# trifectatechfoundation/zlib-rs

Hardware: NVIDIA H100
Metric: deflate_level6_raw_input_throughput_silesia_small_tar (higher is better)
Workload: dtype u8

## Files before the change

### __graft_entry__.py

```python
import os
import subprocess
import sys

ROOT = os.path.dirname(os.path.abspath(__file__))
if ROOT not in sys.path:
    sys.path.insert(0, ROOT)
sys.path.insert(0, os.path.join(ROOT, "tests"))


def build():
    subprocess.check_call(["make", "-C", os.path.join(ROOT, "zlib_rs_b200", "csrc"), "-j8"])
    subprocess.check_call(["make", "-C", os.path.join(ROOT, "oracle")])
    subprocess.check_call(["make", "-C", os.path.join(ROOT, "oracle"), "ref"])
    subprocess.check_call(["make", "-C", os.path.join(ROOT, "tests", "hostmodel")])
    import zlib_rs_b200
    zlib_rs_b200.lib()


def smoke():
    import zlib
    import zlib_rs_b200 as Z
    import oracle_lib as O
    from corpus import synthetic_mix
    d = synthetic_mix(300000, seed=1)
    out = Z.compress2(d, 6)
    assert out == O.compress(d, 6)[1], "GPU deflate differs from the oracle"
    assert zlib.decompress(out) == d
    assert Z.uncompress(out, len(d)) == d
    assert Z.crc32(d) == O.crc32(d) and Z.adler32(d) == O.adler32(d)
    print("smoke ok: %d -> %d bytes, bit-exact vs oracle" % (len(d), len(out)))


if __name__ == "__main__":
    build()
    if len(sys.argv) > 1 and sys.argv[1] == "smoke":
        smoke()
```

### include/zb_engine.h

```cpp
#ifndef ZB_ENGINE_H
#define ZB_ENGINE_H
#include <stddef.h>
#include <stdint.h>

#ifdef __cplusplus
extern "C" {
#endif

#define ZB_API __attribute__((visibility("default")))

#define ZB_OK 0
#define ZB_E_NODEVICE (-100)
#define ZB_E_CUDA (-101)
#define ZB_E_BUF (-5)
#define ZB_E_MEM (-4)
#define ZB_E_PARAM (-2)
#define ZB_E_DATA (-3)
#define ZB_E_INTERNAL (-102)

typedef struct zb_engine zb_engine;

typedef struct zb_deflate_result {
    uint64_t out_bytes;
    uint32_t check;
    int32_t data_type;
    uint32_t iterations;
    uint32_t n_symbols;
    uint32_t n_blocks;
    uint32_t gpu_launches;
    int32_t exact_parity;
    float gpu_ms;
    uint32_t bits_used;
    uint32_t carry;
} zb_deflate_result;

ZB_API zb_engine *zb_engine_create(int device, int *err);
ZB_API void zb_engine_destroy(zb_engine *e);
ZB_API const char *zb_last_error(void);
ZB_API int zb_device_count(void);

ZB_API int zb_deflate(zb_engine *e, const void *src, size_t src_len, int src_on_device, void *dst, size_t dst_cap, int dst_on_device,
               int level, int strategy, int window_bits, zb_deflate_result *res);
#define ZB_FLAG_NOT_LAST 1u
#define ZB_FLAG_LOW_PARALLEL 2u
#define ZB_FLAG_CHECK_ADLER 4u
#define ZB_FLAG_CHECK_CRC 8u
#define ZB_FLAG_END_PARTIAL 16u
#define ZB_FLAG_END_BLOCK 32u
#define ZB_FLAG_PRIME(bits, val) ((((uint32_t)(bits) & 7u) << 12) | (((uint32_t)(val) & 0xffu) << 16))
#define ZB_FLAG_MEMLEVEL(m) ((uint32_t)(m) << 8)
ZB_API int zb_deflate_ex(zb_engine *e, const void *src, size_t src_len, int src_on_device, void *dst, size_t dst_cap, int dst_on_device,
                  int level, int strategy, int window_bits, uint32_t flags, zb_deflate_result *res);
ZB_API int zb_deflate_dict(zb_engine *e, const void *dict, size_t dict_len, const void *src, size_t src_len, int src_on_device, void *dst,
                           size_t dst_cap, int dst_on_device, int level, int strategy, int window_bits, uint32_t flags, zb_deflate_result *res);
ZB_API size_t zb_deflate_bound(size_t src_len);

typedef struct zb_inflate_result {
    uint64_t out_bytes;
    uint64_t in_bytes;
    uint32_t check;
    int32_t status;
    uint32_t gpu_launches;
    float gpu_ms;
    char msg[64];
} zb_inflate_result;

ZB_API int zb_inflate(zb_engine *e, const void *src, size_t src_len, int src_on_device, void *dst, size_t dst_cap, int dst_on_device,
               int window_bits, zb_inflate_result *res);

#define ZB_INF_CHECK_ADLER 1u
#define ZB_INF_CHECK_CRC 2u
ZB_API int zb_inflate_ex(zb_engine *e, const void *src, size_t src_len, int src_on_device, void *dst, size_t dst_cap, int dst_on_device,
                         int window_bits, uint32_t flags, zb_inflate_result *res);

typedef struct zb_inflate_seg {
    uint64_t out_bytes;
    uint64_t end_bit;
    uint32_t final_block, need_input, sync_point;
    uint32_t check;
    uint32_t gpu_launches;
    float gpu_ms;
    char msg[64];
} zb_inflate_seg;
ZB_API int zb_inflate_blocks(zb_engine *e, const void *src, size_t src_len, uint64_t start_bit, const void *dict, size_t dict_len,
                             void *dst, size_t dst_cap, int check_kind, uint32_t check_start, zb_inflate_seg *out);

ZB_API int zb_adler32(zb_engine *e, uint32_t start, const void *buf, size_t len, int on_device, uint32_t *out, float *gpu_ms);
ZB_API int zb_crc32(zb_engine *e, uint32_t start, const void *buf, size_t len, int on_device, uint32_t *out, float *gpu_ms);

ZB_API void zb_engine_set_profile(zb_engine *e, int on);
ZB_API int zb_engine_get_profile(zb_engine *e, float *ms, uint32_t *launches, int n);

ZB_API void *zb_device_alloc(zb_engine *e, size_t bytes);
ZB_API void zb_device_free(zb_engine *e, void *p);
ZB_API int zb_copy_to_device(zb_engine *e, void *dst, const void *src, size_t bytes);
ZB_API int zb_copy_to_host(zb_engine *e, void *dst, const void *src, size_t bytes);
ZB_API int zb_device_fill_random(zb_engine *e, void *dst, size_t bytes, uint64_t seed);

#ifdef __cplusplus
}
#endif
#endif
```

### zlib_rs_b200/__init__.py

```python
import ctypes
import os

_HERE = os.path.dirname(os.path.abspath(__file__))
LIB_PATH = os.environ.get("ZB_LIB_PATH") or os.path.join(_HERE, "libz_b200.so")

Z_OK, Z_STREAM_END, Z_NEED_DICT = 0, 1, 2
Z_ERRNO, Z_STREAM_ERROR, Z_DATA_ERROR, Z_MEM_ERROR, Z_BUF_ERROR, Z_VERSION_ERROR = -1, -2, -3, -4, -5, -6
Z_NO_FLUSH, Z_PARTIAL_FLUSH, Z_SYNC_FLUSH, Z_FULL_FLUSH, Z_FINISH, Z_BLOCK = 0, 1, 2, 3, 4, 5
Z_DEFAULT_STRATEGY, Z_FILTERED, Z_HUFFMAN_ONLY, Z_RLE, Z_FIXED = 0, 1, 2, 3, 4
ZLIB_VERSION = b"1.3.0-zlib-rs-0.6.7-b200"
ZB_FLAG_NOT_LAST = 1
ZB_FLAG_LOW_PARALLEL = 2
ZB_FLAG_CHECK_ADLER = 4
ZB_FLAG_CHECK_CRC = 8


class ZStream(ctypes.Structure):
    _fields_ = [("next_in", ctypes.c_void_p), ("avail_in", ctypes.c_uint), ("total_in", ctypes.c_ulong),
                ("next_out", ctypes.c_void_p), ("avail_out", ctypes.c_uint), ("total_out", ctypes.c_ulong),
                ("msg", ctypes.c_char_p), ("state", ctypes.c_void_p), ("zalloc", ctypes.c_void_p),
                ("zfree", ctypes.c_void_p), ("opaque", ctypes.c_void_p), ("data_type", ctypes.c_int),
                ("adler", ctypes.c_ulong), ("reserved", ctypes.c_ulong)]


class DeflateResult(ctypes.Structure):
    _fields_ = [("out_bytes", ctypes.c_uint64), ("check", ctypes.c_uint32), ("data_type", ctypes.c_int32),
                ("iterations", ctypes.c_uint32), ("n_symbols", ctypes.c_uint32), ("n_blocks", ctypes.c_uint32),
                ("gpu_launches", ctypes.c_uint32), ("exact_parity", ctypes.c_int32), ("gpu_ms", ctypes.c_float),
                ("bits_used", ctypes.c_uint32), ("carry", ctypes.c_uint32)]


class InflateResult(ctypes.Structure):
    _fields_ = [("out_bytes", ctypes.c_uint64), ("in_bytes", ctypes.c_uint64), ("check", ctypes.c_uint32),
                ("status", ctypes.c_int32), ("gpu_launches", ctypes.c_uint32), ("gpu_ms", ctypes.c_float),
                ("msg", ctypes.c_char * 64)]


class ZlibError(Exception):
    def __init__(self, code, msg=""):
        super().__init__("zlib error %d %s" % (code, msg))
        self.code = code
        self.msg = msg


_lib = None


def lib():
    global _lib
    if _lib is None:
        if not os.path.exists(LIB_PATH):
            raise RuntimeError("libz_b200.so is not built: run `python -c 'import __graft_entry__ as g; g.build()'` "
                               "or `make -C zlib_rs_b200/csrc` (needs nvcc, sm_90a)")
        L = ctypes.CDLL(LIB_PATH, mode=ctypes.RTLD_LOCAL)
        vp, sz, u32, u64, ci = ctypes.c_void_p, ctypes.c_size_t, ctypes.c_uint32, ctypes.c_uint64, ctypes.c_int
        ul = ctypes.c_ulong
        zs = ctypes.POINTER(ZStream)
        L.zlibVersion.restype = ctypes.c_char_p
        L.zError.restype, L.zError.argtypes = ctypes.c_char_p, [ci]
        L.deflateInit2_.argtypes = [zs, ci, ci, ci, ci, ci, ctypes.c_char_p, ci]
        L.deflateInit_.argtypes = [zs, ci, ctypes.c_char_p, ci]
        L.deflate.argtypes = [zs, ci]
        L.deflateEnd.argtypes = [zs]
        L.deflateReset.argtypes = [zs]
        L.deflateBound.argtypes, L.deflateBound.restype = [zs, ul], ul
        L.inflateInit2_.argtypes = [zs, ci, ctypes.c_char_p, ci]
        L.inflateInit_.argtypes = [zs, ctypes.c_char_p, ci]
        L.inflate.argtypes = [zs, ci]
        L.inflateEnd.argtypes = [zs]
        L.compress2.argtypes = [vp, ctypes.POINTER(ul), vp, ul, ci]
        L.compress.argtypes = [vp, ctypes.POINTER(ul), vp, ul]
        L.compressBound.argtypes, L.compressBound.restype = [ul], ul
        L.uncompress.argtypes = [vp, ctypes.POINTER(ul), vp, ul]
        L.uncompress2.argtypes = [vp, ctypes.POINTER(ul), vp, ctypes.POINTER(ul)]
        for f in ("adler32", "crc32"):
            getattr(L, f).argtypes, getattr(L, f).restype = [ul, vp, ctypes.c_uint], ul
            getattr(L, f + "_z").argtypes, getattr(L, f + "_z").restype = [ul, vp, sz], ul
        L.adler32_combine.argtypes, L.adler32_combine.restype = [ul, ul, ctypes.c_long], ul
        L.crc32_combine.argtypes, L.crc32_combine.restype = [ul, ul, ctypes.c_long], ul
        L.crc32_combine_gen.argtypes, L.crc32_combine_gen.restype = [ctypes.c_long], ul
        L.adler32_combine64.argtypes, L.adler32_combine64.restype = [ul, ul, ctypes.c_longlong], ul
        L.crc32_combine64.argtypes, L.crc32_combine64.restype = [ul, ul, ctypes.c_longlong], ul
        L.crc32_combine_gen64.argtypes, L.crc32_combine_gen64.restype = [ctypes.c_longlong], ul
        L.crc32_combine_op.argtypes, L.crc32_combine_op.restype = [ul, ul, ul], ul
        L.zb_engine_create.argtypes, L.zb_engine_create.restype = [ci, ctypes.POINTER(ci)], vp
        L.zb_engine_destroy.argtypes = [vp]
        L.zb_last_error.restype = ctypes.c_char_p
        L.zb_device_count.restype = ci
        L.zb_deflate.argtypes = [vp, vp, sz, ci, vp, sz, ci, ci, ci, ci, ctypes.POINTER(DeflateResult)]
        L.zb_deflate_ex.argtypes = [vp, vp, sz, ci, vp, sz, ci, ci, ci, ci, u32, ctypes.POINTER(DeflateResult)]
        L.zb_deflate_bound.argtypes, L.zb_deflate_bound.restype = [sz], sz
        L.zb_inflate.argtypes = [vp, vp, sz, ci, vp, sz, ci, ci, ctypes.POINTER(InflateResult)]
        L.zb_adler32.argtypes = [vp, u32, vp, sz, ci, ctypes.POINTER(u32), ctypes.POINTER(ctypes.c_float)]
        L.zb_crc32.argtypes = [vp, u32, vp, sz, ci, ctypes.POINTER(u32), ctypes.POINTER(ctypes.c_float)]
        L.zb_engine_set_profile.argtypes = [vp, ci]
        L.zb_engine_get_profile.argtypes = [vp, ctypes.POINTER(ctypes.c_float), ctypes.POINTER(u32), ci]
        L.zb_device_alloc.argtypes, L.zb_device_alloc.restype = [vp, sz], vp
        L.zb_device_free.argtypes = [vp, vp]
        L.zb_copy_to_device.argtypes = [vp, vp, vp, sz]
        L.zb_copy_to_host.argtypes = [vp, vp, vp, sz]
        L.zb_device_fill_random.argtypes = [vp, vp, sz, u64]
        _lib = L
    return _lib


def _buf(data):
    data = bytes(data)
    return data, (ctypes.c_char * max(len(data), 1)).from_buffer_copy(data or b"\0")


def compressBound(n):
    return lib().compressBound(n)


def compress2(data, level=-1):
    data, src = _buf(data)
    n = ctypes.c_ulong(lib().compressBound(len(data)))
    dst = ctypes.create_string_buffer(n.value)
    rc = lib().compress2(dst, ctypes.byref(n), src, len(data), level)
    if rc != Z_OK:
        raise ZlibError(rc, lib().zb_last_error().decode())
    return dst.raw[: n.value]


def compress(data):
    return compress2(data, -1)


def uncompress(data, bufsize):
    data, src = _buf(data)
    n = ctypes.c_ulong(bufsize)
    dst = ctypes.create_string_buffer(max(bufsize, 1))
    rc = lib().uncompress(dst, ctypes.byref(n), src, len(data))
    if rc != Z_OK:
        raise ZlibError(rc, lib().zb_last_error().decode())
    return dst.raw[: n.value]


def crc32(data, value=0):
    data, src = _buf(data)
    return lib().crc32_z(value, src if data else None, len(data)) if data else (value if True else 0)


def adler32(data, value=1):
    data, src = _buf(data)
    return lib().adler32_z(value, src, len(data)) if data else value


class Deflate:

    def __init__(self, level=-1, window_bits=15, mem_level=8, strategy=0):
        self.s = ZStream()
        rc = lib().deflateInit2_(ctypes.byref(self.s), level, 8, window_bits, mem_level, strategy, ZLIB_VERSION,
                                 ctypes.sizeof(ZStream))
        if rc != Z_OK:
            raise ZlibError(rc, (self.s.msg or b"").decode())
        self._open = True

    def deflate(self, data, flush=Z_NO_FLUSH, out_chunk=1 << 16):
        data, src = _buf(data)
        self.s.next_in = ctypes.addressof(src)
        self.s.avail_in = len(data)
        out = bytearray()
        obuf = ctypes.create_string_buffer(out_chunk)
        while True:
            self.s.next_out = ctypes.addressof(obuf)
            self.s.avail_out = out_chunk
            rc = lib().deflate(ctypes.byref(self.s), flush)
            out += obuf.raw[: out_chunk - self.s.avail_out]
            if rc == Z_STREAM_END:
                break
            if rc == Z_BUF_ERROR and self.s.avail_in == 0:
                break
            if rc != Z_OK:
                raise ZlibError(rc, (self.s.msg or b"").decode())
            if self.s.avail_out != 0 and self.s.avail_in == 0:
                break
        self.last_rc = rc
        return bytes(out)

    @property
    def adler(self):
        return self.s.adler

    @property
    def total_in(self):
        return self.s.total_in

    @property
    def total_out(self):
        return self.s.total_out

    @property
    def data_type(self):
        return self.s.data_type

    def end(self):
        if self._open:
            self._open = False
            return lib().deflateEnd(ctypes.byref(self.s))
        return Z_OK

    def __del__(self):
        try:
            self.end()
        except Exception:
            pass


class Inflate:

    def __init__(self, window_bits=15):
        self.s = ZStream()
        rc = lib().inflateInit2_(ctypes.byref(self.s), window_bits, ZLIB_VERSION, ctypes.sizeof(ZStream))
        if rc != Z_OK:
            raise ZlibError(rc, (self.s.msg or b"").decode())
        self._open = True
        self.eof = False

    def inflate(self, data, flush=Z_NO_FLUSH, out_chunk=1 << 16):
        data, src = _buf(data)
        self.s.next_in = ctypes.addressof(src)
        self.s.avail_in = len(data)
        out = bytearray()
        obuf = ctypes.create_string_buffer(out_chunk)
        while True:
            self.s.next_out = ctypes.addressof(obuf)
            self.s.avail_out = out_chunk
            rc = lib().inflate(ctypes.byref(self.s), flush)
            out += obuf.raw[: out_chunk - self.s.avail_out]
            if rc == Z_STREAM_END:
                self.eof = True
                break
            if rc == Z_BUF_ERROR:
                break
            if rc != Z_OK:
                raise ZlibError(rc, (self.s.msg or b"").decode())
            if self.s.avail_out != 0 and self.s.avail_in == 0:
                break
        self.last_rc = rc
        return bytes(out)

    @property
    def adler(self):
        return self.s.adler

    def end(self):
        if self._open:
            self._open = False
            return lib().inflateEnd(ctypes.byref(self.s))
        return Z_OK

    def __del__(self):
        try:
            self.end()
        except Exception:
            pass


class Engine:
    def __init__(self, device=0):
        err = ctypes.c_int(0)
        self.h = lib().zb_engine_create(device, ctypes.byref(err))
        if not self.h:
            raise RuntimeError("zb_engine_create failed (%d): %s" % (err.value, lib().zb_last_error().decode()))

    def close(self):
        if self.h:
            lib().zb_engine_destroy(self.h)
            self.h = None

    def __del__(self):
        try:
            self.close()
        except Exception:
            pass

    def _check(self, rc):
        if rc != 0:
            raise ZlibError(rc, lib().zb_last_error().decode())

    def alloc(self, n):
        p = lib().zb_device_alloc(self.h, n)
        if not p:
            raise MemoryError("zb_device_alloc(%d)" % n)
        return p

    def free(self, p):
        lib().zb_device_free(self.h, p)

    def to_device(self, dptr, data):
        data, src = _buf(data)
        self._check(lib().zb_copy_to_device(self.h, dptr, src, len(data)))

    def to_host(self, dptr, n):
        dst = ctypes.create_string_buffer(max(n, 1))
        self._check(lib().zb_copy_to_host(self.h, dst, dptr, n))
        return dst.raw[:n]

    def deflate(self, src, n=None, level=6, strategy=0, window_bits=15, flags=0, src_on_device=False, dst=None, dst_cap=0,
                dst_on_device=False, mem_level=8):
        res = DeflateResult()
        flags |= (mem_level & 15) << 8
        keep = None
        if not src_on_device:
            data, keep = _buf(src)
            n = len(data)
            src = ctypes.addressof(keep)
        own = None
        if dst is None:
            dst_cap = lib().zb_deflate_bound(n) + 64
            own = ctypes.create_string_buffer(dst_cap)
            dst = ctypes.addressof(own)
            dst_on_device = False
        rc = lib().zb_deflate_ex(self.h, src, n, int(src_on_device), dst, dst_cap, int(dst_on_device), level, strategy,
                                 window_bits, flags, ctypes.byref(res))
        self._check(rc)
        return (own.raw[: res.out_bytes] if own is not None else None), res

    def inflate(self, src, out_cap, n=None, window_bits=15, src_on_device=False, dst=None, dst_on_device=False):
        res = InflateResult()
        keep = None
        if not src_on_device:
            data, keep = _buf(src)
            n = len(data)
            src = ctypes.addressof(keep)
        own = None
        if dst is None:
            own = ctypes.create_string_buffer(max(out_cap, 1))
            dst = ctypes.addressof(own)
        rc = lib().zb_inflate(self.h, src, n, int(src_on_device), dst, out_cap, int(dst_on_device), window_bits, ctypes.byref(res))
        return rc, (own.raw[: res.out_bytes] if own is not None else None), res

    def adler32(self, buf, n=None, start=1, on_device=False):
        out, ms = ctypes.c_uint32(0), ctypes.c_float(0)
        keep = None
        if not on_device:
            data, keep = _buf(buf)
            n = len(data)
            buf = ctypes.addressof(keep)
        self._check(lib().zb_adler32(self.h, start, buf, n, int(on_device), ctypes.byref(out), ctypes.byref(ms)))
        return out.value, ms.value

    def crc32(self, buf, n=None, start=0, on_device=False):
        out, ms = ctypes.c_uint32(0), ctypes.c_float(0)
        keep = None
        if not on_device:
            data, keep = _buf(buf)
            n = len(data)
            buf = ctypes.addressof(keep)
        self._check(lib().zb_crc32(self.h, start, buf, n, int(on_device), ctypes.byref(out), ctypes.byref(ms)))
        return out.value, ms.value

    PHASES = ["links", "match", "nxt", "path", "emit_holes", "tail", "blocks", "encode", "checksum", "h2d", "d2h", "match_first"]

    def set_profile(self, on=True):
        lib().zb_engine_set_profile(self.h, int(on))

    def get_profile(self):
        ms = (ctypes.c_float * 12)()
        ln = (ctypes.c_uint32 * 12)()
        k = lib().zb_engine_get_profile(self.h, ms, ln, 12)
        return {self.PHASES[i]: {"ms": ms[i], "launches": ln[i]} for i in range(min(k, len(self.PHASES)))}

    def fill_random(self, dptr, n, seed=42):
        self._check(lib().zb_device_fill_random(self.h, dptr, n, seed))
```

### zlib_rs_b200/csrc/zb_engine.cu

```cuda
#include <cuda_runtime.h>
#include <stdio.h>
#include <stdlib.h>
#include <string.h>
#include <new>
#include "../../include/zb_engine.h"
#include "zb_kernels.cuh"
#include "zb_engine_internal.h"

namespace zb {

constexpr uint32_t kSlowSub9 = 24576;
constexpr uint32_t kTailTiles = 2;
constexpr uint32_t kTailSub = 512;

thread_local char g_err[256] = "";

static void set_err(const char *what, cudaError_t e)
{
    snprintf(g_err, sizeof g_err, "%s: %s", what, cudaGetErrorString(e));
}

#define CK(call)                                                  \
    do {                                                          \
        cudaError_t e_ = (call);                                  \
        if (e_ != cudaSuccess) { set_err(#call, e_); return ZB_E_CUDA; } \
    } while (0)

__global__ void k_match(JobBufs);
__global__ void k_skip(JobBufs);
__global__ void k_nxt(JobBufs);
__global__ void k_path_tiles(JobBufs);
__global__ void k_path_chain(JobBufs, uint32_t, uint32_t);
__global__ void k_path_groups(JobBufs, uint32_t, uint32_t, uint4 *, uint32_t *);
__global__ void k_path_chain2(JobBufs, uint32_t, uint32_t, const uint4 *, uint32_t *, uint32_t *);
__global__ void k_path_mark(JobBufs, const uint32_t *, const uint32_t *);
__global__ void k_iter_lists(JobBufs, uint32_t *, uint32_t *, uint32_t);
__global__ void k_emit(JobBufs);
__global__ void k_holes(JobBufs, uint32_t);
__global__ void k_holes_cmp(JobBufs, uint32_t, uint32_t);
__global__ void k_tail(JobBufs);
__global__ void k_block_hist(JobBufs, uint32_t *);
__global__ void k_build_blocks(JobBufs, const uint32_t *);
__global__ void k_scan_blocks(JobBufs);
__global__ void k_encode(JobBufs);
__global__ void k_finish(JobBufs, const uint32_t *);
__global__ void k_literal_syms(JobBufs);
__global__ void k_stored(JobBufs);
__global__ void k_links2_std(JobBufs, uint32_t);
__global__ void k_links2_roll(JobBufs, uint32_t);
__global__ void k_links_fix_std(JobBufs);
__global__ void k_links_fix_roll(JobBufs);
__global__ void k_slow(JobBufs);
__global__ void k_rle(JobBufs);
__global__ void k_emit_slow(JobBufs);
__global__ void k_tail_slow(JobBufs);
__global__ void k_serial_low(JobBufs);
__global__ void k_links_dict_ghost(JobBufs, uint32_t *);
__global__ void k_links_dict_ghost_apply(JobBufs, const uint32_t *);

constexpr uint32_t kMatchSmemBytes = (kWSize + kMatchSub + 512) + (kWSize + kMatchSub) * 2 + ((kWSize + kMatchSub) / 32 + 1) * 4 * 4 + 8192;
constexpr uint32_t kPathSmemBytes = kPathTile * 4 * 3;
constexpr uint32_t kLinks2SmemBytes = 65536 * 2 + kLinkTile * 2 + kLinkTile + 64 + 2048;
constexpr uint32_t kSkipSmemBytes = 2 * kWSize * 2 + 2 * (2 * kWSize / 32) * 4 + 8192 + 64;
constexpr uint32_t kSlowSubMax = 24576;
constexpr uint32_t kSlowSmemBytes = (kWSize + kSlowSubMax + kSlowAhead) * 3;
constexpr uint32_t kChainSmemBytes = kChainChunkTiles * kPathHead * 8;
constexpr uint32_t kChain2MaxSmem = 200 * 1024;
constexpr uint32_t kSerialSmemBytes = (65536 + kWSize) * 2 + 35824 + 16;
constexpr uint32_t kSerialSmemQuick = 65536 * 2 + 65536 + 16;

int Engine::init(int dev)
{
    int n = 0;
    cudaError_t e = cudaGetDeviceCount(&n);
    if (e != cudaSuccess || n == 0) {
        snprintf(g_err, sizeof g_err, "no CUDA device (%s)", e == cudaSuccess ? "count 0" : cudaGetErrorString(e));
        return ZB_E_NODEVICE;
    }
    if (dev < 0 || dev >= n) { snprintf(g_err, sizeof g_err, "device %d out of range", dev); return ZB_E_PARAM; }
    device = dev;
    CK(cudaSetDevice(dev));
    CK(cudaStreamCreateWithFlags(&st, cudaStreamNonBlocking));
    CK(cudaStreamCreateWithFlags(&st2, cudaStreamNonBlocking));
    CK(cudaEventCreateWithFlags(&evf, cudaEventDisableTiming));
    CK(cudaEventCreateWithFlags(&evt, cudaEventDisableTiming));
    for (int i = 0; i < kUpChunks; i++) CK(cudaEventCreateWithFlags(&evc[i], cudaEventDisableTiming));
    CK(cudaEventCreateWithFlags(&evk, cudaEventDisableTiming));
    CK(cudaEventCreate(&ev0));
    CK(cudaEventCreate(&ev1));
    CK(upload_tables());
    CK(cudaFuncSetAttribute(k_match, cudaFuncAttributeMaxDynamicSharedMemorySize, kMatchSmemBytes));
    CK(cudaFuncSetAttribute(k_skip, cudaFuncAttributeMaxDynamicSharedMemorySize, kSkipSmemBytes));
    CK(cudaFuncSetAttribute(k_links2_std, cudaFuncAttributeMaxDynamicSharedMemorySize, kLinks2SmemBytes));
    CK(cudaFuncSetAttribute(k_links2_roll, cudaFuncAttributeMaxDynamicSharedMemorySize, kLinks2SmemBytes));
    CK(cudaFuncSetAttribute(k_slow, cudaFuncAttributeMaxDynamicSharedMemorySize, kSlowSmemBytes));
    CK(cudaFuncSetAttribute(k_path_tiles, cudaFuncAttributeMaxDynamicSharedMemorySize, kPathSmemBytes));
    CK(cudaFuncSetAttribute(k_path_mark, cudaFuncAttributeMaxDynamicSharedMemorySize, kPathSmemBytes));
    CK(cudaFuncSetAttribute(k_path_chain, cudaFuncAttributeMaxDynamicSharedMemorySize, kChainSmemBytes));
    CK(cudaFuncSetAttribute(k_path_groups, cudaFuncAttributeMaxDynamicSharedMemorySize, kChain2MaxSmem));
    CK(cudaFuncSetAttribute(k_path_chain2, cudaFuncAttributeMaxDynamicSharedMemorySize, kChain2MaxSmem));
    CK(cudaFuncSetAttribute(k_serial_low, cudaFuncAttributeMaxDynamicSharedMemorySize, kSerialSmemBytes));
    CK(cudaMallocHost(&h_info, sizeof(JobInfo)));
    CK(cudaMalloc(&d_info, sizeof(JobInfo)));
    CK(cudaMalloc(&d_check, 16));
    { int rc_ = inflate_init(); if (rc_ != ZB_OK) return rc_; }
    return ZB_OK;
}

Engine::~Engine()
{
    if (device < 0) return;
    cudaSetDevice(device);
    for (auto &b : bufs) if (b.p) cudaFree(b.p);
    if (h_stage) cudaFreeHost(h_stage);
    if (h_info) cudaFreeHost(h_info);
    if (d_info) cudaFree(d_info);
    if (d_check) cudaFree(d_check);
    if (ev0) cudaEventDestroy(ev0);
    if (ev1) cudaEventDestroy(ev1);
    if (evf) cudaEventDestroy(evf);
    if (evt) cudaEventDestroy(evt);
    for (int i = 0; i < kUpChunks; i++) if (evc[i]) cudaEventDestroy(evc[i]);
    if (evk) cudaEventDestroy(evk);
    if (st2) cudaStreamDestroy(st2);
    if (st) cudaStreamDestroy(st);
}

void Engine::pbegin()
{
    if (!profile) return;
    if (!pev0) { cudaEventCreate(&pev0); cudaEventCreate(&pev1); }
    cudaEventRecord(pev0, st);
}

void Engine::pend(int phase, uint32_t nlaunch)
{
    if (!profile) return;
    cudaEventRecord(pev1, st);
    cudaEventSynchronize(pev1);
    float ms = 0;
    cudaEventElapsedTime(&ms, pev0, pev1);
    phase_ms[phase] += ms;
    phase_launches[phase] += nlaunch;
}

int Engine::reserve(int slot, size_t bytes, void **out)
{
    Buf &b = bufs[slot];
    if (b.cap < bytes) {
        if (b.p) { cudaFree(b.p); b.p = nullptr; b.cap = 0; }
        size_t want = bytes + (bytes >> 3) + 4096;
        cudaError_t e = cudaMalloc(&b.p, want);
        if (e != cudaSuccess) { set_err("cudaMalloc", e); return ZB_E_MEM; }
        b.cap = want;
    }
    *out = b.p;
    return ZB_OK;
}

int Engine::stage(size_t bytes)
{
    if (h_stage_cap < bytes) {
        if (h_stage) cudaFreeHost(h_stage);
        h_stage = nullptr;
        h_stage_cap = 0;
        cudaError_t e = cudaMallocHost(&h_stage, bytes + (bytes >> 3) + 4096);
        if (e != cudaSuccess) { set_err("cudaMallocHost", e); return ZB_E_MEM; }
        h_stage_cap = bytes + (bytes >> 3) + 4096;
    }
    return ZB_OK;
}

enum { S_IN, S_L, S_HOLES, S_HOLESN, S_M, S_NXT, S_PEXIT, S_PCNT, S_SYMIDX, S_TENTRY, S_TSYMB, S_TDIRTY, S_SYMS, S_SYMB,
       S_BLOCKS, S_SCRATCH, S_FREQ, S_OUT, S_CK, S_INF0, S_INF1, S_PHEAD, S_SK, S_MARKN, S_LLIST, S_LCNT, S_BMAP, S_HDIFF, S_HCOARSE, S_CSTATE, S_LISTS, S_LR, S_LLAST, S_BBASE, S_MCHG, S_GFN, S_KEYS, S_COUNT };
static_assert(S_COUNT <= Engine::kSlots, "slots");

size_t deflate_bound(size_t n)
{
    return n + ((n + 7) >> 3) + ((n + 63) >> 6) + 5 + 18 + 64;
}

int Engine::deflate(const void *src, size_t n_in, bool src_dev, void *dst, size_t dst_cap, bool dst_dev, int level, int strategy,
                    int window_bits, uint32_t flags, zb_deflate_result *res, const void *dict, size_t dict_len)
{
    size_t dstart = 0;
    if (dict_len) {
        if (!dict || window_bits >= 0) { snprintf(g_err, sizeof g_err, "a dictionary needs a raw stream (the caller frames FDICT / DICTID)"); return ZB_E_PARAM; }
        if (dict_len >= 2 * (size_t)kWSize) { dict = static_cast<const uint8_t *>(dict) + (dict_len - kWSize); dict_len = kWSize; }
        dstart = dict_len;
    }
    const size_t n = n_in + dstart;
    int mem_level = (int)((flags >> 8) & 15u);
    if (mem_level == 0) mem_level = 8;
    if (mem_level > 9) return ZB_E_PARAM;
    if (!res || (!src && n) || !dst) return ZB_E_PARAM;
    memset(res, 0, sizeof *res);
    if (n > 0xF0000000ull) { snprintf(g_err, sizeof g_err, "input too large for one job (%zu)", n); return ZB_E_PARAM; }
    if (level == -1) level = 6;
    if (level < 0 || level > 9 || strategy < 0 || strategy > 4) return ZB_E_PARAM;
    uint32_t wrap;
    if (window_bits < 0) { if (window_bits < -15 || window_bits > -8) return ZB_E_PARAM; wrap = 0; }
    else if (window_bits > 15) { if (window_bits < 24 || window_bits > 31) return ZB_E_PARAM; wrap = 2; }
    else { if (window_bits < 8) return ZB_E_PARAM; wrap = 1; }
    const int wb = window_bits < 0 ? -window_bits : window_bits > 15 ? window_bits - 16 : window_bits;
    CK(cudaSetDevice(device));
    const uint32_t N = (uint32_t)n;
    launches = 0;

    JobBufs jb;
    memset(&jb, 0, sizeof jb);
    int rc;
    void *p;
    const size_t npad = (size_t)N + kPad;
    const uint32_t nwords = (N >> 5) + 2;
    const uint32_t nmt = N / kMatchTile + 1, npt = N / kPathTile + 1;
    const bool low_parallel = (flags & ZB_FLAG_LOW_PARALLEL) != 0 || dstart != 0;
    const bool serial_low = (level == 1 || level == 2) && strategy != 2 && strategy != 3 && !low_parallel;
    const uint32_t block_syms = (serial_low && level == 1) ? kBlockSyms : (1u << (mem_level + 6)) - 1u;
    const uint32_t max_blocks = N / block_syms + 2;
    const size_t out_cap = (deflate_bound(n) + 15) & ~(size_t)15;
    if ((rc = stage((size_t)nmt + 64 + ((size_t)N / 512 + 2 + npt + nmt + 8) * 4 + 64)) != ZB_OK) return rc;
    uint8_t *h_dirty = static_cast<uint8_t *>(h_stage);
    uint32_t *h_lists = reinterpret_cast<uint32_t *>(static_cast<uint8_t *>(h_stage) + (((size_t)nmt + 64 + 15) & ~(size_t)15));
#define RES(slot, bytes, field, type)                                   \
    if ((rc = reserve(slot, bytes, &p)) != ZB_OK) return rc;            \
    jb.field = static_cast<type>(p);
    uint8_t *d_in;
    if ((rc = reserve(S_IN, npad + 16, &p)) != ZB_OK) return rc;
    d_in = static_cast<uint8_t *>(p);
    jb.in = d_in;
    jb.N = N;
    jb.start = (uint32_t)dstart;
    jb.nmt = nmt;
    jb.tail_start = N > 2 * kTailZone ? N - kTailZone : 0;
    jb.block_syms = block_syms;
    jb.serial_mode = serial_low ? (uint32_t)level : 0u;
    RES(S_L, npad * 2, L, uint16_t *)
    RES(S_SK, npad * 2, SK, uint16_t *)
    RES(S_HOLES, (size_t)nwords * 4, holes, uint32_t *)
    RES(S_HOLESN, (size_t)nwords * 4, holes_new, uint32_t *)
    RES(S_M, npad * 4, M, uint32_t *)
    RES(S_NXT, ((size_t)N + 16) * 4, nxt, uint32_t *)
    RES(S_PEXIT, ((size_t)N + 16) * 4, pexit, uint32_t *)
    RES(S_PCNT, ((size_t)N + 16) * 4, pcnt, uint32_t *)
    RES(S_SYMIDX, ((size_t)N + 16) * 4, symidx, uint32_t *)
    RES(S_PHEAD, (size_t)npt * kPathHead * 8, phead, uint2 *)
    RES(S_TENTRY, (size_t)npt * 4, tile_entry, uint32_t *)
    RES(S_TSYMB, (size_t)npt * 4, tile_symbase, uint32_t *)
    RES(S_MARKN, (size_t)npt + 16, mark_needed, uint8_t *)
    const uint32_t nlists = npt * (kPathTile / kPathSub);
    RES(S_LLIST, (size_t)nlists * kLongPerSub * 4, long_list, uint32_t *)
    RES(S_LCNT, (size_t)nlists * 4, long_cnt, uint32_t *)
    RES(S_TDIRTY, (size_t)nmt + 16, tile_dirty, uint8_t *)
    RES(S_SYMS, ((size_t)N + 64) * sizeof(Sym), syms, Sym *)
    RES(S_SYMB, 40000 * 4, sym_base, uint32_t *)
    RES(S_BMAP, (size_t)nmt * 8192, bucket_map, uint32_t *)
    RES(S_LR, npad * 2, Lr, uint16_t *)
    RES(S_KEYS, npad * 2, keys, uint16_t *)
    RES(S_LLAST, (size_t)nmt * 65536 * 2, link_last, uint16_t *)
    RES(S_CSTATE, (size_t)(npt + 1) * 16, chain_state, uint4 *)
    uint32_t chainG = 16;
    while ((uint64_t)chainG * chainG < npt) chainG += 8;
    const uint32_t chain_groups = (npt + chainG - 1) / chainG;
    const uint32_t chain2_smem = chainG * kPathHead * 8 + chain_groups * kPathHead * 16 + chainG * 8;
    const bool chain2 = chain2_smem <= kChain2MaxSmem;
    if ((rc = reserve(S_GFN, (size_t)chain_groups * kPathHead * 16 + ((size_t)npt + 4) * 4, &p)) != ZB_OK) return rc;
    uint4 *d_gfn = static_cast<uint4 *>(p);
    uint32_t *d_mark_cnt = reinterpret_cast<uint32_t *>(d_gfn + (size_t)chain_groups * kPathHead);
    uint32_t *d_mark_list = d_mark_cnt + 4;
    auto launch_chain = [&](uint32_t first_tile) {
        if (chain2) {
            k_path_groups<<<chain_groups, 1024, chainG * kPathHead * 8, st>>>(jb, npt, chainG, d_gfn, d_mark_cnt);
            k_path_chain2<<<chain_groups, 1024, chain2_smem, st>>>(jb, npt, chainG, d_gfn, d_mark_list, d_mark_cnt);
            launches++;
        } else k_path_chain<<<1, 1024, kChainSmemBytes, st>>>(jb, npt, first_tile);
    };
    auto launch_mark = [&](uint32_t grid) {
        if (chain2) k_path_mark<<<grid < npt ? grid : npt, 1024, kPathSmemBytes, st>>>(jb, d_mark_list, d_mark_cnt);
        else k_path_mark<<<npt, 1024, kPathSmemBytes, st>>>(jb, nullptr, nullptr);
    };
    uint32_t *d_lists;
    const uint32_t max_list = N / 512 + 2;
    if ((rc = reserve(S_LISTS, ((size_t)max_list + npt + nmt + 8) * 4, &p)) != ZB_OK) return rc;
    d_lists = static_cast<uint32_t *>(p);
    RES(S_HDIFF, (size_t)nwords * 8, hdiff, uint32_t *)
    jb.hdiff_words = nwords;
    RES(S_HCOARSE, (size_t)(N >> 10) + 16, hcoarse, uint8_t *)
    RES(S_MCHG, (((size_t)N >> 8) + 16) * 4 + 64, mchg, uint8_t *)
    RES(S_BLOCKS, (size_t)max_blocks * sizeof(BlockDesc), blocks, BlockDesc *)
    RES(S_BBASE, (size_t)max_blocks * 4, block_base, uint32_t *)
    uint32_t *d_freq;
    if ((rc = reserve(S_FREQ, (size_t)max_blocks * 320 * 4, &p)) != ZB_OK) return rc;
    d_freq = static_cast<uint32_t *>(p);
    uint8_t *d_out;
    if (dst_dev && dst_cap >= out_cap) d_out = static_cast<uint8_t *>(dst);
    else { if ((rc = reserve(S_OUT, out_cap + 16, &p)) != ZB_OK) return rc; d_out = static_cast<uint8_t *>(p); }
    jb.out = d_out;
    jb.out_cap = out_cap;
    void *d_ck;
    const size_t ck_bytes = ((size_t)N / 16384 + 16) * 8;
    if ((rc = reserve(S_CK, ck_bytes, &d_ck)) != ZB_OK) return rc;
#undef RES
    jb.info = d_info;
    jb.level = (uint32_t)level;
    jb.strategy_fixed = strategy == 4;
    const bool lf_zero = strategy >= 2;
    jb.wrap = wrap;
    jb.hdr_len = wrap == 1 ? 2 : wrap == 2 ? 10 : 0;
    jb.huffman_only = strategy == 2 && level != 0;
    jb.not_last = (flags & ZB_FLAG_NOT_LAST) ? 1 : 0;
    jb.end_mode = (flags & ZB_FLAG_END_PARTIAL) ? 1u : (flags & ZB_FLAG_END_BLOCK) ? 2u : 0u;
    jb.prime_bits = (flags >> 12) & 7u;
    if ((jb.end_mode && !jb.not_last) || (jb.prime_bits && wrap != 0)) { snprintf(g_err, sizeof g_err, "END_* needs NOT_LAST, PRIME a raw stream"); return ZB_E_PARAM; }
    if (jb.not_last && (level == 0 || wrap != 0)) { snprintf(g_err, sizeof g_err, "NOT_LAST needs raw deflate and level > 0"); return ZB_E_PARAM; }
    jb.xfl = level == 9 ? 2 : (strategy >= 2 || level < 2) ? 4 : 0;
    int eng_level = level;
    const int wb_eff = wb == 8 ? 9 : wb;
    const bool small_ok = wb_eff < 15 && (uint64_t)N + kMinLookahead <= (1ull << wb_eff);
    bool exact = (wb_eff == 15 || small_ok) && (dstart == 0 || wb_eff == 15);
    jb.cinfo = small_ok ? (uint32_t)(wb_eff - 8) : 7u;
    jb.wsize = kWSize;
    const bool serial_win = wb_eff < 15 && !small_ok && N <= 32000u && level >= 3 && level <= 6 && strategy != 2 && strategy != 3;
    if (serial_win) {
        jb.wsize = 1u << wb_eff;
        jb.cinfo = (uint32_t)(wb_eff - 8);
        jb.tail_start = 0;
        exact = true;
    }
    const bool par_win = wb_eff < 15 && !small_ok && !serial_win && level >= 3 && level <= 6 && strategy != 2 && strategy != 3 && dstart == 0;
    if (par_win) {
        jb.wsize = 1u << wb_eff;
        jb.cinfo = (uint32_t)(wb_eff - 8);
        exact = true;
    }
    const bool slow_win = wb_eff < 15 && !small_ok && dstart == 0 && level != 0 && ((level >= 7 && strategy != 2) || strategy == 3);
    if (slow_win) {
        jb.wsize = 1u << wb_eff;
        jb.cinfo = (uint32_t)(wb_eff - 8);
        exact = true;
    }
    if (wb_eff < 15 && (level == 0 || (strategy == 2 && level != 0) || serial_low)) {
        jb.wsize = 1u << wb_eff;
        jb.cinfo = (uint32_t)(wb_eff - 8);
        exact = true;
    }
    if (level != 0 && !jb.huffman_only) {
        if (level < 3 && !serial_low) { eng_level = 3; exact = exact && strategy == 3; }
        if (strategy == 3) jb.slow_mode = 2;
        else if (level > 6) { jb.slow_mode = 1; jb.sp = slow_params(level); jb.sp.filtered = strategy == 1; jb.sp.wsize = jb.wsize; }
    }
    if (jb.slow_mode) jb.tail_start = N;
    jb.lp = level_params(eng_level);
    if (level != 0 && !jb.huffman_only) jb.level = (uint32_t)level;
    if (lf_zero && !jb.strategy_fixed && !jb.huffman_only) jb.level = 1;

    CK(cudaEventRecord(ev0, st));
    if (profile) { for (int i = 0; i < kPhases; i++) { phase_ms[i] = 0; phase_launches[i] = 0; } }
    uint32_t up_chunks = 0;
    size_t up_len[kUpChunks] = {0};
    const bool chunked_upload = !src_dev && !dstart && n_in >= ((size_t)4 << 20) && level != 0 && !jb.huffman_only &&
                                !jb.serial_mode && jb.slow_mode != 2;
    if (chunked_upload) {
        size_t chunk = (n_in / kUpChunks + kLinkTile - 1) / kLinkTile * kLinkTile;
        if (chunk < (size_t)device_sm_count() * kLinkTile) chunk = (size_t)device_sm_count() * kLinkTile;
        CK(cudaStreamWaitEvent(st2, ev0, 0));
        for (size_t off = 0; off < n_in; off += chunk) {
            const size_t len = n_in - off < chunk ? n_in - off : chunk;
            CK(cudaMemcpyAsync(d_in + off, static_cast<const uint8_t *>(src) + off, len, cudaMemcpyHostToDevice, st2));
            if (off + len == n_in) CK(cudaMemsetAsync(d_in + n, 0, kPad, st2));
            CK(cudaEventRecord(evc[up_chunks], st2));
            up_len[up_chunks++] = off + len;
        }
    } else {
        pbegin();
        if (dstart) CK(cudaMemcpyAsync(d_in, dict, dstart, src_dev ? cudaMemcpyDefault : cudaMemcpyHostToDevice, st));
        if (n_in) CK(cudaMemcpyAsync(d_in + dstart, src, n_in, src_dev ? cudaMemcpyDeviceToDevice : cudaMemcpyHostToDevice, st));
        CK(cudaMemsetAsync(d_in + n, 0, kPad, st));
        pend(9, 0);
    }
    CK(cudaMemsetAsync(d_info, 0, sizeof(JobInfo), st));
    CK(cudaMemsetAsync(d_out, 0, out_cap, st));
    if (jb.prime_bits) {
        h_prime = (uint8_t)((flags >> 16) & ((1u << jb.prime_bits) - 1u));
        CK(cudaMemcpyAsync(d_out, &h_prime, 1, cudaMemcpyHostToDevice, st));
    }
    cudaStream_t st_ck = chunked_upload ? st2 : st;
    pbegin();
    if (wrap == 1 || (wrap == 0 && (flags & ZB_FLAG_CHECK_ADLER))) { CK(launch_adler32(d_in + dstart, n_in, 1, d_ck, ck_bytes, d_check, st_ck)); launches += 2; }
    else if (wrap == 2 || (wrap == 0 && (flags & ZB_FLAG_CHECK_CRC))) { CK(launch_crc32(d_in + dstart, n_in, 0, d_ck, ck_bytes, d_check, st_ck)); launches += 2; }
    else CK(cudaMemsetAsync(d_check, 0, 4, st_ck));
    if (chunked_upload) CK(cudaEventRecord(evk, st2));
    pend(8, 2);

    auto links_tiles = [&](bool roll) {
        uint32_t t_done = 0;
        for (uint32_t k = 0; k < (chunked_upload ? up_chunks : 1u); k++) {
            uint32_t t_hi = nmt;
            if (chunked_upload) {
                cudaStreamWaitEvent(st, evc[k], 0);
                if (k + 1 < up_chunks) t_hi = up_len[k] >= 64 ? (uint32_t)((up_len[k] - 64) / kLinkTile) : 0;
            }
            if (t_hi <= t_done) continue;
            if (roll) k_links2_roll<<<t_hi - t_done, 1024, kLinks2SmemBytes, st>>>(jb, t_done);
            else k_links2_std<<<t_hi - t_done, 1024, kLinks2SmemBytes, st>>>(jb, t_done);
            if (k) launches++;
            t_done = t_hi;
        }
        if (chunked_upload) cudaStreamWaitEvent(st, evk, 0);
    };
    uint32_t iters = 0;
    if (level == 0) {
        const uint32_t nb = n_in == 0 ? 1 : (uint32_t)((n_in + 65534) / 65535);
        k_stored<<<nb, 256, 0, st>>>(jb);
        launches++;
        k_finish<<<1, 32, 0, st>>>(jb, d_check);
        launches++;
    } else {
        if (jb.huffman_only) {
            k_literal_syms<<<(uint32_t)(n_in / 256 + 1), 256, 0, st>>>(jb);
            launches++;
        } else if (jb.serial_mode) {
            iters = 1;
            pbegin();
            k_serial_low<<<1, 32, jb.serial_mode == 2 ? kSerialSmemBytes : kSerialSmemQuick, st>>>(jb);
            launches++;
            pend(1, 1);
        } else {
            CK(cudaMemsetAsync(jb.holes, 0, (size_t)nwords * 4, st));
            CK(cudaMemsetAsync(jb.holes_new, 0, (size_t)nwords * 4, st));
            CK(cudaMemsetAsync(jb.tile_dirty, 1, nmt, st));
            CK(cudaMemsetAsync(jb.tile_entry, 0xee, (size_t)npt * 4, st));
            CK(cudaMemsetAsync(jb.M + N, 0, (size_t)kPad * 4, st));
            CK(cudaMemsetAsync(jb.L + N, 0, (size_t)kPad * 2, st));
            pbegin();
            if (jb.slow_mode == 2) {
            } else if (jb.slow_mode && jb.sp.slow) {
                links_tiles(true);
                k_links_fix_roll<<<N / 256 + 1, 256, 0, st>>>(jb);
                launches += 2;
            } else {
                links_tiles(false);
                k_links_fix_std<<<N / 256 + 1, 256, 0, st>>>(jb);
                launches += 2;
                if (dstart >= 3 && n_in) {
                    uint32_t *d_first = reinterpret_cast<uint32_t *>(d_check) + 2;
                    CK(cudaMemsetAsync(d_first, 0xff, 4, st));
                    k_links_dict_ghost<<<(kMaxDist + 255) / 256, 256, 0, st>>>(jb, d_first);
                    k_links_dict_ghost_apply<<<1, 32, 0, st>>>(jb, d_first);
                    launches += 2;
                }
            }
            if (!jb.slow_mode) CK(cudaMemcpyAsync(jb.Lr, jb.L, npad * 2, cudaMemcpyDeviceToDevice, st));
            pend(0, 1);
            if (jb.slow_mode) {
                if (n_in > 0) {
                    iters = 1;
                    pbegin();
                    if (jb.slow_mode == 2) k_rle<<<(N + 255) / 256, 256, 0, st>>>(jb);
                    else {
                        jb.match_sub = level >= 9 ? kSlowSub9 : level == 8 ? 4096u : 8192u;
                        k_slow<<<(N + jb.match_sub - 1) / jb.match_sub, 1024, (kWSize + jb.match_sub + kSlowAhead) * 3, st>>>(jb);
                    }
                    pend(1, 1);
                    if (profile) phase_ms[11] = phase_ms[1];
                    pbegin();
                    k_path_tiles<<<npt, 1024, kPathSmemBytes, st>>>(jb);
                    launch_chain(0);
                    launch_mark(npt);
                    pend(3, 3);
                    pbegin();
                    k_emit_slow<<<(N + 255) / 256, 256, 0, st>>>(jb);
                    pend(4, 1);
                    launches += 5;
                }
                pbegin();
                k_tail_slow<<<1, 32, 0, st>>>(jb);
                launches++;
                pend(5, 1);
            } else {
            if (jb.tail_start > 0) {
                uint32_t n_dirty = nmt;
                for (;;) {
                    iters++;
                    uint32_t mthreads = 1024;
                    if (iters == 1) jb.match_sub = 4096;
                    else if (n_dirty <= kTailTiles) { jb.match_sub = kTailSub; mthreads = 256; }
                    else {
                        const uint64_t per_cta = (uint64_t)n_dirty * kMatchTile / (4 * (uint64_t)device_sm_count());
                        jb.match_sub = per_cta >= 8192 ? 8192 : per_cta >= 4096 ? 4096 : per_cta >= 2048 ? 2048 : 1024;
                    }
                    uint32_t nsub = (N + jb.match_sub - 1) / jb.match_sub;
                    uint32_t n_ptiles = npt, first_ptile = 0;
                    jb.skip_list = nullptr;
                    jb.nxt_list = nullptr;
                    if (iters > 1) {
                        jb.skip_list = d_lists;
                        jb.nxt_list = d_lists + nmt + 8;
                        n_ptiles = h_info->n_ptiles ? h_info->n_ptiles : 1;
                        first_ptile = h_info->first_ptile;
                        nsub = (n_dirty ? n_dirty : 1) * (kMatchTile / jb.match_sub);
                        if (n_dirty) {
                            pbegin();
                            k_skip<<<n_dirty, 1024, kSkipSmemBytes, st>>>(jb);
                            pend(1, 1);
                            launches++;
                        }
                    }
                    const uint32_t msmem = (kWSize + jb.match_sub + 512) + (kWSize + jb.match_sub) * 2 +
                                           (iters > 1 ? ((kWSize + jb.match_sub) / 32 + 1) * 4 * 4 + 8192 : 64);
                    jb.use_bucket_map = iters > 1;
                    pbegin();
                    k_match<<<nsub, mthreads, msmem, st>>>(jb);
                    pend(1, 1);
                    if (profile && iters == 1) phase_ms[11] = phase_ms[1];
                    pbegin();
                    k_nxt<<<n_ptiles * (kPathTile / 1024), 1024, 0, st>>>(jb);
                    pend(2, 1);
                    pbegin();
                    k_path_tiles<<<n_ptiles, 1024, kPathSmemBytes, st>>>(jb);
                    launch_chain(first_ptile);
                    launch_mark(iters == 1 ? npt : 2 * n_ptiles + 16);
                    pend(3, 3);
                    pbegin();
                    k_holes<<<(nlists * kLongPerSub + 255) / 256, 256, 0, st>>>(jb, nlists);
                    k_holes_cmp<<<(nwords + 255) / 256, 256, 0, st>>>(jb, nwords, nmt);
                    pend(4, 2);
                    launches += 7;
                    k_iter_lists<<<1, 1024, 0, st>>>(jb, d_lists, d_lists + nmt + 8, npt);
                    launches++;
                    CK(cudaMemcpyAsync(h_info, d_info, sizeof(JobInfo), cudaMemcpyDeviceToHost, st));
                    CK(cudaStreamSynchronize(st));
                    if (h_info->error) { snprintf(g_err, sizeof g_err, "engine error flags 0x%x (parse)", h_info->error); return ZB_E_INTERNAL; }
                    if (getenv("ZB_DEBUG")) {
                        static unsigned long long last[3];
                        if (iters == 1) memset(last, 0, sizeof last);
                        const double ctas = (double)(h_info->dbg[0] - last[0]) + 1e-9;
                        fprintf(stderr, "iter %u dirty %u: ctas %llu stage %.1f walk %.1f kcyc/cta, holes_changed %u\n", iters, n_dirty,
                                h_info->dbg[0] - last[0], (h_info->dbg[1] - last[1]) / 1e3 / ctas, (h_info->dbg[2] - last[2]) / 1e3 / ctas,
                                h_info->holes_changed);
                        memcpy(last, h_info->dbg, sizeof last);
                    }
                    if (!h_info->holes_changed) break;
                    n_dirty = h_info->n_dirty;
                    if (iters > N / 257u + 4096u) { snprintf(g_err, sizeof g_err, "hole iteration did not converge"); return ZB_E_INTERNAL; }
                }
            }
            CK(cudaEventRecord(evf, st));
            CK(cudaStreamWaitEvent(st2, evf, 0));
            k_tail<<<1, 32, 0, st2>>>(jb);
            launches++;
            CK(cudaEventRecord(evt, st2));
            if (jb.tail_start > 0) {
                pbegin();
                k_emit<<<(jb.tail_start + 255) / 256, 256, 0, st>>>(jb);
                launches++;
                pend(4, 1);
            }
            pbegin();
            CK(cudaStreamWaitEvent(st, evt, 0));
            pend(5, 1);
            }
        }
        CK(cudaMemcpyAsync(h_info, d_info, sizeof(JobInfo), cudaMemcpyDeviceToHost, st));
        CK(cudaStreamSynchronize(st));
        if (h_info->error) { snprintf(g_err, sizeof g_err, "engine error flags 0x%x (tail)", h_info->error); return ZB_E_INTERNAL; }
        const uint32_t nblocks = h_info->n_blocks;
        if (nblocks == 0 || nblocks > max_blocks) { snprintf(g_err, sizeof g_err, "bad block count %u", nblocks); return ZB_E_INTERNAL; }
        pbegin();
        k_block_hist<<<nblocks, 256, 0, st>>>(jb, d_freq);
        k_build_blocks<<<nblocks, 32, 0, st>>>(jb, d_freq);
        k_scan_blocks<<<1, 256, 0, st>>>(jb);
        pend(6, 3);
        pbegin();
        k_encode<<<nblocks, 1024, 0, st>>>(jb);
        k_finish<<<1, 32, 0, st>>>(jb, d_check);
        pend(7, 2);
        launches += 5;
    }
    CK(cudaMemcpyAsync(h_info, d_info, sizeof(JobInfo), cudaMemcpyDeviceToHost, st));
    CK(cudaStreamSynchronize(st));
    CK(cudaGetLastError());
    if (h_info->error) {
        if (h_info->error & 8u) return ZB_E_BUF;
        snprintf(g_err, sizeof g_err, "engine error flags 0x%x (encode)", h_info->error);
        return ZB_E_INTERNAL;
    }
    const uint64_t out_bytes = h_info->out_bytes;
    if (out_bytes > dst_cap) {
        res->out_bytes = out_bytes;
        return ZB_E_BUF;
    }
    if (d_out != dst) {
        pbegin();
        CK(cudaMemcpyAsync(dst, d_out, out_bytes, dst_dev ? cudaMemcpyDeviceToDevice : cudaMemcpyDeviceToHost, st));
        pend(10, 0);
    }
    CK(cudaEventRecord(ev1, st));
    CK(cudaStreamSynchronize(st));
    float ms = 0;
    CK(cudaEventElapsedTime(&ms, ev0, ev1));
    res->out_bytes = out_bytes;
    res->check = h_info->adler;
    res->data_type = (int32_t)h_info->data_type;
    res->iterations = iters;
    res->n_symbols = h_info->n_syms;
    res->n_blocks = h_info->n_blocks;
    res->gpu_launches = launches;
    res->exact_parity = exact ? 1 : 0;
    res->gpu_ms = ms;
    res->bits_used = (uint32_t)(h_info->total_bits & 7u) ? (uint32_t)(h_info->total_bits & 7u) : 8u;
    if (jb.not_last && jb.end_mode && (h_info->total_bits & 7u)) {
        uint8_t last = 0;
        CK(cudaMemcpy(&last, d_out + out_bytes, 1, cudaMemcpyDeviceToHost));
        res->carry = last & ((1u << (h_info->total_bits & 7u)) - 1u);
    }
    return ZB_OK;
}

int Engine::checksum(bool crc, uint32_t start, const void *buf, size_t len, bool on_dev, uint32_t *out, float *ms_out)
{
    if (!out) return ZB_E_PARAM;
    CK(cudaSetDevice(device));
    int rc;
    void *p;
    const uint8_t *d = static_cast<const uint8_t *>(buf);
    CK(cudaEventRecord(ev0, st));
    if (!on_dev && len) {
        if ((rc = reserve(S_IN, len + 16, &p)) != ZB_OK) return rc;
        CK(cudaMemcpyAsync(p, buf, len, cudaMemcpyHostToDevice, st));
        d = static_cast<const uint8_t *>(p);
    }
    void *d_ck;
    const size_t ck_bytes = (len / 16384 + 16) * 8;
    if ((rc = reserve(S_CK, ck_bytes, &d_ck)) != ZB_OK) return rc;
    if (crc) CK(launch_crc32(d, len, start, d_ck, ck_bytes, d_check, st));
    else CK(launch_adler32(d, len, start, d_ck, ck_bytes, d_check, st));
    launches = 2;
    CK(cudaMemcpyAsync(h_info, d_check, 4, cudaMemcpyDeviceToHost, st));
    CK(cudaEventRecord(ev1, st));
    CK(cudaStreamSynchronize(st));
    *out = *reinterpret_cast<uint32_t *>(h_info);
    if (ms_out) CK(cudaEventElapsedTime(ms_out, ev0, ev1));
    return ZB_OK;
}

__global__ void k_fill_random(uint64_t *dst, uint64_t nwords, uint64_t seed)
{
    for (uint64_t i = blockIdx.x * (uint64_t)blockDim.x + threadIdx.x; i < nwords; i += (uint64_t)gridDim.x * blockDim.x) {
        uint64_t z = (i + seed) * 0x9E3779B97F4A7C15ull;
        z = (z ^ (z >> 30)) * 0xBF58476D1CE4E5B9ull;
        z = (z ^ (z >> 27)) * 0x94D049BB133111EBull;
        dst[i] = z ^ (z >> 31);
    }
}

}

using zb::Engine;

extern "C" {

struct zb_engine { Engine e; };

const char *zb_last_error(void) { return zb::g_err; }

int zb_device_count(void)
{
    int n = 0;
    if (cudaGetDeviceCount(&n) != cudaSuccess) return 0;
    return n;
}

zb_engine *zb_engine_create(int device, int *err)
{
    zb_engine *z = new (std::nothrow) zb_engine;
    int rc = z ? z->e.init(device) : ZB_E_MEM;
    if (err) *err = rc;
    if (rc != ZB_OK) { delete z; return nullptr; }
    return z;
}

void zb_engine_destroy(zb_engine *z) { delete z; }

int zb_deflate(zb_engine *z, const void *src, size_t n, int src_dev, void *dst, size_t cap, int dst_dev, int level, int strategy,
               int window_bits, zb_deflate_result *res)
{
    if (!z) return ZB_E_NODEVICE;
    return z->e.deflate(src, n, src_dev != 0, dst, cap, dst_dev != 0, level, strategy, window_bits, 0, res);
}

int zb_deflate_dict(zb_engine *z, const void *dict, size_t dict_len, const void *src, size_t n, int src_dev, void *dst, size_t cap, int dst_dev,
                    int level, int strategy, int window_bits, uint32_t flags, zb_deflate_result *res)
{
    if (!z) return ZB_E_NODEVICE;
    return z->e.deflate(src, n, src_dev != 0, dst, cap, dst_dev != 0, level, strategy, window_bits, flags, res, dict, dict_len);
}

int zb_deflate_ex(zb_engine *z, const void *src, size_t n, int src_dev, void *dst, size_t cap, int dst_dev, int level, int strategy,
                  int window_bits, uint32_t flags, zb_deflate_result *res)
{
    if (!z) return ZB_E_NODEVICE;
    return z->e.deflate(src, n, src_dev != 0, dst, cap, dst_dev != 0, level, strategy, window_bits, flags, res);
}

size_t zb_deflate_bound(size_t n) { return zb::deflate_bound(n); }

int zb_inflate(zb_engine *z, const void *src, size_t n, int src_dev, void *dst, size_t cap, int dst_dev, int window_bits,
               zb_inflate_result *res)
{
    if (!z) return ZB_E_NODEVICE;
    return z->e.inflate(src, n, src_dev != 0, dst, cap, dst_dev != 0, window_bits, res);
}

int zb_inflate_ex(zb_engine *z, const void *src, size_t n, int src_dev, void *dst, size_t cap, int dst_dev, int window_bits, uint32_t flags,
                  zb_inflate_result *res)
{
    if (!z) return ZB_E_NODEVICE;
    return z->e.inflate(src, n, src_dev != 0, dst, cap, dst_dev != 0, window_bits, res, flags);
}

int zb_inflate_blocks(zb_engine *z, const void *src, size_t n, uint64_t start_bit, const void *dict, size_t dict_len, void *dst, size_t cap,
                      int check_kind, uint32_t check_start, zb_inflate_seg *out)
{
    if (!z) return ZB_E_NODEVICE;
    return z->e.inflate_blocks(src, n, start_bit, dict, dict_len, dst, cap, check_kind, check_start, out);
}

int zb_adler32(zb_engine *z, uint32_t start, const void *buf, size_t len, int on_dev, uint32_t *out, float *ms)
{
    if (!z) return ZB_E_NODEVICE;
    return z->e.checksum(false, start, buf, len, on_dev != 0, out, ms);
}

int zb_crc32(zb_engine *z, uint32_t start, const void *buf, size_t len, int on_dev, uint32_t *out, float *ms)
{
    if (!z) return ZB_E_NODEVICE;
    return z->e.checksum(true, start, buf, len, on_dev != 0, out, ms);
}

void zb_engine_set_profile(zb_engine *z, int on) { if (z) z->e.profile = on != 0; }

int zb_engine_get_profile(zb_engine *z, float *ms, uint32_t *launches, int n)
{
    if (!z) return 0;
    int k = n < Engine::kPhases ? n : Engine::kPhases;
    for (int i = 0; i < k; i++) { if (ms) ms[i] = z->e.phase_ms[i]; if (launches) launches[i] = z->e.phase_launches[i]; }
    return k;
}

void *zb_device_alloc(zb_engine *z, size_t bytes)
{
    if (!z) return nullptr;
    cudaSetDevice(z->e.device);
    void *p = nullptr;
    if (cudaMalloc(&p, bytes + zb::kPad + 16) != cudaSuccess) return nullptr;
    cudaMemset(static_cast<uint8_t *>(p) + bytes, 0, zb::kPad);
    return p;
}

void zb_device_free(zb_engine *z, void *p)
{
    if (!z || !p) return;
    cudaSetDevice(z->e.device);
    cudaFree(p);
}

int zb_copy_to_device(zb_engine *z, void *dst, const void *src, size_t bytes)
{
    if (!z) return ZB_E_NODEVICE;
    cudaSetDevice(z->e.device);
    return cudaMemcpy(dst, src, bytes, cudaMemcpyHostToDevice) == cudaSuccess ? ZB_OK : ZB_E_CUDA;
}

int zb_copy_to_host(zb_engine *z, void *dst, const void *src, size_t bytes)
{
    if (!z) return ZB_E_NODEVICE;
    cudaSetDevice(z->e.device);
    return cudaMemcpy(dst, src, bytes, cudaMemcpyDeviceToHost) == cudaSuccess ? ZB_OK : ZB_E_CUDA;
}

int zb_device_fill_random(zb_engine *z, void *dst, size_t bytes, uint64_t seed)
{
    if (!z) return ZB_E_NODEVICE;
    cudaSetDevice(z->e.device);
    zb::k_fill_random<<<zb::device_sm_count() * 8, 256, 0, z->e.st>>>(static_cast<uint64_t *>(dst), bytes / 8, seed);
    return cudaStreamSynchronize(z->e.st) == cudaSuccess ? ZB_OK : ZB_E_CUDA;
}

}
```

### zlib_rs_b200/csrc/zb_engine_internal.h

```cpp
#pragma once
#include <cuda_runtime.h>
#include <stddef.h>
#include <stdint.h>
#include "../../include/zb_engine.h"
#include "zb_kernels.cuh"

namespace zb {

extern thread_local char g_err[256];
size_t deflate_bound(size_t n);

struct Engine {
    static constexpr int kSlots = 40;
    struct Buf { void *p = nullptr; size_t cap = 0; };
    int device = -1;
    cudaStream_t st = nullptr, st2 = nullptr;
    cudaEvent_t evf = nullptr, evt = nullptr;
    cudaEvent_t ev0 = nullptr, ev1 = nullptr;
    static constexpr int kUpChunks = 8;
    cudaEvent_t evk = nullptr;
    cudaEvent_t evc[kUpChunks] = {nullptr};
    Buf bufs[kSlots];
    void *h_stage = nullptr;
    size_t h_stage_cap = 0;
    JobInfo *h_info = nullptr, *d_info = nullptr;
    uint32_t *d_check = nullptr;
    void *d_inf_state = nullptr, *h_inf_state = nullptr;
    uint32_t launches = 0;
    uint8_t h_prime = 0;
    static constexpr int kPhases = 12;
    bool profile = false;
    float phase_ms[kPhases] = {0};
    uint32_t phase_launches[kPhases] = {0};
    cudaEvent_t pev0 = nullptr, pev1 = nullptr;
    void pbegin();
    void pend(int phase, uint32_t nlaunch);

    int init(int dev);
    int inflate_init();
    ~Engine();
    int reserve(int slot, size_t bytes, void **out);
    int stage(size_t bytes);
    int deflate(const void *src, size_t n, bool src_dev, void *dst, size_t dst_cap, bool dst_dev, int level, int strategy,
                int window_bits, uint32_t flags, zb_deflate_result *res, const void *dict = nullptr, size_t dict_len = 0);
    int inflate(const void *src, size_t n, bool src_dev, void *dst, size_t dst_cap, bool dst_dev, int window_bits,
                zb_inflate_result *res, uint32_t flags = 0);
    int inflate_blocks(const void *src, size_t n, uint64_t start_bit, const void *dict, size_t dict_len, void *dst, size_t dst_cap,
                       int check_kind, uint32_t check_start, zb_inflate_seg *out);
    int checksum(bool crc, uint32_t start, const void *buf, size_t len, bool on_dev, uint32_t *out, float *ms);
};

}
```

### zlib_rs_b200/csrc/zb_kernels.cu

```cuda
#include "zb_kernels.cuh"

namespace zb {

__constant__ HuffTables c_tab;

cudaError_t upload_tables()
{
    HuffTables t;
    init_tables(t);
    return cudaMemcpyToSymbol(c_tab, &t, sizeof t);
}

struct GAcc {
    const uint8_t *data;
    uint32_t N;
    const uint16_t *L;
    const uint32_t *holes;
    const uint32_t *M;
    uint32_t w = kWSize;
    __device__ __forceinline__ uint32_t byte(uint32_t y) const
    {
        while (y >= N) {
            if (y < 2 * w) return 0;
            y -= w;
        }
        return data[y];
    }
    __device__ __forceinline__ uint32_t link(uint32_t y) const { return y + 4 <= N ? L[y] : 0; }
    __device__ __forceinline__ bool inserted(uint32_t y) const { return !((holes[y >> 5] >> (y & 31)) & 1u); }
    __device__ __forceinline__ Match mlook(uint32_t x) const
    {
        uint32_t v = M[x];
        return Match{v >> 16, x - (v & 0xffffu)};
    }
};

struct SAcc {
    const uint8_t *sdata;
    const uint16_t *sL;
    const uint32_t *sholes;
    uint32_t ws;
    __device__ __forceinline__ uint32_t byte(uint32_t y) const { return sdata[y - ws]; }
    __device__ __forceinline__ uint32_t link(uint32_t y) const { return sL[y - ws]; }
    __device__ __forceinline__ bool inserted(uint32_t y) const
    {
        uint32_t i = y - ws;
        return !((sholes[i >> 5] >> (i & 31)) & 1u);
    }
};

struct SAccR {
    const uint8_t *sdata;
    const uint16_t *sL;
    uint32_t ws;
    __device__ __forceinline__ uint32_t byte(uint32_t y) const { return sdata[y - ws]; }
    __device__ __forceinline__ uint32_t link(uint32_t y) const { const uint32_t v = sL[y - ws]; return v == 0xffffu ? 0u : v; }
    __device__ __forceinline__ bool inserted(uint32_t) const { return true; }
};


__device__ __forceinline__ uint32_t lds_u32(const uint32_t *words, uint32_t byte_idx)
{
    const uint32_t w = byte_idx >> 2;
    return __funnelshift_r(words[w], words[w + 1], (byte_idx & 3u) * 8u);
}

constexpr uint32_t kFirstFlag = 0xffffu;

template <bool kRoll>
__device__ __forceinline__ void links2_body(const JobBufs &jb, uint32_t tile0)
{
    const uint32_t tile = tile0 + blockIdx.x;
    extern __shared__ __align__(16) uint8_t smem[];
    constexpr uint32_t kKeys = kRoll ? 32768u : 65536u;
    uint16_t *head = reinterpret_cast<uint16_t *>(smem);
    uint16_t *lists = reinterpret_cast<uint16_t *>(smem + kKeys * 2);
    uint8_t *sd = smem + kKeys * 2 + kLinkTile * 2;
    uint16_t *run = reinterpret_cast<uint16_t *>(smem + kKeys * 2 + kLinkTile * 2 + kLinkTile + 64);
    __shared__ uint16_t c_base[32], c_total[32];
    const uint32_t *words = reinterpret_cast<const uint32_t *>(sd);
    const uint32_t tid = threadIdx.x, lane = tid & 31, warp = tid >> 5;
    const uint32_t N = jb.N, need = kRoll ? 3u : 4u, cap = kRoll ? jb.wsize - 1u : jb.wsize - kMinLookahead;
    const uint32_t ts = tile * kLinkTile;
    const uint32_t te = min(ts + kLinkTile, N);
    const uint32_t tv = N >= need ? min(te, N - need + 1) : ts;
    for (uint32_t i = tid; i < kKeys / 2; i += 1024) reinterpret_cast<uint32_t *>(head)[i] = 0;
    run[tid] = 0;
    {
        const uint4 *src = reinterpret_cast<const uint4 *>(jb.in + ts);
        uint4 *dst = reinterpret_cast<uint4 *>(sd);
        for (uint32_t i = tid; i < (te - ts + 16 + 15) / 16; i += 1024) dst[i] = src[i];
    }
    __syncthreads();
    const uint32_t nv = tv > ts ? tv - ts : 0;
    auto key_of = [&](uint32_t i) -> uint32_t { return kRoll ? hash_roll3(sd[i], sd[i + 1], sd[i + 2]) : hash_u32(lds_u32(words, i)); };
    uint16_t *myrun = run + warp * 32;
    for (uint32_t b = 0; b < 32; b++) {
        const uint32_t i = warp * 1024 + b * 32 + lane;
        const uint32_t key = i < nv ? key_of(i) : 0u;
        const uint32_t c = i < nv ? (key & 31u) : 32u;
        if (!kRoll && i < nv) jb.keys[ts + i] = (uint16_t)key;
        const uint32_t peers = __match_any_sync(0xffffffffu, c);
        if (c < 32u && (peers & ((1u << lane) - 1u)) == 0) myrun[c] += (uint16_t)__popc(peers);
        __syncwarp();
    }
    __syncthreads();
    if (warp == 0) {
        uint32_t tot = 0;
        for (uint32_t w = 0; w < 32; w++) { const uint32_t t = run[w * 32 + lane]; run[w * 32 + lane] = (uint16_t)tot; tot += t; }
        uint32_t incl = tot;
#pragma unroll
        for (int d = 1; d < 32; d <<= 1) { const uint32_t t = __shfl_up_sync(0xffffffffu, incl, d); if (lane >= (uint32_t)d) incl += t; }
        const uint32_t base = incl - tot;
        for (uint32_t w = 0; w < 32; w++) run[w * 32 + lane] += (uint16_t)base;
        c_base[lane] = (uint16_t)base;
        c_total[lane] = (uint16_t)tot;
    }
    __syncthreads();
    for (uint32_t b = 0; b < 32; b++) {
        const uint32_t i = warp * 1024 + b * 32 + lane;
        const uint32_t c = i < nv ? (key_of(i) & 31u) : 32u;
        const uint32_t peers = __match_any_sync(0xffffffffu, c);
        const uint32_t lower = peers & ((1u << lane) - 1u);
        if (c < 32u) {
            const uint32_t at = myrun[c];
            lists[at + __popc(lower)] = (uint16_t)i;
        }
        __syncwarp();
        if (c < 32u && lower == 0) myrun[c] += (uint16_t)__popc(peers);
        __syncwarp();
    }
    __syncthreads();
    {
        const uint32_t lb = c_base[warp], ln = c_total[warp];
        for (uint32_t k = 0; k < ln; k += 32) {
            const bool mine = k + lane < ln;
            const uint32_t m = __ballot_sync(0xffffffffu, mine);
            if (mine) {
                const uint32_t i = lists[lb + k + lane];
                const uint32_t key = key_of(i);
                const uint32_t peers = __match_any_sync(m, key);
                const uint32_t lower = peers & ((1u << lane) - 1u);
                const uint32_t pi = __shfl_sync(m, i, lower ? 31 - __clz(lower) : lane);
                const uint32_t pred = lower ? pi + 1 : head[key];
                uint32_t d = pred ? i + 1 - pred : kFirstFlag;
                if (pred && d > cap) d = 0;
                jb.L[ts + i] = (uint16_t)d;
                if ((peers >> lane) == 1u) head[key] = (uint16_t)(i + 1);
            }
            __syncwarp();
        }
    }
    for (uint32_t x = tv + tid; x < te; x += 1024) jb.L[x] = 0;
    __syncthreads();
    uint4 *out = reinterpret_cast<uint4 *>(jb.link_last + (size_t)tile * kKeys);
    const uint4 *hv = reinterpret_cast<const uint4 *>(head);
    for (uint32_t i = tid; i < kKeys * 2 / 16; i += 1024) out[i] = hv[i];
}

template <bool kRoll>
__device__ __forceinline__ void links_fix_body(const JobBufs &jb)
{
    constexpr uint32_t kKeys = kRoll ? 32768u : 65536u;
    const uint32_t x = blockIdx.x * 256 + threadIdx.x;
    if (x >= jb.N || jb.L[x] != kFirstFlag) return;
    const uint32_t tile = x / kLinkTile, cap = kRoll ? jb.wsize - 1u : jb.wsize - kMinLookahead;
    uint32_t d = 0;
    if (tile > 0) {
        const uint8_t *q = jb.in + x;
        const uint32_t key = kRoll ? hash_roll3(q[0], q[1], q[2])
                                   : hash_u32((uint32_t)q[0] | ((uint32_t)q[1] << 8) | ((uint32_t)q[2] << 16) | ((uint32_t)q[3] << 24));
        const uint32_t last = jb.link_last[(size_t)(tile - 1) * kKeys + key];
        if (last) {
            d = x - ((tile - 1) * kLinkTile + last - 1);
            if (d > cap) d = 0;
        }
    }
    jb.L[x] = (uint16_t)d;
}

__global__ void __launch_bounds__(1024) k_links2_std(JobBufs jb, uint32_t tile0) { links2_body<false>(jb, tile0); }
__global__ void __launch_bounds__(1024) k_links2_roll(JobBufs jb, uint32_t tile0) { links2_body<true>(jb, tile0); }
__global__ void __launch_bounds__(256) k_links_fix_std(JobBufs jb) { links_fix_body<false>(jb); }
__global__ void __launch_bounds__(256) k_links_fix_roll(JobBufs jb) { links_fix_body<true>(jb); }

constexpr uint32_t kSkipSpan = 2 * kWSize;
__global__ void __launch_bounds__(1024) k_skip(JobBufs jb)
{
    extern __shared__ __align__(16) uint8_t smem[];
    uint16_t *sL = reinterpret_cast<uint16_t *>(smem);
    uint32_t *sh = reinterpret_cast<uint32_t *>(smem + kSkipSpan * 2);
    uint32_t *sf = sh + kSkipSpan / 32;
    uint32_t *sbm = sf + kSkipSpan / 32;
    const uint32_t tile = jb.skip_list ? jb.skip_list[blockIdx.x] : blockIdx.x;
    const uint32_t ts = tile * kMatchTile;
    if (ts >= jb.N) return;
    const uint32_t te = min(ts + kMatchTile, jb.N);
    const uint32_t ws = ts >= kWSize ? ts - kWSize : 0;
    const uint32_t span = te - ws, tid = threadIdx.x;
    const uint32_t md = jb.wsize - kMinLookahead;
    {
        const uint4 *ls = reinterpret_cast<const uint4 *>(jb.L + ws);
        uint4 *ld = reinterpret_cast<uint4 *>(sL);
        for (uint32_t i = tid; i < (span + 7) / 8; i += 1024) ld[i] = ls[i];
        for (uint32_t i = tid; i < (span + 31) / 32; i += 1024) sh[i] = jb.holes[(ws >> 5) + i];
        const uint32_t *bm1 = jb.bucket_map + (size_t)tile * 2048, *bm0 = tile ? bm1 - 2048 : bm1;
        for (uint32_t i = tid; i < 2048; i += 1024) sbm[i] = bm0[i] | bm1[i];
    }
    __syncthreads();
    {
        const uint4 *kp = reinterpret_cast<const uint4 *>(jb.keys + ws);
        const uint32_t ngrp = ((span + 31) & ~31u) / 8, ngrp_w = (ngrp + 31) & ~31u;
#pragma unroll 4
        for (uint32_t g = tid; g < ngrp_w; g += 1024) {
            const bool valid = g < ngrp;
            const uint4 kv = valid ? kp[g] : make_uint4(0, 0, 0, 0);
            const uint32_t k[8] = {kv.x & 0xffffu, kv.x >> 16, kv.y & 0xffffu, kv.y >> 16, kv.z & 0xffffu, kv.z >> 16, kv.w & 0xffffu, kv.w >> 16};
            uint32_t b = 0;
#pragma unroll
            for (int j = 0; j < 8; j++) b |= ((sbm[k[j] >> 5] >> (k[j] & 31u)) & 1u) << j;
            b <<= 8 * (tid & 3u);
            b |= __shfl_xor_sync(0xffffffffu, b, 1);
            b |= __shfl_xor_sync(0xffffffffu, b, 2);
            if (valid && (tid & 3u) == 0) sf[g >> 2] = b;
        }
    }
    __syncthreads();
    const uint32_t lane = tid & 31, warp = tid >> 5, nwords = (span + 31) / 32;
    uint32_t nz[2];
#pragma unroll
    for (int h = 0; h < 2; h++) {
        const uint32_t w = warp * 64 + lane + 32 * h;
        nz[h] = __ballot_sync(0xffffffffu, w < nwords && (sh[w] & sf[w]) != 0);
    }
    for (uint32_t round = 0; round < 24; round++) {
        int ch = 0;
#pragma unroll
        for (int h = 0; h < 2; h++) {
            uint32_t m = nz[h];
            while (m) {
                const uint32_t w = warp * 64 + (__ffs(m) - 1) + 32 * h;
                m &= m - 1;
                const uint32_t i = w * 32 + lane;
                const bool on = (((sh[w] & sf[w]) >> lane) & 1u) && i < span;
                for (int rep = 0; rep < 6; rep++) {
                    bool c = false;
                    if (on) {
                        const uint32_t d = sL[i];
                        if (d != 0 && d <= i) {
                            const uint32_t t = i - d;
                            if ((sh[t >> 5] >> (t & 31)) & 1u) {
                                const uint32_t d2 = sL[t];
                                sL[i] = (uint16_t)((d2 == 0 || d + d2 > md) ? 0u : d + d2);
                                c = true;
                            }
                        }
                    }
                    __syncwarp();
                    if (!__any_sync(0xffffffffu, c)) break;
                    ch = 1;
                }
            }
        }
        if (!__syncthreads_or(ch)) break;
    }
    for (uint32_t i = ts - ws + tid; i < span; i += 1024) {
        if (sf[i >> 5] == 0) continue;
        if (!((sf[i >> 5] >> (i & 31)) & 1u)) continue;
        uint32_t d = sL[i];
        if (!((sh[i >> 5] >> (i & 31)) & 1u) && d != 0 && d <= i) {
            const uint32_t t = i - d;
            if ((sh[t >> 5] >> (t & 31)) & 1u) {
                const uint32_t d2 = sL[t];
                d = (d2 == 0 || d + d2 > md) ? 0u : d + d2;
            }
        }
        jb.Lr[ws + i] = (uint16_t)d;
    }
}

constexpr uint32_t kMatchData = kWSize + kMatchSub + 512;
constexpr uint32_t kMatchSmem = kMatchData + (kWSize + kMatchSub) * 2 + ((kWSize + kMatchSub) / 32) * 4;

constexpr uint32_t kBatch = 8;
constexpr uint32_t kBatchCmp = 2;
constexpr uint32_t kWalkBurst = 8;
constexpr uint32_t kCmpBurst = 4;
constexpr uint32_t kCoopCmp = 4;
enum { LS_IDLE = 0, LS_WALK = 1, LS_PEND = 2, LS_DONE = 3, LS_FIN = 4 };

struct DiffMaps {
    const uint32_t *del, *pdel;
    const uint32_t *add, *padd;
    __device__ __forceinline__ static bool any(const uint32_t *b, const uint32_t *p, uint32_t lo, uint32_t hi)
    {
        const uint32_t c_hi = p[hi >> 5] + __popc(b[hi >> 5] & ((1u << (hi & 31)) - 1u));
        const uint32_t c_lo = p[lo >> 5] + __popc(b[lo >> 5] & ((1u << (lo & 31)) - 1u));
        return c_hi != c_lo;
    }
};

__device__ __forceinline__ void sld_u64u(uint32_t a, uint32_t &lo, uint32_t &hi)
{
    const uint32_t al = a & ~3u, sh = (a & 3u) * 8u;
    const uint32_t w0 = sld_u32(al), w1 = sld_u32(al + 4), w2 = sld_u32(al + 8);
    lo = __funnelshift_r(w0, w1, sh);
    hi = __funnelshift_r(w1, w2, sh);
}

__device__ __forceinline__ void match_tile_fast(const JobBufs &jb, const uint8_t *sdata, const uint16_t *sL, const uint32_t *sbm,
                                                const DiffMaps dm, uint32_t ws, uint32_t te, uint32_t *s_next)
{
    const bool filt = jb.use_bucket_map != 0;
    const uint32_t dbase = (uint32_t)__cvta_generic_to_shared(sdata);
    const uint32_t lbase = (uint32_t)__cvta_generic_to_shared(sL);
    const uint32_t N = jb.N, nice = jb.lp.nice, budget = jb.lp.chain;
    const uint32_t md = jb.wsize - kMinLookahead;
    const uint32_t lane = threadIdx.x & 31;
    uint32_t *const Mout = jb.M + ws;
    uint16_t *const RDout = jb.SK + ws;
    uint32_t xr = 0;
    uint32_t cr = 0;
    uint32_t dn = 0;
    uint32_t best = 2, chain = 0, res = 0;
    uint32_t xb = 0;
    uint32_t fbase = 0;
    uint32_t lowr = 0;
    uint32_t clen = 0;
    uint32_t rd = 0;
    uint32_t xw4 = 0;
    uint32_t state = LS_IDLE;
    auto second_look = [&]() -> bool {
        const uint32_t w = sld_u32u((best >= 3u ? fbase - 3u : dbase) + cr) ^ xw4;
        return (best >= 3u ? w : (w & 0x00ffffffu)) == 0u;
    };
    auto load_xw4 = [&]() { xw4 = sld_u32u((best >= 3u ? fbase - 3u : dbase) + xr); };
    for (;;) {
        if (state == LS_WALK) {
            if (chain > kWalkBurst) {
                uint32_t crl = cr - lowr;
                uint32_t fl = fbase + lowr, ll = lbase + 2 * lowr;
                asm volatile("" : "+r"(fl), "+r"(ll));
                bool more = false;
#pragma unroll
                for (uint32_t k = 0; k < kWalkBurst; k++) {
                    const uint32_t fbk = sld_u8(fl + crl);
                    dn = sld_u16(ll + 2 * crl);
                    if (fbk == xb) break;
                    chain--;
                    if ((int32_t)crl < (int32_t)dn) break;
                    crl -= dn;
                    if (k + 1 == kWalkBurst) more = true;
                }
                cr = crl + lowr;
                const uint32_t fb = more ? ~xb : sld_u8(fl + crl);
                if (!more) {
                    if (fb == xb) {
                        if (second_look()) { state = LS_PEND; clen = 0; }
                        else {
                            chain--;
                            if (cr < lowr + dn) { rd = 0xffffu; state = LS_FIN; }
                            else cr -= dn;
                        }
                    }
                    else { rd = 0xffffu; state = LS_FIN; }
                }
            } else {
                const uint32_t fb = sld_u8(fbase + cr);
                dn = sld_u16(lbase + 2 * cr);
                if (fb == xb && second_look()) { state = LS_PEND; clen = 0; }
                else if (--chain == 0) { rd = (xr - cr) | 0x8000u; state = LS_FIN; }
                else if (cr < lowr + dn) { rd = 0xffffu; state = LS_FIN; }
                else cr -= dn;
            }
        }
        const uint32_t m_walk = __ballot_sync(0xffffffffu, state == LS_WALK);
        const uint32_t m_pend = __ballot_sync(0xffffffffu, state == LS_PEND);
        if (m_pend && (__popc(m_pend) >= (int)kBatchCmp || m_walk == 0)) {
            uint32_t len = 0;
            bool resolved = false;
            if (state == LS_PEND) {
                uint32_t pa = dbase + xr + clen, pb = dbase + cr + clen;
#pragma unroll 1
                for (uint32_t k = 0; k < kCmpBurst; k++) {
                    uint32_t a0, a1, b0, b1;
                    sld_u64u(pa, a0, a1);
                    sld_u64u(pb, b0, b1);
                    const uint32_t d0 = a0 ^ b0, d1 = a1 ^ b1;
                    if ((d0 | d1) != 0 || clen + 8 >= kMaxMatch) {
                        len = d0 ? clen + ((__ffs(d0) - 1) >> 3) : d1 ? clen + 4 + ((__ffs(d1) - 1) >> 3) : clen + 8;
                        resolved = true;
                        break;
                    }
                    clen += 8; pa += 8; pb += 8;
                }
            }
            uint32_t m_long = 0;
            if (__popc(m_walk | m_pend) <= kCoopCmp) m_long = __ballot_sync(0xffffffffu, state == LS_PEND && !resolved);
            if (m_long) {
                while (m_long) {
                    const uint32_t src = __ffs(m_long) - 1;
                    m_long &= m_long - 1;
                    const uint32_t cl0 = __shfl_sync(0xffffffffu, clen, src);
                    const uint32_t pa0 = __shfl_sync(0xffffffffu, dbase + xr + clen, src) + 8u * lane;
                    const uint32_t pb0 = __shfl_sync(0xffffffffu, dbase + cr + clen, src) + 8u * lane;
                    uint32_t a0, a1, b0, b1;
                    sld_u64u(pa0, a0, a1);
                    sld_u64u(pb0, b0, b1);
                    const uint32_t d0 = a0 ^ b0, d1 = a1 ^ b1;
                    const uint32_t mm = __ballot_sync(0xffffffffu, (d0 | d1) != 0);
                    const uint32_t first = mm ? __ffs(mm) - 1 : 0u;
                    const uint32_t mine = d0 ? ((__ffs(d0) - 1) >> 3) : 4u + ((__ffs(d1) - 1) >> 3);
                    const uint32_t bo = __shfl_sync(0xffffffffu, mine, first);
                    if (lane == src) { len = mm ? cl0 + 8u * first + bo : cl0 + 256u; resolved = true; }
                }
            }
            if (resolved) {
                if (len > kMaxMatch) len = kMaxMatch;
                state = LS_WALK;
                if (len > best) {
                    best = len;
                    res = (len << 16) | (xr - cr);
                    if (best >= nice) { rd = xr - cr; state = LS_FIN; }
                    else { fbase = dbase + best; xb = sld_u8(fbase + xr); load_xw4(); }
                }
                if (state == LS_WALK) {
                    if (--chain == 0) { rd = (xr - cr) | 0x8000u; state = LS_FIN; }
                    else if (cr < lowr + dn) { rd = 0xffffu; state = LS_FIN; }
                    else cr -= dn;
                }
            }
        }
        if (state == LS_FIN) {
            if (filt && Mout[xr] != res) jb.mchg[(ws + xr) >> 6] = 1;
            Mout[xr] = res; RDout[xr] = (uint16_t)rd; state = LS_IDLE;
        }
        const uint32_t m_idle = __ballot_sync(0xffffffffu, state == LS_IDLE);
        const uint32_t m_busy = __ballot_sync(0xffffffffu, state == LS_WALK || state == LS_PEND);
        if ((m_idle | m_busy) == 0) break;
        if (m_idle == 0) continue;
        if (__popc(m_idle) < (int)kBatch && m_busy != 0) continue;
        {
            uint32_t base = 0;
            const uint32_t leader = __ffs(m_idle) - 1;
            if (lane == leader) base = atomicAdd(s_next, (uint32_t)__popc(m_idle));
            base = __shfl_sync(0xffffffffu, base, leader);
            if (state == LS_IDLE) {
                const uint32_t x = base + __popc(m_idle & ((1u << lane) - 1u));
                if (x >= te) state = LS_DONE;
                else if (x + kMSafe > N) { jb.M[x] = 0; }
                else {
                    xr = x - ws;
                    bool skip = false;
                    if (filt) {
                        const uint32_t h = hash_u32(sld_u32u(dbase + xr));
                        skip = !((sbm[h >> 5] >> (h & 31)) & 1u);
                        if (!skip) {
                            const uint32_t rdo = RDout[xr];
                            const bool on_budget = rdo != 0xffffu && (rdo & 0x8000u);
                            const uint32_t lo = rdo == 0xffffu ? (xr > md ? xr - md : 0u) : xr - (rdo & 0x7fffu);
                            bool redo = DiffMaps::any(dm.del, dm.pdel, lo, xr);
                            if (!redo) {
                                if (on_budget) redo = DiffMaps::any(dm.add, dm.padd, lo, xr);
                                else {
                                    const uint32_t m = Mout[xr];
                                    if (m) { const uint32_t h2 = xr - (m & 0xffffu); redo = (dm.add[h2 >> 5] >> (h2 & 31)) & 1u; }
                                }
                            }
                            if (!redo) redo = sld_u16(lbase + 2 * xr) == md;
                            skip = !redo;
                        }
                    }
                    if (!skip) {
                        const uint32_t d0 = sld_u16(lbase + 2 * xr);
                        lowr = xr > md ? xr - md : 0;
                        if (ws == 0 && lowr == 0) lowr = 1;
                        if (xr < lowr + d0) {
                            if (filt && Mout[xr] != 0) jb.mchg[(ws + xr) >> 6] = 1;
                            Mout[xr] = 0; RDout[xr] = 0xffffu;
                        }
                        else {
                            cr = xr - d0;
                            if (lowr + md == xr) lowr++;
                            best = 2; chain = budget; res = 0;
                            fbase = dbase + 2;
                            xb = sld_u8(fbase + xr);
                            load_xw4();
                            state = LS_WALK;
                        }
                    }
                }
            }
        }
    }
}

__global__ void __launch_bounds__(1024, 2) k_match(JobBufs jb)
{
    extern __shared__ __align__(16) uint8_t smem[];
    __shared__ uint32_t s_next;
    __shared__ __align__(8) unsigned long long s_mbar;
    const uint32_t sub = jb.match_sub;
    const uint32_t per_tile = kMatchTile / sub;
    const uint32_t ts = (jb.skip_list ? jb.skip_list[blockIdx.x / per_tile] * per_tile + blockIdx.x % per_tile : blockIdx.x) * sub;
    if (ts >= jb.N) return;
    {
        const uint32_t t0 = ts / kMatchTile, t1 = (min(ts + sub, jb.N) - 1) / kMatchTile;
        if (!jb.tile_dirty[t0] && !jb.tile_dirty[t1]) return;
    }
    const uint32_t data_bytes = kWSize + sub + 512;
    uint8_t *sdata = smem;
    uint16_t *sL = reinterpret_cast<uint16_t *>(smem + data_bytes);
    uint32_t *sh = reinterpret_cast<uint32_t *>(smem + data_bytes + (kWSize + sub) * 2);
    uint32_t *sbm = sh;
    const uint32_t wmax = (kWSize + sub) / 32 + 1;
    uint32_t *sdel = sbm + 2048, *pdel = sdel + wmax, *sadd = pdel + wmax, *padd = sadd + wmax;
    __shared__ uint32_t s_wsum[32];
    const uint32_t N = jb.N;
    const uint32_t te = min(ts + sub, N);
    const uint32_t ws = ts >= kWSize ? ts - kWSize : 0;
    const uint32_t tid = threadIdx.x, nthr = blockDim.x;
    if (jb.use_bucket_map) {
        const uint32_t mt = ts / kMatchTile;
        const uint32_t *bm1 = jb.bucket_map + (size_t)mt * 2048, *bm0 = mt ? bm1 - 2048 : bm1;
        int hit = 0;
        for (uint32_t x = ts + tid; x < te; x += nthr) {
            const uint8_t *q = jb.in + x;
            const uint32_t h = hash_u32((uint32_t)q[0] | ((uint32_t)q[1] << 8) | ((uint32_t)q[2] << 16) | ((uint32_t)q[3] << 24));
            if (((bm0[h >> 5] | bm1[h >> 5]) >> (h & 31)) & 1u) {
                const uint32_t rd = jb.SK[x];
                const uint32_t lo = rd == 0xffffu ? (x > jb.wsize - kMinLookahead ? x - (jb.wsize - kMinLookahead) : 0u) : x - (rd & 0x7fffu);
                for (uint32_t b = lo >> 10; b <= (x >> 10); b++) hit |= jb.hcoarse[b];
            }
        }
        if (!__syncthreads_or(hit)) return;
        for (uint32_t i = tid; i < 2048; i += nthr) sbm[i] = bm0[i] | bm1[i];
        const uint32_t nwd = (te - ws + 31) / 32;
        const uint32_t per = (nwd + 1 + nthr - 1) / nthr;
        const uint32_t wb = tid * per;
        const uint32_t lane_ = tid & 31, warp_ = tid >> 5;
        for (int which = 0; which < 2; which++) {
            const uint32_t *src = which ? jb.hdiff : jb.hdiff + jb.hdiff_words;
            uint32_t *bits = which ? sadd : sdel, *pre = which ? padd : pdel;
            uint32_t mine = 0;
            for (uint32_t k = 0; k < per; k++) {
                const uint32_t w = wb + k;
                if (w <= nwd) { const uint32_t v = w < nwd ? src[(ws >> 5) + w] : 0u; bits[w] = v; mine += __popc(v); }
            }
            uint32_t incl = mine;
#pragma unroll
            for (int d = 1; d < 32; d <<= 1) {
                const uint32_t t = __shfl_up_sync(0xffffffffu, incl, d);
                if (lane_ >= (uint32_t)d) incl += t;
            }
            __syncthreads();
            if (lane_ == 31) s_wsum[warp_] = incl;
            __syncthreads();
            uint32_t run = incl - mine;
            for (uint32_t k = 0; k < warp_; k++) run += s_wsum[k];
            for (uint32_t k = 0; k < per; k++) {
                const uint32_t w = wb + k;
                if (w <= nwd) { pre[w] = run; run += __popc(bits[w]); }
            }
        }
    }
    if (tid == 0) {
        s_next = ts;
        const uint32_t mb = (uint32_t)__cvta_generic_to_shared(&s_mbar);
        asm volatile("mbarrier.init.shared::cta.b64 [%0], 1;" ::"r"(mb) : "memory");
        asm volatile("fence.proxy.async.shared::cta;" ::: "memory");
    }
    const long long t_0 = clock64();
    __syncthreads();
    {
        uint32_t n16 = (te + 512 - ws + 15) / 16;
        if (n16 > data_bytes / 16) n16 = data_bytes / 16;
        const bool bulk = (reinterpret_cast<uintptr_t>(jb.in) & 15u) == 0;
        if (bulk) {
            if (tid == 0) {
                const uint32_t mb = (uint32_t)__cvta_generic_to_shared(&s_mbar), dsts = (uint32_t)__cvta_generic_to_shared(sdata);
                asm volatile("mbarrier.arrive.expect_tx.shared::cta.b64 _, [%0], %1;" ::"r"(mb), "r"(n16 * 16u) : "memory");
                asm volatile("cp.async.bulk.shared::cluster.global.mbarrier::complete_tx::bytes [%0], [%1], %2, [%3];"
                             ::"r"(dsts), "l"(jb.in + ws), "r"(n16 * 16u), "r"(mb) : "memory");
            }
        } else {
            const uint4 *src = reinterpret_cast<const uint4 *>(jb.in + ws);
            uint4 *dst = reinterpret_cast<uint4 *>(sdata);
            for (uint32_t i = tid; i < n16; i += nthr) dst[i] = src[i];
        }
        const uint32_t nl = (te - ws + 7) / 8;
        const uint4 *ls = reinterpret_cast<const uint4 *>(jb.Lr + ws);
        uint4 *ld = reinterpret_cast<uint4 *>(sL);
        for (uint32_t i = tid; i < nl; i += nthr) {
            uint4 v = ls[i];
            v.x |= __vcmpeq2(v.x, 0u); v.y |= __vcmpeq2(v.y, 0u); v.z |= __vcmpeq2(v.z, 0u); v.w |= __vcmpeq2(v.w, 0u);
            ld[i] = v;
        }
        if (bulk) {
            const uint32_t mb = (uint32_t)__cvta_generic_to_shared(&s_mbar);
            uint32_t done = 0;
            while (!done) {
                asm volatile("{\n.reg .pred p;\nmbarrier.try_wait.parity.shared::cta.b64 p, [%1], 0;\nselp.u32 %0, 1, 0, p;\n}"
                             : "=r"(done) : "r"(mb) : "memory");
            }
        }
    }
    __syncthreads();
    const long long t_1 = clock64();
    const LevelParams lp = jb.lp;
    if (!lp.early_exit) {
        match_tile_fast(jb, sdata, sL, sbm, DiffMaps{sdel, pdel, sadd, padd}, ws, te, &s_next);
        __syncthreads();
        if (tid == 0) {
            const long long t_2 = clock64();
            atomicAdd(&jb.info->dbg[0], 1ull);
            atomicAdd(&jb.info->dbg[1], (unsigned long long)(t_1 - t_0));
            atomicAdd(&jb.info->dbg[2], (unsigned long long)(t_2 - t_1));
        }
        return;
    }
    SAccR a{sdata, sL, ws};
    for (uint32_t x = ts + tid; x < te; x += nthr) {
        uint32_t v = 0;
        if (jb.use_bucket_map && x + 4 <= N) {
            const uint32_t h = hash_u32(a.byte(x) | (a.byte(x + 1) << 8) | (a.byte(x + 2) << 16) | (a.byte(x + 3) << 24));
            if (!((sbm[h >> 5] >> (h & 31)) & 1u)) continue;
        }
        if (x + kMSafe <= N) {
            Match m = jb.wsize == kWSize ? lm_walk(a, x, 0xffffffffu, lp) : lm_walk(a, x, 0xffffffffu, lp, DynWin{jb.wsize});
            if (m.len) v = (m.len << 16) | (x - m.start);
        }
        if (jb.use_bucket_map && jb.M[x] != v) jb.mchg[x >> 6] = 1;
        jb.M[x] = v;
        jb.SK[x] = 0xffffu;
    }
}

constexpr uint32_t kMacroReach = 22016;

__device__ __forceinline__ bool path_tile_dirty(const JobBufs &jb, uint32_t pt)
{
    const uint32_t m0 = (pt * kPathTile) / kMatchTile;
    uint32_t m1 = ((pt + 1) * kPathTile + kMacroReach - 1) / kMatchTile;
    if (m1 >= jb.nmt) m1 = jb.nmt - 1;
    bool d = false;
    for (uint32_t m = m0; m <= m1; m++) d = d || jb.tile_dirty[m];
    return d;
}

__global__ void __launch_bounds__(1024) k_nxt(JobBufs jb)
{
    constexpr uint32_t per = kPathTile / 1024;
    const uint32_t tile = jb.nxt_list ? jb.nxt_list[blockIdx.x / per] : blockIdx.x / per;
    if (!path_tile_dirty(jb, tile)) return;
    const uint32_t p = tile * kPathTile + (blockIdx.x % per) * 1024 + threadIdx.x;
    if (p >= jb.tail_start) return;
    if (jb.use_bucket_map) {
        const uint32_t old = jb.nxt[p];
        const uint32_t b0 = p >> 6, b1 = min(p + (old & 0xffffu), jb.N) >> 6;
        bool chg = false;
        for (uint32_t b = b0; b <= b1; b++) chg = chg || jb.mchg[b];
        if (!chg) return;
    }
    GAcc a{jb.in, jb.N, jb.L, jb.holes, jb.M, jb.wsize};
    const uint32_t long_len = 16 * jb.lp.lazy;
    uint32_t ns = 0, nlong = 0, lpos = 0, llen = 0;
    auto see = [&](const Sym &s) {
        if (s.dist && (uint32_t)s.lc + 3u > long_len) { nlong++; lpos = s.pos; llen = s.lc + 3u; }
    };
    const uint32_t np = jb.wsize == kWSize ? macro_step(a, p, jb.lp, jb.tail_start, see, &ns)
                                           : macro_step(a, p, jb.lp, jb.tail_start, see, &ns, DynWin{jb.wsize});
    const uint32_t delta = np - p;
    if (delta > 0xffffu || ns > 0xffu || delta == 0) atomicOr(&jb.info->error, 1u);
    if (nlong && (nlong != 1 || lpos + llen != np || (jb.lp.early_exit ? lpos != p : (llen != 257u && llen != 258u))))
        atomicOr(&jb.info->error, 16u);
    jb.nxt[p] = (delta & 0xffffu) | ((ns & 0xffu) << 16) | (nlong ? kNxtLong : 0u) | (llen == 258u ? kNxtLong258 : 0u) |
                (np >= jb.tail_start ? kNxtTail : 0u);
}

constexpr uint32_t kStuck = 0x80000000u;
__device__ __forceinline__ void path_subtile(const uint32_t *nx, uint32_t *ex, uint32_t *cn, uint32_t s0, uint32_t s1, uint32_t lane)
{
    for (int32_t b = (int32_t)s1 - 32; b >= (int32_t)s0; b -= 32) {
        const uint32_t p = (uint32_t)b + lane;
        const uint32_t v = nx[p];
        uint32_t t, c;
        if (v & kNxtTail) { t = kStuck | p; c = 0; }
        else { t = p + (v & 0xffffu); c = (v >> 16) & 0xffu; }
#pragma unroll
        for (int r = 0; r < 5; r++) {
            const bool inb = !(t & kStuck) && t < (uint32_t)b + 32u;
            const uint32_t src = inb ? t - (uint32_t)b : lane;
            const uint32_t t2 = __shfl_sync(0xffffffffu, t, src);
            const uint32_t c2 = __shfl_sync(0xffffffffu, c, src);
            if (inb) { t = t2; c += c2; }
        }
        if (!(t & kStuck) && t < s1) { c += cn[t]; t = ex[t]; }
        ex[p] = t;
        cn[p] = c;
        __syncwarp();
    }
}

constexpr uint32_t kPathSmem = kPathTile * 4 * 3;

__device__ __forceinline__ void path_load(const JobBufs &jb, uint32_t tbeg, uint32_t *nx)
{
    const uint4 *src = reinterpret_cast<const uint4 *>(jb.nxt + tbeg);
    uint4 *dst = reinterpret_cast<uint4 *>(nx);
#pragma unroll 4
    for (uint32_t g = threadIdx.x; g < kPathTile / 4; g += blockDim.x) {
        const uint32_t p = tbeg + 4 * g;
        uint4 v;
        if (p + 3 < jb.tail_start) v = src[g];
        else {
            const uint32_t t = kNxtTail | 1u;
            v.x = p < jb.tail_start ? jb.nxt[p] : t;
            v.y = p + 1 < jb.tail_start ? jb.nxt[p + 1] : t;
            v.z = p + 2 < jb.tail_start ? jb.nxt[p + 2] : t;
            v.w = t;
        }
        dst[g] = v;
    }
}

__global__ void __launch_bounds__(1024) k_path_tiles(JobBufs jb)
{
    extern __shared__ __align__(16) uint8_t smem[];
    uint32_t *nx = reinterpret_cast<uint32_t *>(smem);
    uint32_t *ex = nx + kPathTile;
    uint32_t *cn = ex + kPathTile;
    const uint32_t tile = jb.nxt_list ? jb.nxt_list[blockIdx.x] : blockIdx.x;
    const uint32_t tbeg = tile * kPathTile;
    if (!path_tile_dirty(jb, tile)) return;
    path_load(jb, tbeg, nx);
    __syncthreads();
    const uint32_t warp = threadIdx.x >> 5, lane = threadIdx.x & 31;
    constexpr uint32_t kExitSub = 1024, nsub = kPathTile / kExitSub;
    for (uint32_t s = warp; s < nsub; s += blockDim.x / 32) path_subtile(nx, ex, cn, s * kExitSub, (s + 1) * kExitSub, lane);
    __syncthreads();
    for (int32_t j = (int32_t)nsub - 2; j >= 0; j--) {
        for (uint32_t i = threadIdx.x; i < kExitSub; i += blockDim.x) {
            const uint32_t p = (uint32_t)j * kExitSub + i;
            uint32_t t = ex[p];
            if (!(t & kStuck) && t < kPathTile) { cn[p] += cn[t]; ex[p] = ex[t]; }
        }
        __syncthreads();
    }
    for (uint32_t i = threadIdx.x; i < kPathTile; i += blockDim.x) {
        const uint32_t p = tbeg + i;
        const uint32_t t = ex[i];
        const uint32_t xa = (t & kStuck) ? (kStuck | (tbeg + (t & ~kStuck))) : tbeg + t;
        if (p < jb.tail_start) {
            jb.pexit[p] = xa;
            jb.pcnt[p] = cn[i];
        }
        if (i < kPathHead) jb.phead[(size_t)tile * kPathHead + i] = make_uint2(xa, cn[i]);
    }
}

constexpr uint32_t kChainChunk = kChainChunkTiles;
__global__ void __launch_bounds__(1024) k_path_chain(JobBufs jb, uint32_t ntiles, uint32_t first_tile)
{
    extern __shared__ __align__(16) uint8_t smem[];
    uint2 *hd = reinterpret_cast<uint2 *>(smem);
    __shared__ uint32_t s_e, s_base, s_done, s_tail;
    __shared__ uint32_t c_entry[kChainChunk], c_base[kChainChunk];
    if (threadIdx.x == 0) {
        if (first_tile == 0) { s_e = jb.start; s_base = 0; s_done = jb.tail_start == 0; s_tail = jb.start; }
        else { const uint4 v = jb.chain_state[first_tile]; s_e = v.x; s_base = v.y; s_done = v.z; s_tail = v.w; }
    }
    for (uint32_t t = threadIdx.x; t < first_tile; t += blockDim.x) jb.mark_needed[t] = 0;
    __syncthreads();
    for (uint32_t c0 = first_tile; c0 < ntiles; c0 += kChainChunk) {
        const uint32_t nt = min(kChainChunk, ntiles - c0);
        for (uint32_t i = threadIdx.x; i < nt * kPathHead; i += blockDim.x) hd[i] = jb.phead[(size_t)c0 * kPathHead + i];
        __syncthreads();
        if (threadIdx.x == 0) {
            uint32_t e = s_e, base = s_base;
            bool done = s_done != 0;
            uint32_t tail_entry = s_tail;
            for (uint32_t k = 0; k < nt; k++) {
                const uint32_t tbeg = (c0 + k) * kPathTile, tend = tbeg + kPathTile;
                jb.chain_state[c0 + k] = make_uint4(e, base, done ? 1u : 0u, tail_entry);
                c_base[k] = base;
                if (done || e >= tend || e >= jb.tail_start) { c_entry[k] = 0xffffffffu; continue; }
                c_entry[k] = e;
                uint32_t x, c;
                if (e - tbeg < kPathHead) { const uint2 v = hd[k * kPathHead + (e - tbeg)]; x = v.x; c = v.y; }
                else { x = jb.pexit[e]; c = jb.pcnt[e]; }
                base += c;
                if (x & kStuck) { tail_entry = x & ~kStuck; done = true; }
                else e = x;
            }
            s_e = e; s_base = base; s_done = done; s_tail = tail_entry;
        }
        __syncthreads();
        for (uint32_t k = threadIdx.x; k < nt; k += blockDim.x) {
            const uint32_t t = c0 + k;
            jb.tile_symbase[t] = c_base[k];
            jb.mark_needed[t] = (jb.tile_entry[t] != c_entry[k]) || path_tile_dirty(jb, t);
            jb.tile_entry[t] = c_entry[k];
        }
        __syncthreads();
    }
    if (threadIdx.x == 0) {
        uint32_t tail_entry = s_tail;
        if (!s_done) { tail_entry = s_e; if (s_e < jb.tail_start) atomicOr(&jb.info->error, 2u); }
        jb.info->tail_entry = tail_entry;
        jb.info->n_mid_syms = s_base;
    }
}

struct ChainState { uint32_t e, base, done, tail; };

template <bool OUT>
__device__ __forceinline__ void chain_walk_group(const JobBufs &jb, const uint2 *hd, uint32_t t0, uint32_t nt, ChainState &s,
                                                 uint32_t *c_entry, uint32_t *c_base)
{
    for (uint32_t k = 0; k < nt; k++) {
        const uint32_t tbeg = (t0 + k) * kPathTile, tend = tbeg + kPathTile;
        if (OUT) c_base[k] = s.base;
        if (s.done || s.e >= tend || s.e >= jb.tail_start) { if (OUT) c_entry[k] = 0xffffffffu; continue; }
        if (OUT) c_entry[k] = s.e;
        uint32_t x, c;
        if (s.e - tbeg < kPathHead) { const uint2 v = hd[k * kPathHead + (s.e - tbeg)]; x = v.x; c = v.y; }
        else { x = jb.pexit[s.e]; c = jb.pcnt[s.e]; }
        s.base += c;
        if (x & kStuck) { s.tail = x & ~kStuck; s.done = 1; }
        else s.e = x;
    }
}

__device__ __forceinline__ void chain_stage_heads(const JobBufs &jb, uint2 *hd, uint32_t t0, uint32_t nt)
{
    const uint4 *src = reinterpret_cast<const uint4 *>(jb.phead + (size_t)t0 * kPathHead);
    uint4 *dst = reinterpret_cast<uint4 *>(hd);
    for (uint32_t i = threadIdx.x; i < nt * kPathHead / 2; i += blockDim.x) dst[i] = src[i];
}

__global__ void __launch_bounds__(1024) k_path_groups(JobBufs jb, uint32_t ntiles, uint32_t G, uint4 *gfn, uint32_t *mark_cnt)
{
    if (blockIdx.x == 0 && threadIdx.x == 0) *mark_cnt = 0;
    extern __shared__ __align__(16) uint8_t smem[];
    uint2 *hd = reinterpret_cast<uint2 *>(smem);
    const uint32_t t0 = blockIdx.x * G, nt = min(G, ntiles - t0);
    chain_stage_heads(jb, hd, t0, nt);
    __syncthreads();
    if (threadIdx.x < kPathHead) {
        ChainState s{t0 * kPathTile + threadIdx.x, 0u, 0u, 0u};
        chain_walk_group<false>(jb, hd, t0, nt, s, nullptr, nullptr);
        gfn[(size_t)blockIdx.x * kPathHead + threadIdx.x] = make_uint4(s.e, s.base, s.done, s.tail);
    }
}

__global__ void __launch_bounds__(1024) k_path_chain2(JobBufs jb, uint32_t ntiles, uint32_t G, const uint4 *gfn, uint32_t *mark_list,
                                                        uint32_t *mark_cnt)
{
    extern __shared__ __align__(16) uint8_t smem[];
    uint2 *hd = reinterpret_cast<uint2 *>(smem);
    uint4 *sg = reinterpret_cast<uint4 *>(smem + (size_t)G * kPathHead * 8);
    uint32_t *c_entry = reinterpret_cast<uint32_t *>(sg + (size_t)blockIdx.x * kPathHead), *c_base = c_entry + G;
    __shared__ ChainState s_st;
    __shared__ uint32_t s_j;
    const uint32_t g = blockIdx.x;
    for (uint32_t i = threadIdx.x; i < g * kPathHead; i += blockDim.x) sg[i] = gfn[i];
    if (threadIdx.x == 0) { s_st = ChainState{jb.start, 0u, jb.tail_start == 0 ? 1u : 0u, jb.start}; s_j = 0; }
    __syncthreads();
    for (;;) {
        if (threadIdx.x == 0) {
            ChainState s = s_st;
            uint32_t j = s_j;
            for (; j < g; j++) {
                const uint32_t gbeg = j * G * kPathTile;
                if (s.done || s.e >= jb.tail_start || s.e - gbeg >= G * kPathTile) continue;
                if (s.e - gbeg >= kPathHead) break;
                const uint4 f = sg[j * kPathHead + (s.e - gbeg)];
                s.e = f.x; s.base += f.y;
                if (f.z) { s.done = 1; s.tail = f.w; }
            }
            s_st = s; s_j = j;
        }
        __syncthreads();
        const uint32_t j = s_j;
        if (j >= g) break;
        chain_stage_heads(jb, hd, j * G, G);
        __syncthreads();
        if (threadIdx.x == 0) {
            ChainState s = s_st;
            chain_walk_group<false>(jb, hd, j * G, G, s, nullptr, nullptr);
            s_st = s; s_j = j + 1;
        }
        __syncthreads();
    }
    const uint32_t t0 = g * G, nt = min(G, ntiles - t0);
    chain_stage_heads(jb, hd, t0, nt);
    __syncthreads();
    if (threadIdx.x == 0) {
        ChainState s = s_st;
        chain_walk_group<true>(jb, hd, t0, nt, s, c_entry, c_base);
        if (g == gridDim.x - 1) {
            uint32_t tail_entry = s.tail;
            if (!s.done) { tail_entry = s.e; if (s.e < jb.tail_start) atomicOr(&jb.info->error, 2u); }
            jb.info->tail_entry = tail_entry;
            jb.info->n_mid_syms = s.base;
        }
    }
    __syncthreads();
    for (uint32_t k = threadIdx.x; k < nt; k += blockDim.x) {
        const uint32_t t = t0 + k;
        jb.tile_symbase[t] = c_base[k];
        const bool mn = (jb.tile_entry[t] != c_entry[k]) || path_tile_dirty(jb, t);
        jb.mark_needed[t] = mn;
        jb.tile_entry[t] = c_entry[k];
        if (mn) mark_list[atomicAdd(mark_cnt, 1u)] = t;
    }
}

__global__ void __launch_bounds__(1024) k_path_mark(JobBufs jb, const uint32_t *list, const uint32_t *list_cnt)
{
    extern __shared__ __align__(16) uint8_t smem[];
    uint32_t *nx = reinterpret_cast<uint32_t *>(smem);
    uint32_t *ex = nx + kPathTile;
    uint32_t *cn = ex + kPathTile;
    __shared__ uint32_t sub_entry[kPathTile / kPathSub], sub_base[kPathTile / kPathSub];
    constexpr uint32_t nsub = kPathTile / kPathSub;
    const uint32_t count = list ? *list_cnt : gridDim.x;
    for (uint32_t b = blockIdx.x; b < count; b += gridDim.x) {
        const uint32_t tile = list ? list[b] : b;
        const uint32_t tbeg = tile * kPathTile;
        if (!jb.mark_needed[tile]) continue;
        const uint32_t entry = jb.tile_entry[tile];
        if (threadIdx.x < nsub) jb.long_cnt[tile * nsub + threadIdx.x] = 0;
        if (entry == 0xffffffffu) {
            for (uint32_t i = threadIdx.x; i < kPathTile; i += blockDim.x)
                if (tbeg + i < jb.tail_start) jb.symidx[tbeg + i] = 0;
            continue;
        }
        __syncthreads();
        path_load(jb, tbeg, nx);
        __syncthreads();
        const uint32_t warp = threadIdx.x >> 5, lane = threadIdx.x & 31;
        for (uint32_t s = warp; s < nsub; s += blockDim.x / 32) path_subtile(nx, ex, cn, s * kPathSub, (s + 1) * kPathSub, lane);
        __syncthreads();
        if (threadIdx.x == 0) {
            uint32_t cur = entry - tbeg, cbase = 0;
            for (uint32_t j = 0; j < nsub; j++) {
                if (!(cur & kStuck) && cur < (j + 1) * kPathSub) {
                    sub_entry[j] = cur;
                    sub_base[j] = cbase;
                    cbase += cn[cur];
                    cur = ex[cur];
                } else sub_entry[j] = 0xffffffffu;
            }
        }
        __syncthreads();
        for (uint32_t i = threadIdx.x; i < kPathTile; i += blockDim.x) ex[i] = 0;
        __syncthreads();
        if (threadIdx.x < nsub) {
            const uint32_t s = threadIdx.x;
            uint32_t p = sub_entry[s];
            if (p != 0xffffffffu) {
                uint32_t idx = sub_base[s], nlong = 0;
                const uint32_t s1 = (s + 1) * kPathSub;
                uint32_t *ll = jb.long_list + (size_t)(tile * nsub + s) * kLongPerSub;
                while (p < s1) {
                    const uint32_t v = nx[p];
                    if (v & kNxtTail) break;
                    if (v & kNxtLong) {
                        if (nlong < kLongPerSub) ll[nlong++] = tbeg + p;
                        else atomicOr(&jb.info->error, 32u);
                    }
                    ex[p] = idx + 1;
                    idx += (v >> 16) & 0xffu;
                    p += v & 0xffffu;
                }
                jb.long_cnt[tile * nsub + s] = nlong;
            }
        }
        __syncthreads();
        for (uint32_t i = threadIdx.x; i < kPathTile; i += blockDim.x)
            if (tbeg + i < jb.tail_start) jb.symidx[tbeg + i] = ex[i];
    }
}

__global__ void __launch_bounds__(256) k_holes(JobBufs jb, uint32_t nlists)
{
    const uint32_t t = blockIdx.x * blockDim.x + threadIdx.x;
    {
        const uint32_t nthr = gridDim.x * blockDim.x;
        for (uint32_t i = t; i < jb.nmt; i += nthr) jb.tile_dirty[i] = 0;
        for (uint32_t i = t; i < jb.nmt * 512; i += nthr) reinterpret_cast<uint4 *>(jb.bucket_map)[i] = make_uint4(0, 0, 0, 0);
        for (uint32_t i = t; i < (jb.N >> 10) + 16; i += nthr) jb.hcoarse[i] = 0;
        for (uint32_t i = t; i < (jb.N >> 8) + 16; i += nthr) reinterpret_cast<uint32_t *>(jb.mchg)[i] = 0;
        if (t == 0) jb.info->holes_changed = 0;
    }
    const uint32_t list = t / kLongPerSub, slot = t % kLongPerSub;
    if (list >= nlists || slot >= jb.long_cnt[list]) return;
    const uint32_t p = jb.long_list[(size_t)list * kLongPerSub + slot];
    const uint32_t v = jb.nxt[p], delta = v & 0xffffu;
    const uint32_t len = jb.lp.early_exit ? delta : ((v & kNxtLong258) ? 258u : 257u);
    const uint32_t pos = p + delta - len;
    uint32_t y0 = pos + 1, y1 = pos + len - 1;
    uint32_t *hn = jb.holes_new;
    while (y0 < y1) {
        const uint32_t w = y0 >> 5, lo = y0 & 31;
        const uint32_t n = min(32u - lo, y1 - y0);
        const uint32_t mask = (n == 32 ? 0xffffffffu : ((1u << n) - 1u)) << lo;
        atomicOr(&hn[w], mask);
        y0 += n;
    }
}

__global__ void __launch_bounds__(256) k_emit(JobBufs jb)
{
    const uint32_t p = blockIdx.x * blockDim.x + threadIdx.x;
    if (p >= jb.tail_start) return;
    const uint32_t idx = jb.symidx[p];
    if (!idx) return;
    GAcc a{jb.in, jb.N, jb.L, jb.holes, jb.M, jb.wsize};
    uint32_t k = jb.tile_symbase[p / kPathTile] + idx - 1, ns = 0;
    Sym *syms = jb.syms;
    auto put = [&](const Sym &s) { syms[k++] = s; };
    if (jb.wsize == kWSize) macro_step(a, p, jb.lp, jb.tail_start, put, &ns);
    else macro_step(a, p, jb.lp, jb.tail_start, put, &ns, DynWin{jb.wsize});
}

__global__ void __launch_bounds__(256) k_holes_cmp(JobBufs jb, uint32_t nwords, uint32_t nmtiles)
{
    __shared__ uint32_t sb[2048];
    const uint32_t w = blockIdx.x * blockDim.x + threadIdx.x;
    uint32_t a = 0, b = 0;
    if (w < nwords) { a = jb.holes[w]; b = jb.holes_new[w]; }
    const bool changed = a != b;
    if (!__syncthreads_or(changed)) {
        if (w < nwords) { jb.hdiff[w] = 0; jb.hdiff[jb.hdiff_words + w] = 0; jb.holes_new[w] = 0; }
        return;
    }
    for (uint32_t i = threadIdx.x; i < 2048; i += blockDim.x) sb[i] = 0;
    __syncthreads();
    if (w < nwords) {
        jb.hdiff[w] = b & ~a;
        jb.hdiff[jb.hdiff_words + w] = a & ~b;
        if (changed) {
            jb.hcoarse[w >> 5] = 1;
            const uint32_t t = (w * 32) / kMatchTile;
            jb.info->holes_changed = 1u;
            jb.tile_dirty[t] = 1;
            if (t + 1 < nmtiles) jb.tile_dirty[t + 1] = 1;
            jb.holes[w] = b;
            uint32_t diff = a ^ b;
            while (diff) {
                const uint32_t y = w * 32 + (__ffs(diff) - 1);
                diff &= diff - 1;
                if (y + 4 <= jb.N) {
                    const uint8_t *q = jb.in + y;
                    const uint32_t h = hash_u32((uint32_t)q[0] | ((uint32_t)q[1] << 8) | ((uint32_t)q[2] << 16) | ((uint32_t)q[3] << 24));
                    atomicOr(&sb[h >> 5], 1u << (h & 31));
                }
            }
        }
        jb.holes_new[w] = 0;
    }
    __syncthreads();
    uint32_t *bm = jb.bucket_map + (size_t)((blockIdx.x * blockDim.x * 32) / kMatchTile) * 2048;
    for (uint32_t i = threadIdx.x; i < 2048; i += blockDim.x) if (sb[i]) atomicOr(&bm[i], sb[i]);
}

__global__ void __launch_bounds__(1024) k_iter_lists(JobBufs jb, uint32_t *skip_list, uint32_t *path_list, uint32_t npt)
{
    __shared__ uint32_t s_wsum[32], s_total, s_first;
    const uint32_t tid = threadIdx.x, lane = tid & 31, warp = tid >> 5;
    if (tid == 0) s_first = 0xffffffffu;
    uint32_t base = 0;
    for (int which = 0; which < 2; which++) {
        const uint32_t n = which ? npt : jb.nmt;
        uint32_t *out = which ? path_list : skip_list;
        base = 0;
        for (uint32_t c0 = 0; c0 < n; c0 += 1024) {
            const uint32_t i = c0 + tid;
            const bool d = i < n && (which ? path_tile_dirty(jb, i) : jb.tile_dirty[i] != 0);
            const uint32_t m = __ballot_sync(0xffffffffu, d);
            __syncthreads();
            if (lane == 0) s_wsum[warp] = __popc(m);
            __syncthreads();
            if (warp == 0) {
                const uint32_t v = s_wsum[lane];
                uint32_t incl = v;
#pragma unroll
                for (int k = 1; k < 32; k <<= 1) { const uint32_t t = __shfl_up_sync(0xffffffffu, incl, k); if (lane >= (uint32_t)k) incl += t; }
                s_wsum[lane] = incl - v;
                if (lane == 31) s_total = incl;
            }
            __syncthreads();
            if (d) {
                out[base + s_wsum[warp] + __popc(m & ((1u << lane) - 1u))] = i;
                if (which) atomicMin(&s_first, i);
            }
            base += s_total;
        }
        __syncthreads();
        if (tid == 0) {
            if (which) { jb.info->n_ptiles = base; jb.info->first_ptile = s_first == 0xffffffffu ? 0u : s_first; }
            else jb.info->n_dirty = base;
        }
        if (tid == 0 && base == 0) out[0] = 0;
    }
}

struct GAccW {
    GAcc g;
    uint32_t w;
    __device__ __forceinline__ uint32_t byte(uint32_t y) const
    {
        while (y >= g.N) {
            if (y < 2 * w) return 0;
            y -= w;
        }
        return g.data[y];
    }
    __device__ __forceinline__ uint32_t link(uint32_t y) const { return g.link(y); }
    __device__ __forceinline__ bool inserted(uint32_t y) const { return g.inserted(y); }
};

__global__ void __launch_bounds__(32) k_tail(JobBufs jb)
{
    __shared__ uint32_t ins[1024];
    if (threadIdx.x != 0) return;
    GAcc a{jb.in, jb.N, jb.L, jb.holes, jb.M, jb.wsize};
    const uint32_t p0 = max(jb.info->tail_entry, jb.start);
    const uint32_t n_mid = jb.info->n_mid_syms;
    uint32_t k = 0;
    Sym *syms = jb.syms + n_mid;
    uint32_t *sb = jb.sym_base;
    if (jb.N - p0 > 1024u * 32u - 64u) { atomicOr(&jb.info->error, 4u); return; }
    auto emit = [&](const Sym &s, uint32_t B) {
        syms[k] = s;
        sb[k] = B;
        k++;
    };
    uint32_t fb;
    if (jb.wsize == kWSize) fb = serial_medium(a, jb.N, p0, ins, 1024u, jb.lp, emit);
    else fb = serial_medium(GAccW{a, jb.wsize}, jb.N, p0, ins, 1024u, jb.lp, emit, DynWin{jb.wsize});
    jb.info->n_syms = n_mid + k;
    jb.info->final_base = fb;
    jb.info->n_blocks = (n_mid + k) / jb.block_syms + 1;
}

__device__ __forceinline__ uint32_t sym_end(const Sym &s) { return s.pos + (s.dist ? (uint32_t)s.lc + 3u : 1u); }

__global__ void __launch_bounds__(256) k_block_hist(JobBufs jb, uint32_t *freq )
{
    __shared__ uint32_t lf[kLCodes], df[kDCodes];
    const uint32_t b = blockIdx.x;
    const uint32_t nsyms = jb.info->n_syms, nblocks = jb.info->n_blocks;
    for (uint32_t i = threadIdx.x; i < kLCodes; i += blockDim.x) lf[i] = 0;
    if (threadIdx.x < kDCodes) df[threadIdx.x] = 0;
    __syncthreads();
    const uint32_t begin = b * jb.block_syms;
    const uint32_t count = (b + 1 < nblocks) ? jb.block_syms : nsyms - begin;
    for (uint32_t i = threadIdx.x; i < count; i += blockDim.x) {
        const Sym s = jb.syms[begin + i];
        if (s.dist == 0) atomicAdd(&lf[s.lc], 1u);
        else {
            atomicAdd(&lf[257 + c_tab.length_code[s.lc]], 1u);
            atomicAdd(&df[d_code(c_tab, s.dist - 1u)], 1u);
        }
    }
    __syncthreads();
    for (uint32_t i = threadIdx.x; i < kLCodes; i += blockDim.x) freq[b * 320 + i] = lf[i];
    if (threadIdx.x < kDCodes) freq[b * 320 + kLCodes + threadIdx.x] = df[threadIdx.x];
    if (threadIdx.x == 0) {
        BlockDesc &bd = jb.blocks[b];
        const bool last = b + 1 == nblocks;
        bd.sym_begin = begin;
        bd.sym_count = count;
        bd.last = last && !jb.not_last;
        const uint32_t start = begin == 0 ? jb.start : sym_end(jb.syms[begin - 1]);
        const uint32_t end = last ? jb.N : sym_end(jb.syms[begin + count - 1]);
        bd.in_start = start;
        bd.in_len = end - start;
        uint32_t Bf;
        if (last) Bf = jb.info->final_base;
        else {
            const uint32_t li = begin + count - 1, n_mid = jb.info->n_mid_syms;
            if (jb.serial_mode) {
                Bf = jb.serial_mode == 2 ? jb.block_base[b] : 0;
            } else if (jb.huffman_only) {
                const uint32_t q = jb.syms[li].pos, w = jb.wsize;
                Bf = q < 2 * w ? 0 : w * (1 + (q - 2 * w) / w);
            } else if (jb.slow_mode == 2) {
                Bf = base_at(jb.syms[li].pos, jb.N, jb.wsize);
            } else if (jb.slow_mode) {
                Bf = base_at(jb.syms[li].pos + 1, jb.N, jb.wsize);
            } else Bf = li < n_mid ? wbase_w(DynWin{jb.wsize}, jb.syms[li].pos) : jb.sym_base[li - n_mid];
        }
        bd.have_window = start >= Bf;
    }
}

__device__ __forceinline__ uint32_t brev_bits(uint32_t code, uint32_t len) { return __brev(code) >> (32u - len); }

template <int KIND>
__device__ __forceinline__ uint32_t xbits_of(uint32_t n) { return KIND == 0 ? (n >= 257 ? extra_lbits(n - 257) : 0u) : KIND == 1 ? extra_dbits(n) : extra_blbits(n); }

template <int KIND>
__device__ int build_tree_warp(TreeScratch &s, TreeState &st, CtData *tree, uint32_t *sh_cnt )
{
    constexpr int elems = KIND == 0 ? kLCodes : KIND == 1 ? kDCodes : kBlCodes;
    constexpr int max_length = KIND == 2 ? kMaxBlBits : kMaxBits;
    const uint32_t lane = threadIdx.x & 31;
    int heap_len = 0, max_code = -1;
    for (int b0 = 0; b0 < elems; b0 += 32) {
        const int n = b0 + (int)lane;
        const bool nz = n < elems && tree[n].fc != 0;
        const uint32_t m = __ballot_sync(0xffffffffu, nz);
        if (nz) { s.heap[heap_len + 1 + __popc(m & ((1u << lane) - 1u))] = (uint32_t)n; s.depth[n] = 0; }
        else if (n < elems) tree[n].dl = 0;
        heap_len += __popc(m);
        if (m) max_code = b0 + 31 - __clz(m);
    }
    __syncwarp();
    if (heap_len < 2) {
        if (lane == 0) {
            while (heap_len < 2) {
                const int node = max_code < 2 ? ++max_code : 0;
                s.heap[++heap_len] = (uint32_t)node;
                tree[node].fc = 1;
                s.depth[node] = 0;
                st.opt_len--;
                if (KIND == 0) st.static_len -= c_tab.sl_len[node];
                else if (KIND == 1) st.static_len -= 5;
            }
        }
        heap_len = 2;
        max_code = __shfl_sync(0xffffffffu, max_code, 0);
        __syncwarp();
    }
    for (int n = 1 + (int)lane; n <= heap_len; n += 32) s.hk[n] = heap_entry(tree, s.depth, s.heap[n]);
    __syncwarp();
    for (int lvl = 31 - __clz(heap_len / 2); lvl >= 0; lvl--) {
        const int first = 1 << lvl, last = min((2 << lvl) - 1, heap_len / 2);
        for (int k = first + (int)lane; k <= last; k += 32) pqdownheap(s, heap_len, k);
        __syncwarp();
    }
    int heap_max = kHeapSize;
    if (lane == 0) {
        int node = elems;
        do {
            const int n = (int)(s.hk[1] & 0xffffu);
            s.hk[1] = s.hk[heap_len--];
            pqdownheap(s, heap_len, 1);
            const int m = (int)(s.hk[1] & 0xffffu);
            s.heap[--heap_max] = (uint32_t)n;
            s.heap[--heap_max] = (uint32_t)m;
            tree[node].fc = (uint16_t)(tree[n].fc + tree[m].fc);
            s.depth[node] = (uint8_t)((s.depth[n] >= s.depth[m] ? s.depth[n] : s.depth[m]) + 1);
            tree[n].dl = tree[m].dl = (uint16_t)node;
            s.hk[1] = heap_entry(tree, s.depth, (uint32_t)node);
            node++;
            pqdownheap(s, heap_len, 1);
        } while (heap_len >= 2);
        s.heap[--heap_max] = (uint32_t)(s.hk[1] & 0xffffu);
        int overflow = 0;
        tree[s.heap[heap_max]].dl = 0;
        for (int h = heap_max + 1; h < kHeapSize; h++) {
            const int n = (int)s.heap[h];
            int bits = tree[tree[n].dl].dl + 1;
            if (bits > max_length) { bits = max_length; overflow++; }
            tree[n].dl = (uint16_t)bits;
        }
        sh_cnt[0] = (uint32_t)overflow;
    }
    heap_max = __shfl_sync(0xffffffffu, heap_max, 0);
    __syncwarp();
    const int overflow = (int)sh_cnt[0];
    __syncwarp();
    if (lane < 16) sh_cnt[lane] = 0;
    __syncwarp();
    uint64_t opt = 0, stat = 0;
    for (int n = (int)lane; n <= max_code; n += 32) {
        const uint32_t bits = tree[n].dl;
        if (tree[n].fc == 0 || bits == 0) continue;
        atomicAdd(&sh_cnt[bits], 1u);
        const uint32_t xb = xbits_of<KIND>((uint32_t)n);
        const uint64_t f = tree[n].fc;
        opt += f * (uint64_t)(bits + xb);
        if (KIND == 0) stat += f * (uint64_t)(c_tab.sl_len[n] + xb);
        else if (KIND == 1) stat += f * (uint64_t)(5 + xb);
    }
#pragma unroll
    for (int d = 16; d >= 1; d >>= 1) { opt += __shfl_xor_sync(0xffffffffu, opt, d); stat += __shfl_xor_sync(0xffffffffu, stat, d); }
    __syncwarp();
    if (lane == 0) {
        st.opt_len += opt;
        st.static_len += stat;
        if (overflow > 0) {
            int ov = overflow, bits;
            do {
                bits = max_length - 1;
                while (sh_cnt[bits] == 0) bits--;
                sh_cnt[bits]--;
                sh_cnt[bits + 1] += 2;
                sh_cnt[max_length]--;
                ov -= 2;
            } while (ov > 0);
            int h = kHeapSize;
            for (bits = max_length; bits != 0; bits--) {
                int n = (int)sh_cnt[bits];
                while (n != 0) {
                    const int m = (int)s.heap[--h];
                    if (m > max_code) continue;
                    if (tree[m].dl != (uint16_t)bits) {
                        st.opt_len += (uint64_t)bits * tree[m].fc;
                        st.opt_len -= (uint64_t)tree[m].dl * tree[m].fc;
                        tree[m].dl = (uint16_t)bits;
                    }
                    n--;
                }
            }
        }
    }
    __syncwarp();
    uint32_t nc = 0;
    {
        uint32_t code = 0;
        for (uint32_t b = 1; b <= (uint32_t)kMaxBits; b++) { code = (code + sh_cnt[b - 1]) << 1; if (b == lane) nc = code; }
    }
    for (int b0 = 0; b0 <= max_code; b0 += 32) {
        const int n = b0 + (int)lane;
        const uint32_t len = n <= max_code ? tree[n].dl : 0u;
        const uint32_t same = __match_any_sync(0xffffffffu, len);
        const uint32_t rank = __popc(same & ((1u << lane) - 1u));
        const uint32_t base = __shfl_sync(0xffffffffu, nc, len & 31u);
        if (len) tree[n].fc = (uint16_t)brev_bits(base + rank, len);
#pragma unroll 1
        for (uint32_t l = 1; l <= (uint32_t)kMaxBits; l++) {
            const uint32_t cnt = __popc(__ballot_sync(0xffffffffu, len == l));
            if (lane == l) nc += cnt;
        }
    }
    __syncwarp();
    return max_code;
}

struct WordSink {
    uint8_t *buf;
    uint32_t nbits;
    __device__ __forceinline__ void put(uint32_t val, uint32_t len)
    {
        const uint32_t byte = nbits >> 3, sh = nbits & 7u;
        const uint32_t v = (val & ((1u << len) - 1u)) << sh;
        if (sh == 0) buf[byte] = (uint8_t)v; else buf[byte] |= (uint8_t)v;
        if (sh + len > 8) { buf[byte + 1] = (uint8_t)(v >> 8); if (sh + len > 16) buf[byte + 2] = (uint8_t)(v >> 16); }
        nbits += len;
    }
};

__device__ void send_tree_fast(WordSink &o, const CtData *bltree, const CtData *tree, int max_code)
{
    int prevlen = -1, curlen, nextlen = tree[0].dl, count = 0, max_count = 7, min_count = 4;
    if (nextlen == 0) { max_count = 138; min_count = 3; }
    for (int n = 0; n <= max_code; n++) {
        curlen = nextlen;
        nextlen = tree[n + 1].dl;
        if (++count < max_count && curlen == nextlen) continue;
        else if (count < min_count) { do { o.put(bltree[curlen].fc, bltree[curlen].dl); } while (--count != 0); }
        else if (curlen != 0) {
            if (curlen != prevlen) { o.put(bltree[curlen].fc, bltree[curlen].dl); count--; }
            o.put(bltree[16].fc, bltree[16].dl);
            o.put((uint32_t)(count - 3), 2);
        } else if (count <= 10) {
            o.put(bltree[17].fc, bltree[17].dl);
            o.put((uint32_t)(count - 3), 3);
        } else {
            o.put(bltree[18].fc, bltree[18].dl);
            o.put((uint32_t)(count - 11), 7);
        }
        count = 0;
        prevlen = curlen;
        if (nextlen == 0) { max_count = 138; min_count = 3; }
        else if (curlen == nextlen) { max_count = 6; min_count = 3; }
        else { max_count = 7; min_count = 4; }
    }
}

__device__ void build_block_warp(TreeScratch &s, BlockDesc &b, const uint32_t *lfreq, const uint32_t *dfreq, bool have_window,
                                 bool strategy_fixed, uint32_t *sh_cnt, TreeState *sh_st)
{
    const uint32_t lane = threadIdx.x & 31;
    uint64_t opt_lenb = 0, static_lenb = 0;
    int max_blindex = 0, lmax = 0, dmax = 0;
    TreeState &st = *sh_st;
    if (lane == 0) { st = TreeState{0, 0}; b.data_type = 2; b.no_eob = 0; }
    __syncwarp();
    if (b.sym_count == 0) {
        if (lane == 0) st.static_len = 7;
    } else {
        {
            bool black = false, white = false;
            for (uint32_t n = lane; n < 256; n += 32) {
                if (lfreq[n] == 0) continue;
                if (n < 32 && ((0xf3ffc07fu >> n) & 1u)) black = true;
                if (n == 9 || n == 10 || n == 13 || n >= 32) white = true;
            }
            const bool ab = __any_sync(0xffffffffu, black), aw = __any_sync(0xffffffffu, white);
            if (lane == 0) b.data_type = ab ? 0u : aw ? 1u : 0u;
        }
        for (int n = (int)lane; n < kHeapSize; n += 32) s.ltree[n] = CtData{(uint16_t)(n < kLCodes ? lfreq[n] : 0), 0};
        for (int n = (int)lane; n < 2 * kDCodes + 1; n += 32) s.dtree[n] = CtData{(uint16_t)(n < kDCodes ? dfreq[n] : 0), 0};
        for (int n = (int)lane; n < 2 * kBlCodes + 1; n += 32) s.bltree[n] = CtData{0, 0};
        __syncwarp();
        if (lane == 0) s.ltree[kEndBlock].fc = 1;
        __syncwarp();
        lmax = build_tree_warp<0>(s, st, s.ltree, sh_cnt);
        dmax = build_tree_warp<1>(s, st, s.dtree, sh_cnt);
        if (lane == 0) {
            scan_tree(s.bltree, s.ltree, lmax);
            scan_tree(s.bltree, s.dtree, dmax);
        }
        __syncwarp();
        build_tree_warp<2>(s, st, s.bltree, sh_cnt);
        for (max_blindex = kBlCodes - 1; max_blindex >= 3; max_blindex--)
            if (s.bltree[bl_order(max_blindex)].dl != 0) break;
        if (lane == 0) st.opt_len += 3 * ((uint64_t)max_blindex + 1) + 5 + 5 + 4;
        __syncwarp();
        opt_lenb = (st.opt_len + 3 + 7) >> 3;
        static_lenb = (st.static_len + 3 + 7) >> 3;
        if (static_lenb <= opt_lenb || strategy_fixed) opt_lenb = static_lenb;
    }
    __syncwarp();
    if ((uint64_t)b.in_len + 4 <= opt_lenb && have_window) {
        if (lane == 0) { b.type = 0; b.hdr[0] = (uint8_t)b.last; b.hdr_bits = 3; b.body_bits = 0; }
    } else if (static_lenb == opt_lenb) {
        if (lane == 0) { b.type = 1; b.hdr[0] = (uint8_t)(2 | b.last); b.hdr_bits = 3; b.body_bits = st.static_len; }
        for (int n = (int)lane; n < kLCodes; n += 32) { b.lcode[n] = c_tab.sl_code[n]; b.llen[n] = c_tab.sl_len[n]; }
        if (lane < (uint32_t)kDCodes) { b.dcode[lane] = c_tab.sd_code[lane]; b.dlen[lane] = 5; }
    } else {
        if (lane == 0) {
            b.type = 2;
            WordSink o{b.hdr, 0};
            o.put(4 | b.last, 3);
            const int lcodes = lmax + 1, dcodes = dmax + 1, blcodes = max_blindex + 1;
            o.put((uint32_t)(lcodes - 257), 5);
            o.put((uint32_t)(dcodes - 1), 5);
            o.put((uint32_t)(blcodes - 4), 4);
            for (int r = 0; r < blcodes; r++) o.put(s.bltree[bl_order(r)].dl, 3);
            send_tree_fast(o, s.bltree, s.ltree, lcodes - 1);
            send_tree_fast(o, s.bltree, s.dtree, dcodes - 1);
            b.hdr_bits = o.nbits;
            b.body_bits = 3 + st.opt_len - o.nbits;
        }
        for (int n = (int)lane; n < kLCodes; n += 32) { b.lcode[n] = n <= lmax ? s.ltree[n].fc : 0; b.llen[n] = n <= lmax ? (uint8_t)s.ltree[n].dl : 0; }
        if (lane < (uint32_t)kDCodes) { b.dcode[lane] = (int)lane <= dmax ? s.dtree[lane].fc : 0; b.dlen[lane] = (int)lane <= dmax ? (uint8_t)s.dtree[lane].dl : 0; }
    }
    __syncwarp();
}

__global__ void __launch_bounds__(32) k_build_blocks(JobBufs jb, const uint32_t *freq)
{
    __shared__ TreeScratch s;
    __shared__ BlockDesc bd;
    __shared__ uint32_t fr[320];
    __shared__ uint32_t sh_cnt[16];
    __shared__ TreeState sh_st;
    const uint32_t b = blockIdx.x;
    if (b >= jb.info->n_blocks) return;
    for (uint32_t i = threadIdx.x; i < 320; i += 32) fr[i] = freq[b * 320 + i];
    for (uint32_t i = threadIdx.x; i < sizeof(BlockDesc) / 4; i += 32)
        reinterpret_cast<uint32_t *>(&bd)[i] = reinterpret_cast<const uint32_t *>(&jb.blocks[b])[i];
    __syncwarp();
    if (jb.serial_mode == 1) {
        if (threadIdx.x == 0) build_quick_piece(c_tab, bd, fr, fr + kLCodes, b == 0, b + 1 == jb.info->n_blocks, jb.not_last == 0);
    } else build_block_warp(s, bd, fr, fr + kLCodes, bd.have_window != 0, jb.strategy_fixed != 0, sh_cnt, &sh_st);
    __syncwarp();
    for (uint32_t i = threadIdx.x; i < sizeof(BlockDesc) / 4; i += 32)
        reinterpret_cast<uint32_t *>(&jb.blocks[b])[i] = reinterpret_cast<const uint32_t *>(&bd)[i];
}

__device__ __forceinline__ void or_bits(uint32_t *out32, uint64_t pos, uint64_t val, uint32_t n)
{
    if (n == 0) return;
    const uint64_t w = pos >> 5;
    const uint32_t sh = (uint32_t)(pos & 31);
    atomicOr(&out32[w], (uint32_t)(val << sh));
    if (sh + n > 32) {
        atomicOr(&out32[w + 1], (uint32_t)(val >> (32 - sh)));
        if (sh + n > 64) atomicOr(&out32[w + 2], (uint32_t)(val >> (64 - sh)));
    }
}

constexpr uint32_t kScanChunk = 1024;
__global__ void __launch_bounds__(256) k_scan_blocks(JobBufs jb)
{
    __shared__ uint64_t s_bits[kScanChunk];
    __shared__ uint64_t s_base[kScanChunk];
    __shared__ uint64_t s_bit;
    const uint32_t nb = jb.info->n_blocks;
    if (threadIdx.x == 0) s_bit = 8ull * jb.hdr_len + jb.prime_bits;
    for (uint32_t c0 = 0; c0 < nb; c0 += kScanChunk) {
        const uint32_t nc = min(kScanChunk, nb - c0);
        for (uint32_t i = threadIdx.x; i < nc; i += blockDim.x) {
            const BlockDesc &bd = jb.blocks[c0 + i];
            s_bits[i] = bd.type == 0 ? (1ull << 63) | (uint16_t)bd.in_len : (uint64_t)bd.hdr_bits + bd.body_bits;
        }
        __syncthreads();
        if (threadIdx.x == 0) {
            uint64_t bit = s_bit;
            for (uint32_t i = 0; i < nc; i++) {
                s_base[i] = bit;
                const uint64_t v = s_bits[i];
                bit = (v >> 63) ? ((bit + 3 + 7) & ~7ull) + 32 + 8ull * (v & 0xffffu) : bit + v;
            }
            s_bit = bit;
        }
        __syncthreads();
        for (uint32_t i = threadIdx.x; i < nc; i += blockDim.x) jb.blocks[c0 + i].bit_base = s_base[i];
        __syncthreads();
    }
    if (threadIdx.x != 0) return;
    uint64_t bit = s_bit;
    if (jb.not_last && jb.end_mode == 0) {
        const uint64_t p = (bit + 3 + 7) & ~7ull;
        jb.info->marker_byte = p >> 3;
        bit = p + 32;
    } else if (jb.not_last && jb.end_mode == 1) {
        or_bits(reinterpret_cast<uint32_t *>(jb.out), bit, 2u, 10);
        bit += 10;
    }
    jb.info->total_bits = bit;
    const uint64_t bytes = (jb.not_last && jb.end_mode ? (bit >> 3) : ((bit + 7) >> 3)) + (jb.wrap == 1 ? 4 : jb.wrap == 2 ? 8 : 0);
    jb.info->out_bytes = bytes;
    jb.info->data_type = jb.blocks[0].sym_count ? jb.blocks[0].data_type : 2u;
    if (bytes > jb.out_cap) { atomicOr(&jb.info->error, 8u); return; }
    if (jb.wrap == 1) {
        const uint32_t lf = (jb.huffman_only || jb.strategy_fixed || jb.level < 2) ? 0 : jb.level < 6 ? 1 : jb.level == 6 ? 2 : 3;
        uint32_t h = ((8u + (jb.cinfo << 4)) << 8) | (lf << 6);
        h += 31 - (h % 31);
        jb.out[0] = (uint8_t)(h >> 8);
        jb.out[1] = (uint8_t)h;
    } else if (jb.wrap == 2) {
        const uint8_t g[10] = {31, 139, 8, 0, 0, 0, 0, 0, (uint8_t)jb.xfl, 3};
        for (int i = 0; i < 10; i++) jb.out[i] = g[i];
    }
}

__global__ void __launch_bounds__(1024) k_encode(JobBufs jb)
{
    __shared__ HuffTables st;
    __shared__ uint16_t s_lcode[kLCodes], s_dcode[kDCodes];
    __shared__ uint8_t s_llen[kLCodes], s_dlen[kDCodes];
    __shared__ uint64_t warp_sum[32];
    if (jb.info->error) return;
    const BlockDesc &bd = jb.blocks[blockIdx.x];
    uint32_t *out32 = reinterpret_cast<uint32_t *>(jb.out);
    const uint32_t tid = threadIdx.x;
    if (bd.type == 0) {
        const uint64_t p = ((bd.bit_base + 3 + 7) >> 3);
        const uint32_t sl = (uint16_t)bd.in_len;
        if (tid == 0) {
            or_bits(out32, bd.bit_base, bd.hdr[0] & 7u, 3);
            jb.out[p] = (uint8_t)sl;
            jb.out[p + 1] = (uint8_t)(sl >> 8);
            jb.out[p + 2] = (uint8_t)~sl;
            jb.out[p + 3] = (uint8_t)((~sl) >> 8);
        }
        for (uint32_t i = tid; i < sl; i += blockDim.x) jb.out[p + 4 + i] = jb.in[bd.in_start + i];
        return;
    }
    for (uint32_t i = tid; i < sizeof(HuffTables) / 4; i += blockDim.x)
        reinterpret_cast<uint32_t *>(&st)[i] = reinterpret_cast<const uint32_t *>(&c_tab)[i];
    for (uint32_t i = tid; i < kLCodes; i += blockDim.x) { s_lcode[i] = bd.lcode[i]; s_llen[i] = bd.llen[i]; }
    if (tid < kDCodes) { s_dcode[tid] = bd.dcode[tid]; s_dlen[tid] = bd.dlen[tid]; }
    __syncthreads();
    for (uint32_t wi = tid; wi * 32 < bd.hdr_bits; wi += blockDim.x) {
        uint32_t v = bd.hdr[wi * 4] | (bd.hdr[wi * 4 + 1] << 8) | (bd.hdr[wi * 4 + 2] << 16) | ((uint32_t)bd.hdr[wi * 4 + 3] << 24);
        const uint32_t n = min(32u, bd.hdr_bits - wi * 32);
        if (n < 32) v &= (1u << n) - 1u;
        or_bits(out32, bd.bit_base + wi * 32ull, v, n);
    }
    const uint32_t total = bd.sym_count + (bd.no_eob ? 0u : 1u);
    const uint32_t lane = tid & 31, warp = tid >> 5;
    uint64_t round_bits = 0;
    for (uint32_t rb = 0; rb == 0 || rb < total; rb += blockDim.x * kSymsPerThread) {
        const uint32_t first = rb + tid * kSymsPerThread;
        uint64_t vals[kSymsPerThread];
        uint8_t lens[kSymsPerThread];
        uint32_t mybits = 0;
#pragma unroll
        for (uint32_t j = 0; j < kSymsPerThread; j++) {
            const uint32_t i = first + j;
            uint64_t v = 0;
            uint32_t n = 0;
            if (i < bd.sym_count) {
                const Sym s = jb.syms[bd.sym_begin + i];
                if (s.dist == 0) { v = s_lcode[s.lc]; n = s_llen[s.lc]; }
                else {
                    uint32_t code = st.length_code[s.lc];
                    v = s_lcode[code + 257];
                    n = s_llen[code + 257];
                    uint32_t extra = extra_lbits(code);
                    if (extra) { v |= (uint64_t)(s.lc - st.base_length[code]) << n; n += extra; }
                    const uint32_t d = s.dist - 1u;
                    code = st.dist_code[d < 256 ? d : 256 + (d >> 7)];
                    uint64_t dv = s_dcode[code];
                    uint32_t dn = s_dlen[code];
                    extra = extra_dbits(code);
                    if (extra) { dv |= (uint64_t)(d - st.base_dist[code]) << dn; dn += extra; }
                    v |= dv << n;
                    n += dn;
                }
            } else if (i + 1 == total && !bd.no_eob) { v = s_lcode[kEndBlock]; n = s_llen[kEndBlock]; }
            vals[j] = v;
            lens[j] = (uint8_t)n;
            mybits += n;
        }
        uint64_t incl = mybits;
#pragma unroll
        for (int o = 1; o < 32; o <<= 1) {
            const uint64_t t = __shfl_up_sync(0xffffffffu, incl, o);
            if ((int)lane >= o) incl += t;
        }
        if (lane == 31) warp_sum[warp] = incl;
        __syncthreads();
        if (warp == 0) {
            uint64_t ws = warp_sum[lane];
#pragma unroll
            for (int o = 1; o < 32; o <<= 1) {
                const uint64_t t = __shfl_up_sync(0xffffffffu, ws, o);
                if ((int)lane >= o) ws += t;
            }
            warp_sum[lane] = ws;
        }
        __syncthreads();
        uint64_t pos = bd.bit_base + bd.hdr_bits + round_bits + (incl - mybits) + (warp ? warp_sum[warp - 1] : 0);
#pragma unroll
        for (uint32_t j = 0; j < kSymsPerThread; j++) {
            or_bits(out32, pos, vals[j], lens[j]);
            pos += lens[j];
        }
        round_bits += warp_sum[31];
        __syncthreads();
    }
    if (tid == blockDim.x - 1 && round_bits != bd.body_bits) atomicOr(&jb.info->error, 16u);
}

__global__ void k_finish(JobBufs jb, const uint32_t *check)
{
    if (threadIdx.x != 0 || blockIdx.x != 0) return;
    if (jb.info->error) return;
    const uint64_t p = (jb.info->total_bits + 7) >> 3;
    const uint32_t a = *check;
    if (jb.not_last && jb.end_mode == 0) { jb.out[jb.info->marker_byte + 2] = 0xff; jb.out[jb.info->marker_byte + 3] = 0xff; }
    if (jb.wrap == 1) {
        jb.out[p] = (uint8_t)(a >> 24);
        jb.out[p + 1] = (uint8_t)(a >> 16);
        jb.out[p + 2] = (uint8_t)(a >> 8);
        jb.out[p + 3] = (uint8_t)a;
    } else if (jb.wrap == 2) {
        for (int i = 0; i < 4; i++) jb.out[p + i] = (uint8_t)(a >> (8 * i));
        for (int i = 0; i < 4; i++) jb.out[p + 4 + i] = (uint8_t)((jb.N - jb.start) >> (8 * i));
    }
    jb.info->adler = a;
}

__global__ void __launch_bounds__(256) k_literal_syms(JobBufs jb)
{
    const uint32_t p = blockIdx.x * blockDim.x + threadIdx.x;
    const uint32_t n = jb.N - jb.start;
    if (p == 0) {
        jb.info->n_mid_syms = n;
        jb.info->n_syms = n;
        jb.info->n_blocks = n / jb.block_syms + 1;
        const uint32_t w = jb.wsize, q = jb.N ? jb.N - 1 : 0;
        uint32_t B = q < 2 * w ? 0 : w * (1 + (q - 2 * w) / w);
        if (jb.N - B >= 2 * w - kMinLookahead) B += w;
        jb.info->final_base = B;
    }
    if (p < n) jb.syms[p] = Sym{0, jb.in[jb.start + p], jb.start + p};
}

__global__ void __launch_bounds__(256) k_stored(JobBufs jb)
{
    const uint32_t N = jb.N - jb.start;
    const uint32_t nb = N == 0 ? 1 : (N + 65534) / 65535;
    const uint32_t b = blockIdx.x;
    if (b >= nb) return;
    const uint32_t start = b * 65535u;
    const uint32_t len = min(65535u, N - start);
    uint8_t *o = jb.out + jb.hdr_len + (uint64_t)b * (65535u + 5u);
    if (threadIdx.x == 0) {
        o[0] = b + 1 == nb ? 1 : 0;
        o[1] = (uint8_t)len;
        o[2] = (uint8_t)(len >> 8);
        o[3] = (uint8_t)~len;
        o[4] = (uint8_t)((~len) >> 8);
        if (b == 0) {
            jb.info->total_bits = 8ull * (jb.hdr_len + (uint64_t)N + 5ull * nb);
            jb.info->out_bytes = jb.hdr_len + (uint64_t)N + 5ull * nb + (jb.wrap == 1 ? 4 : jb.wrap == 2 ? 8 : 0);
            jb.info->data_type = 2;
            if (jb.wrap == 1) {
                uint32_t h = (8u + (jb.cinfo << 4)) << 8;
                h += 31 - (h % 31);
                jb.out[0] = (uint8_t)(h >> 8);
                jb.out[1] = (uint8_t)h;
            }
            else if (jb.wrap == 2) {
                const uint8_t g[10] = {31, 139, 8, 0, 0, 0, 0, 0, 4, 3};
                for (int i = 0; i < 10; i++) jb.out[i] = g[i];
            }
        }
    }
    for (uint32_t i = threadIdx.x; i < len; i += blockDim.x) o[5 + i] = jb.in[jb.start + start + i];
}

__global__ void __launch_bounds__(256) k_links_dict_ghost(JobBufs jb, uint32_t *first)
{
    const uint32_t s = jb.start;
    if (s < 3 || s >= jb.N) return;
    const uint8_t *d = jb.in;
    const uint32_t g = s - 3;
    const uint32_t k0 = hash_u32((uint32_t)d[g] | ((uint32_t)d[g + 1] << 8) | ((uint32_t)d[g + 2] << 16));
    const uint32_t kt = hash_u32((uint32_t)d[g] | ((uint32_t)d[g + 1] << 8) | ((uint32_t)d[g + 2] << 16) | ((uint32_t)d[g + 3] << 24));
    if (k0 == kt) return;
    const uint32_t x = g + 1 + blockIdx.x * blockDim.x + threadIdx.x;
    if (x > g + kMaxDist || x + 4 > jb.N) return;
    const uint32_t kx = hash_u32((uint32_t)d[x] | ((uint32_t)d[x + 1] << 8) | ((uint32_t)d[x + 2] << 16) | ((uint32_t)d[x + 3] << 24));
    if (kx == k0) atomicMin(first, x);
}
__global__ void k_links_dict_ghost_apply(JobBufs jb, const uint32_t *first)
{
    if (threadIdx.x != 0 || blockIdx.x != 0) return;
    const uint32_t x = *first;
    if (x != 0xffffffffu) jb.L[x] = (uint16_t)(x - (jb.start - 3));
}

}
```

### zlib_rs_b200/csrc/zb_kernels.cuh

```cuda
#pragma once
#include <cuda_runtime.h>
#include "zb_core.h"
#include "zb_huff.h"
#include "zb_slow.h"

namespace zb {

constexpr uint32_t kLinkTile = 32768;
constexpr uint32_t kMatchTile = 32768;
constexpr uint32_t kMatchSub = 8192;
constexpr uint32_t kPathTile = 16384;
constexpr uint32_t kPathSub = 256;
constexpr uint32_t kLongPerSub = 4;
constexpr uint32_t kPathHead = 64;
constexpr uint32_t kChainChunkTiles = 320;
constexpr uint32_t kNxtTail = 0x80000000u;
constexpr uint32_t kNxtLong = 0x40000000u;
constexpr uint32_t kNxtLong258 = 0x20000000u;
constexpr uint32_t kSymsPerThread = 16;
constexpr uint32_t kSlowAhead = 1024;

__device__ __forceinline__ uint32_t sld_u8(uint32_t a) { uint32_t v; asm volatile("ld.shared.u8 %0, [%1];" : "=r"(v) : "r"(a)); return v; }
__device__ __forceinline__ uint32_t sld_u16(uint32_t a) { uint32_t v; asm volatile("ld.shared.u16 %0, [%1];" : "=r"(v) : "r"(a)); return v; }
__device__ __forceinline__ uint32_t sld_u32(uint32_t a) { uint32_t v; asm volatile("ld.shared.u32 %0, [%1];" : "=r"(v) : "r"(a)); return v; }
__device__ __forceinline__ uint32_t sld_u32u(uint32_t a)
{
    const uint32_t al = a & ~3u;
    return __funnelshift_r(sld_u32(al), sld_u32(al + 4), (a & 3u) * 8u);
}

struct JobInfo {
    uint32_t n_mid_syms;
    uint32_t tail_entry;
    uint32_t n_syms;
    uint32_t final_base;
    uint32_t holes_changed;
    uint32_t n_dirty, n_ptiles, first_ptile;
    uint32_t n_blocks;
    uint32_t data_type;
    uint32_t error;
    uint64_t total_bits;
    uint64_t out_bytes;
    uint32_t adler;
    uint64_t marker_byte;
    unsigned long long dbg[3];
};

struct JobBufs {
    const uint8_t *in;
    uint32_t N;
    uint32_t start;
    uint32_t tail_start;
    uint16_t *L;
    uint16_t *SK;
    uint32_t *hdiff;
    uint32_t hdiff_words;
    uint8_t *hcoarse;
    uint8_t *mchg;
    uint32_t *holes;
    uint32_t *holes_new;
    uint32_t *M;
    uint32_t *nxt;
    uint32_t *pexit;
    uint32_t *pcnt;
    uint2 *phead;
    uint32_t *symidx;
    uint32_t *tile_entry;
    uint32_t *tile_symbase;
    uint8_t *tile_dirty;
    Sym *syms;
    uint32_t *sym_base;
    BlockDesc *blocks;
    TreeScratch *scratch;
    uint8_t *out;
    uint64_t out_cap;
    JobInfo *info;
    LevelParams lp;
    uint32_t level;
    uint32_t strategy_fixed;
    uint32_t wrap;
    uint32_t hdr_len;
    uint32_t xfl;
    uint32_t huffman_only;
    uint32_t match_sub;
    uint32_t nmt;
    uint8_t *mark_needed;
    uint32_t *long_list;
    uint32_t *long_cnt;
    SlowParams sp;
    uint32_t slow_mode;
    uint16_t *link_last;
    uint16_t *Lr;
    uint16_t *keys;
    const uint32_t *skip_list;
    const uint32_t *nxt_list;
    uint4 *chain_state;
    uint32_t *bucket_map;
    uint32_t use_bucket_map;
    uint32_t not_last;
    uint32_t end_mode;
    uint32_t prime_bits;
    uint32_t block_syms;
    uint32_t serial_mode;
    uint32_t *block_base;
    uint32_t wsize;
    uint32_t cinfo;
};

cudaError_t upload_tables();
int device_sm_count();
cudaError_t launch_adler32(const uint8_t *d_buf, uint64_t len, uint32_t start, void *d_scratch, size_t scratch_bytes, uint32_t *d_out,
                           cudaStream_t st);
cudaError_t launch_crc32(const uint8_t *d_buf, uint64_t len, uint32_t start, void *d_scratch, size_t scratch_bytes, uint32_t *d_out,
                         cudaStream_t st);

}
```

Measured before the change: 1.608.

## Replace dense rematch of dirty tiles with sparse redo-list matching kernel

On later hole iterations, the dense k_match over all sub-tiles is replaced by a two-stage scheme. k_redo_list filters positions whose previous match could be affected by hash-diff changes and compacts them into work items. A persistent k_match_sparse then processes those items with dynamic scheduling over smaller 4 KB pieces. The aim is to avoid re-matching unchanged positions, at the cost of extra list-building kernels and reliance on the conservative redo predicate being correct. It also adds per-iteration profiling and a debug cross-check path.

After: 1.643, median of 6. +2.2%, better.

```diff
diff --git a/__graft_entry__.py b/__graft_entry__.py
--- a/__graft_entry__.py
+++ b/__graft_entry__.py
@@ -13,6 +13,7 @@
     subprocess.check_call(["make", "-C", os.path.join(ROOT, "oracle")])
     subprocess.check_call(["make", "-C", os.path.join(ROOT, "oracle"), "ref"])
     subprocess.check_call(["make", "-C", os.path.join(ROOT, "tests", "hostmodel")])
+    subprocess.check_call(["make", "-C", os.path.join(ROOT, "tests", "sparse_model")])
     import zlib_rs_b200
     zlib_rs_b200.lib()
 
diff --git a/include/zb_engine.h b/include/zb_engine.h
--- a/include/zb_engine.h
+++ b/include/zb_engine.h
@@ -91,6 +91,20 @@
 ZB_API void zb_engine_set_profile(zb_engine *e, int on);
 ZB_API int zb_engine_get_profile(zb_engine *e, float *ms, uint32_t *launches, int n);
 
+typedef struct zb_iter_profile {
+    uint32_t iteration;
+    uint32_t dirty_tiles;
+    float skip_ms;
+    float match_ms;
+    float nxt_ms, path_ms;
+    float holes_ms;
+    uint64_t ctas;
+    uint64_t windows;
+    uint64_t walked;
+    uint64_t mismatches;
+} zb_iter_profile;
+ZB_API int zb_engine_get_iter_profile(zb_engine *e, zb_iter_profile *out, int n);
+
 ZB_API void *zb_device_alloc(zb_engine *e, size_t bytes);
 ZB_API void zb_device_free(zb_engine *e, void *p);
 ZB_API int zb_copy_to_device(zb_engine *e, void *dst, const void *src, size_t bytes);
diff --git a/zlib_rs_b200/__init__.py b/zlib_rs_b200/__init__.py
--- a/zlib_rs_b200/__init__.py
+++ b/zlib_rs_b200/__init__.py
@@ -28,6 +28,12 @@
                 ("iterations", ctypes.c_uint32), ("n_symbols", ctypes.c_uint32), ("n_blocks", ctypes.c_uint32),
                 ("gpu_launches", ctypes.c_uint32), ("exact_parity", ctypes.c_int32), ("gpu_ms", ctypes.c_float),
                 ("bits_used", ctypes.c_uint32), ("carry", ctypes.c_uint32)]
+
+
+class IterProfile(ctypes.Structure):
+    _fields_ = [("iteration", ctypes.c_uint32), ("dirty_tiles", ctypes.c_uint32), ("skip_ms", ctypes.c_float),
+                ("match_ms", ctypes.c_float), ("nxt_ms", ctypes.c_float), ("path_ms", ctypes.c_float), ("holes_ms", ctypes.c_float),
+                ("ctas", ctypes.c_uint64), ("windows", ctypes.c_uint64), ("walked", ctypes.c_uint64), ("mismatches", ctypes.c_uint64)]
 
 
 class InflateResult(ctypes.Structure):
@@ -95,6 +101,8 @@
         L.zb_crc32.argtypes = [vp, u32, vp, sz, ci, ctypes.POINTER(u32), ctypes.POINTER(ctypes.c_float)]
         L.zb_engine_set_profile.argtypes = [vp, ci]
         L.zb_engine_get_profile.argtypes = [vp, ctypes.POINTER(ctypes.c_float), ctypes.POINTER(u32), ci]
+        if hasattr(L, "zb_engine_get_iter_profile"):
+            L.zb_engine_get_iter_profile.argtypes = [vp, ctypes.POINTER(IterProfile), ci]
         L.zb_device_alloc.argtypes, L.zb_device_alloc.restype = [vp, sz], vp
         L.zb_device_free.argtypes = [vp, vp]
         L.zb_copy_to_device.argtypes = [vp, vp, vp, sz]
@@ -363,5 +371,11 @@
         k = lib().zb_engine_get_profile(self.h, ms, ln, 12)
         return {self.PHASES[i]: {"ms": ms[i], "launches": ln[i]} for i in range(min(k, len(self.PHASES)))}
 
+    def get_iter_profile(self):
+        n = lib().zb_engine_get_iter_profile(self.h, None, 0)
+        arr = (IterProfile * max(n, 1))()
+        lib().zb_engine_get_iter_profile(self.h, arr, n)
+        return [{f: getattr(arr[i], f) for f, _ in IterProfile._fields_} for i in range(n)]
+
     def fill_random(self, dptr, n, seed=42):
         self._check(lib().zb_device_fill_random(self.h, dptr, n, seed))
diff --git a/zlib_rs_b200/csrc/zb_engine.cu b/zlib_rs_b200/csrc/zb_engine.cu
--- a/zlib_rs_b200/csrc/zb_engine.cu
+++ b/zlib_rs_b200/csrc/zb_engine.cu
@@ -12,6 +12,7 @@
 constexpr uint32_t kSlowSub9 = 24576;
 constexpr uint32_t kTailTiles = 2;
 constexpr uint32_t kTailSub = 512;
+constexpr uint32_t kRedoItemWide = 1024, kRedoItemNarrow = 256, kRedoNarrowTiles = 16;
 
 thread_local char g_err[256] = "";
 
@@ -28,6 +29,9 @@
 
 __global__ void k_match(JobBufs);
 __global__ void k_skip(JobBufs);
+__global__ void k_redo_list(JobBufs);
+__global__ void k_match_sparse(JobBufs);
+__global__ void k_match_check(JobBufs, const uint32_t *);
 __global__ void k_nxt(JobBufs);
 __global__ void k_path_tiles(JobBufs);
 __global__ void k_path_chain(JobBufs, uint32_t, uint32_t);
@@ -58,7 +62,8 @@
 __global__ void k_links_dict_ghost(JobBufs, uint32_t *);
 __global__ void k_links_dict_ghost_apply(JobBufs, const uint32_t *);
 
-constexpr uint32_t kMatchSmemBytes = (kWSize + kMatchSub + 512) + (kWSize + kMatchSub) * 2 + ((kWSize + kMatchSub) / 32 + 1) * 4 * 4 + 8192;
+constexpr uint32_t kMatchSmemBytes = (kWSize + kMatchSub + 512) + (kWSize + kMatchSub) * 2 + 8192;
+constexpr uint32_t kSparseSmemBytes = (kWSize + kRedoPiece + 512) + (kWSize + kRedoPiece) * 2;
 constexpr uint32_t kPathSmemBytes = kPathTile * 4 * 3;
 constexpr uint32_t kLinks2SmemBytes = 65536 * 2 + kLinkTile * 2 + kLinkTile + 64 + 2048;
 constexpr uint32_t kSkipSmemBytes = 2 * kWSize * 2 + 2 * (2 * kWSize / 32) * 4 + 8192 + 64;
@@ -90,6 +95,7 @@
     CK(cudaEventCreate(&ev1));
     CK(upload_tables());
     CK(cudaFuncSetAttribute(k_match, cudaFuncAttributeMaxDynamicSharedMemorySize, kMatchSmemBytes));
+    CK(cudaFuncSetAttribute(k_match_sparse, cudaFuncAttributeMaxDynamicSharedMemorySize, kSparseSmemBytes));
     CK(cudaFuncSetAttribute(k_skip, cudaFuncAttributeMaxDynamicSharedMemorySize, kSkipSmemBytes));
     CK(cudaFuncSetAttribute(k_links2_std, cudaFuncAttributeMaxDynamicSharedMemorySize, kLinks2SmemBytes));
     CK(cudaFuncSetAttribute(k_links2_roll, cudaFuncAttributeMaxDynamicSharedMemorySize, kLinks2SmemBytes));
@@ -133,15 +139,16 @@
     cudaEventRecord(pev0, st);
 }
 
-void Engine::pend(int phase, uint32_t nlaunch)
-{
-    if (!profile) return;
+float Engine::pend(int phase, uint32_t nlaunch)
+{
+    if (!profile) return 0.f;
     cudaEventRecord(pev1, st);
     cudaEventSynchronize(pev1);
     float ms = 0;
     cudaEventElapsedTime(&ms, pev0, pev1);
     phase_ms[phase] += ms;
     phase_launches[phase] += nlaunch;
+    return ms;
 }
 
 int Engine::reserve(int slot, size_t bytes, void **out)
@@ -172,7 +179,7 @@
 }
 
 enum { S_IN, S_L, S_HOLES, S_HOLESN, S_M, S_NXT, S_PEXIT, S_PCNT, S_SYMIDX, S_TENTRY, S_TSYMB, S_TDIRTY, S_SYMS, S_SYMB,
-       S_BLOCKS, S_SCRATCH, S_FREQ, S_OUT, S_CK, S_INF0, S_INF1, S_PHEAD, S_SK, S_MARKN, S_LLIST, S_LCNT, S_BMAP, S_HDIFF, S_HCOARSE, S_CSTATE, S_LISTS, S_LR, S_LLAST, S_BBASE, S_MCHG, S_GFN, S_KEYS, S_COUNT };
+       S_BLOCKS, S_SCRATCH, S_FREQ, S_OUT, S_CK, S_INF0, S_INF1, S_PHEAD, S_SK, S_MARKN, S_LLIST, S_LCNT, S_BMAP, S_HDIFF, S_HCOARSE, S_CSTATE, S_LISTS, S_LR, S_LLAST, S_BBASE, S_MCHG, S_GFN, S_KEYS, S_REDO, S_ITEMS, S_DBG, S_COUNT };
 static_assert(S_COUNT <= Engine::kSlots, "slots");
 
 size_t deflate_bound(size_t n)
@@ -285,6 +292,8 @@
     d_lists = static_cast<uint32_t *>(p);
     RES(S_HDIFF, (size_t)nwords * 8, hdiff, uint32_t *)
     jb.hdiff_words = nwords;
+    RES(S_REDO, ((size_t)N + kMatchTile) * 4, redo_pos, uint32_t *)
+    RES(S_ITEMS, ((size_t)nmt * (kMatchTile / kRedoItemNarrow) + 4) * 16, redo_items, uint4 *)
     RES(S_HCOARSE, (size_t)(N >> 10) + 16, hcoarse, uint8_t *)
     RES(S_MCHG, (((size_t)N >> 8) + 16) * 4 + 64, mchg, uint8_t *)
     RES(S_BLOCKS, (size_t)max_blocks * sizeof(BlockDesc), blocks, BlockDesc *)
@@ -355,7 +364,8 @@
     if (lf_zero && !jb.strategy_fixed && !jb.huffman_only) jb.level = 1;
 
     CK(cudaEventRecord(ev0, st));
-    if (profile) { for (int i = 0; i < kPhases; i++) { phase_ms[i] = 0; phase_launches[i] = 0; } }
+    if (profile) { for (int i = 0; i < kPhases; i++) { phase_ms[i] = 0; phase_launches[i] = 0; } iter_prof.clear(); }
+    jb.debug = getenv("ZB_DEBUG") ? 1u : 0u;
     uint32_t up_chunks = 0;
     size_t up_len[kUpChunks] = {0};
     const bool chunked_upload = !src_dev && !dstart && n_in >= ((size_t)4 << 20) && level != 0 && !jb.huffman_only &&
@@ -480,6 +490,7 @@
             } else {
             if (jb.tail_start > 0) {
                 uint32_t n_dirty = nmt;
+                unsigned long long dbg_last[kDbgCounters] = {0};
                 for (;;) {
                     iters++;
                     uint32_t mthreads = 1024;
@@ -491,6 +502,10 @@
                     }
                     uint32_t nsub = (N + jb.match_sub - 1) / jb.match_sub;
                     uint32_t n_ptiles = npt, first_ptile = 0;
+                    zb_iter_profile ip;
+                    memset(&ip, 0, sizeof ip);
+                    ip.iteration = iters;
+                    ip.dirty_tiles = n_dirty;
                     jb.skip_list = nullptr;
                     jb.nxt_list = nullptr;
                     if (iters > 1) {
@@ -502,44 +517,72 @@
                         if (n_dirty) {
                             pbegin();
                             k_skip<<<n_dirty, 1024, kSkipSmemBytes, st>>>(jb);
-                            pend(1, 1);
+                            ip.skip_ms = pend(1, 1);
                             launches++;
                         }
                     }
-                    const uint32_t msmem = (kWSize + jb.match_sub + 512) + (kWSize + jb.match_sub) * 2 +
-                                           (iters > 1 ? ((kWSize + jb.match_sub) / 32 + 1) * 4 * 4 + 8192 : 64);
                     jb.use_bucket_map = iters > 1;
-                    pbegin();
-                    k_match<<<nsub, mthreads, msmem, st>>>(jb);
-                    pend(1, 1);
+                    if (iters > 1 && !jb.lp.early_exit) {
+                        jb.redo_item = n_dirty <= kRedoNarrowTiles ? kRedoItemNarrow : kRedoItemWide;
+                        pbegin();
+                        if (n_dirty) k_redo_list<<<n_dirty * (kMatchTile / kRedoPiece), 1024, 0, st>>>(jb);
+                        k_match_sparse<<<2 * device_sm_count(), 1024, kSparseSmemBytes, st>>>(jb);
+                        ip.match_ms = pend(1, 2);
+                        launches++;
+                        if (jb.debug && n_dirty) {
+                            if ((rc = reserve(S_DBG, (size_t)N * 6 + 64, &p)) != ZB_OK) return rc;
+                            uint32_t *m_sparse = static_cast<uint32_t *>(p);
+                            uint16_t *sk_sparse = reinterpret_cast<uint16_t *>(m_sparse + N);
+                            CK(cudaMemcpyAsync(m_sparse, jb.M, (size_t)N * 4, cudaMemcpyDeviceToDevice, st));
+                            CK(cudaMemcpyAsync(sk_sparse, jb.SK, (size_t)N * 2, cudaMemcpyDeviceToDevice, st));
+                            JobBufs jc = jb;
+                            jc.debug = 0;
+                            jc.use_bucket_map = 0;
+                            jc.match_sub = 4096;
+                            k_match<<<n_dirty * (kMatchTile / 4096), 1024, (kWSize + 4096 + 512) + (kWSize + 4096) * 2 + 64, st>>>(jc);
+                            k_match_check<<<n_dirty, 256, 0, st>>>(jb, m_sparse);
+                            CK(cudaMemcpyAsync(jb.M, m_sparse, (size_t)N * 4, cudaMemcpyDeviceToDevice, st));
+                            CK(cudaMemcpyAsync(jb.SK, sk_sparse, (size_t)N * 2, cudaMemcpyDeviceToDevice, st));
+                        }
+                    } else {
+                        const uint32_t msmem = (kWSize + jb.match_sub + 512) + (kWSize + jb.match_sub) * 2 + (iters > 1 ? 8192 : 64);
+                        pbegin();
+                        k_match<<<nsub, mthreads, msmem, st>>>(jb);
+                        ip.match_ms = pend(1, 1);
+                    }
                     if (profile && iters == 1) phase_ms[11] = phase_ms[1];
                     pbegin();
                     k_nxt<<<n_ptiles * (kPathTile / 1024), 1024, 0, st>>>(jb);
-                    pend(2, 1);
+                    ip.nxt_ms = pend(2, 1);
                     pbegin();
                     k_path_tiles<<<n_ptiles, 1024, kPathSmemBytes, st>>>(jb);
                     launch_chain(first_ptile);
                     launch_mark(iters == 1 ? npt : 2 * n_ptiles + 16);
-                    pend(3, 3);
+                    ip.path_ms = pend(3, 3);
                     pbegin();
                     k_holes<<<(nlists * kLongPerSub + 255) / 256, 256, 0, st>>>(jb, nlists);
                     k_holes_cmp<<<(nwords + 255) / 256, 256, 0, st>>>(jb, nwords, nmt);
-                    pend(4, 2);
-                    launches += 7;
                     k_iter_lists<<<1, 1024, 0, st>>>(jb, d_lists, d_lists + nmt + 8, npt);
-                    launches++;
+                    ip.holes_ms = pend(4, 3);
+                    launches += 8;
                     CK(cudaMemcpyAsync(h_info, d_info, sizeof(JobInfo), cudaMemcpyDeviceToHost, st));
                     CK(cudaStreamSynchronize(st));
                     if (h_info->error) { snprintf(g_err, sizeof g_err, "engine error flags 0x%x (parse)", h_info->error); return ZB_E_INTERNAL; }
-                    if (getenv("ZB_DEBUG")) {
-                        static unsigned long long last[3];
-                        if (iters == 1) memset(last, 0, sizeof last);
-                        const double ctas = (double)(h_info->dbg[0] - last[0]) + 1e-9;
-                        fprintf(stderr, "iter %u dirty %u: ctas %llu stage %.1f walk %.1f kcyc/cta, holes_changed %u\n", iters, n_dirty,
-                                h_info->dbg[0] - last[0], (h_info->dbg[1] - last[1]) / 1e3 / ctas, (h_info->dbg[2] - last[2]) / 1e3 / ctas,
-                                h_info->holes_changed);
-                        memcpy(last, h_info->dbg, sizeof last);
+                    if (jb.debug) {
+                        unsigned long long prev[kDbgCounters];
+                        memcpy(prev, dbg_last, sizeof prev);
+                        memcpy(dbg_last, h_info->dbg, sizeof dbg_last);
+                        ip.ctas = dbg_last[kDbgCtas] - prev[kDbgCtas];
+                        ip.windows = dbg_last[kDbgWindows] - prev[kDbgWindows];
+                        ip.walked = dbg_last[kDbgWalked] - prev[kDbgWalked];
+                        ip.mismatches = dbg_last[kDbgMismatch] - prev[kDbgMismatch];
+                        const double w = (double)ip.windows + 1e-9;
+                        fprintf(stderr, "iter %u dirty %u: ctas %llu windows %llu walked %llu stage %.1f walk %.1f kcyc/window, "
+                                "mismatches %llu, holes_changed %u\n", iters, n_dirty, (unsigned long long)ip.ctas,
+                                (unsigned long long)ip.windows, (unsigned long long)ip.walked, (dbg_last[kDbgStage] - prev[kDbgStage]) / 1e3 / w,
+                                (dbg_last[kDbgWalk] - prev[kDbgWalk]) / 1e3 / w, (unsigned long long)ip.mismatches, h_info->holes_changed);
                     }
+                    if (profile) iter_prof.push_back(ip);
                     if (!h_info->holes_changed) break;
                     n_dirty = h_info->n_dirty;
                     if (iters > N / 257u + 4096u) { snprintf(g_err, sizeof g_err, "hole iteration did not converge"); return ZB_E_INTERNAL; }
@@ -740,6 +783,14 @@
 
 void zb_engine_set_profile(zb_engine *z, int on) { if (z) z->e.profile = on != 0; }
 
+int zb_engine_get_iter_profile(zb_engine *z, zb_iter_profile *out, int n)
+{
+    if (!z) return 0;
+    const int k = n < (int)z->e.iter_prof.size() ? n : (int)z->e.iter_prof.size();
+    for (int i = 0; i < k; i++) out[i] = z->e.iter_prof[i];
+    return (int)z->e.iter_prof.size();
+}
+
 int zb_engine_get_profile(zb_engine *z, float *ms, uint32_t *launches, int n)
 {
     if (!z) return 0;
diff --git a/zlib_rs_b200/csrc/zb_engine_internal.h b/zlib_rs_b200/csrc/zb_engine_internal.h
--- a/zlib_rs_b200/csrc/zb_engine_internal.h
+++ b/zlib_rs_b200/csrc/zb_engine_internal.h
@@ -2,6 +2,7 @@
 #include <cuda_runtime.h>
 #include <stddef.h>
 #include <stdint.h>
+#include <vector>
 #include "../../include/zb_engine.h"
 #include "zb_kernels.cuh"
 
@@ -34,7 +35,8 @@
     uint32_t phase_launches[kPhases] = {0};
     cudaEvent_t pev0 = nullptr, pev1 = nullptr;
     void pbegin();
-    void pend(int phase, uint32_t nlaunch);
+    float pend(int phase, uint32_t nlaunch);
+    std::vector<zb_iter_profile> iter_prof;
 
     int init(int dev);
     int inflate_init();
diff --git a/zlib_rs_b200/csrc/zb_kernels.cu b/zlib_rs_b200/csrc/zb_kernels.cu
--- a/zlib_rs_b200/csrc/zb_kernels.cu
+++ b/zlib_rs_b200/csrc/zb_kernels.cu
@@ -289,17 +289,6 @@
 constexpr uint32_t kCoopCmp = 4;
 enum { LS_IDLE = 0, LS_WALK = 1, LS_PEND = 2, LS_DONE = 3, LS_FIN = 4 };
 
-struct DiffMaps {
-    const uint32_t *del, *pdel;
-    const uint32_t *add, *padd;
-    __device__ __forceinline__ static bool any(const uint32_t *b, const uint32_t *p, uint32_t lo, uint32_t hi)
-    {
-        const uint32_t c_hi = p[hi >> 5] + __popc(b[hi >> 5] & ((1u << (hi & 31)) - 1u));
-        const uint32_t c_lo = p[lo >> 5] + __popc(b[lo >> 5] & ((1u << (lo & 31)) - 1u));
-        return c_hi != c_lo;
-    }
-};
-
 __device__ __forceinline__ void sld_u64u(uint32_t a, uint32_t &lo, uint32_t &hi)
 {
     const uint32_t al = a & ~3u, sh = (a & 3u) * 8u;
@@ -308,10 +297,11 @@
     hi = __funnelshift_r(w1, w2, sh);
 }
 
-__device__ __forceinline__ void match_tile_fast(const JobBufs &jb, const uint8_t *sdata, const uint16_t *sL, const uint32_t *sbm,
-                                                const DiffMaps dm, uint32_t ws, uint32_t te, uint32_t *s_next)
-{
-    const bool filt = jb.use_bucket_map != 0;
+template <bool kSparse>
+__device__ __forceinline__ void match_tile_fast(const JobBufs &jb, const uint8_t *sdata, const uint16_t *sL, uint32_t ws, uint32_t end,
+                                                uint32_t *s_next)
+{
+    constexpr bool filt = kSparse;
     const uint32_t dbase = (uint32_t)__cvta_generic_to_shared(sdata);
     const uint32_t lbase = (uint32_t)__cvta_generic_to_shared(sL);
     const uint32_t N = jb.N, nice = jb.lp.nice, budget = jb.lp.chain;
@@ -446,32 +436,14 @@
             if (lane == leader) base = atomicAdd(s_next, (uint32_t)__popc(m_idle));
             base = __shfl_sync(0xffffffffu, base, leader);
             if (state == LS_IDLE) {
-                const uint32_t x = base + __popc(m_idle & ((1u << lane) - 1u));
-                if (x >= te) state = LS_DONE;
-                else if (x + kMSafe > N) { jb.M[x] = 0; }
+                const uint32_t k = base + __popc(m_idle & ((1u << lane) - 1u));
+                const uint32_t x = kSparse && k < end ? jb.redo_pos[k] : k;
+                if (k >= end) state = LS_DONE;
+                else if (!kSparse && x + kMSafe > N) { jb.M[x] = 0; }
                 else {
                     xr = x - ws;
-                    bool skip = false;
-                    if (filt) {
-                        const uint32_t h = hash_u32(sld_u32u(dbase + xr));
-                        skip = !((sbm[h >> 5] >> (h & 31)) & 1u);
-                        if (!skip) {
-                            const uint32_t rdo = RDout[xr];
-                            const bool on_budget = rdo != 0xffffu && (rdo & 0x8000u);
-                            const uint32_t lo = rdo == 0xffffu ? (xr > md ? xr - md : 0u) : xr - (rdo & 0x7fffu);
-                            bool redo = DiffMaps::any(dm.del, dm.pdel, lo, xr);
-                            if (!redo) {
-                                if (on_budget) redo = DiffMaps::any(dm.add, dm.padd, lo, xr);
-                                else {
-                                    const uint32_t m = Mout[xr];
-                                    if (m) { const uint32_t h2 = xr - (m & 0xffffu); redo = (dm.add[h2 >> 5] >> (h2 & 31)) & 1u; }
-                                }
-                            }
-                            if (!redo) redo = sld_u16(lbase + 2 * xr) == md;
-                            skip = !redo;
-                        }
-                    }
-                    if (!skip) {
+                    if (kSparse && jb.debug) atomicAdd(&jb.info->dbg[kDbgWalked], 1ull);
+                    {
                         const uint32_t d0 = sld_u16(lbase + 2 * xr);
                         lowr = xr > md ? xr - md : 0;
                         if (ws == 0 && lowr == 0) lowr = 1;
@@ -495,6 +467,51 @@
     }
 }
 
+__device__ __forceinline__ void stage_window(const JobBufs &jb, uint8_t *sdata, uint16_t *sL, uint32_t ws, uint32_t te, uint32_t data_bytes,
+                                             unsigned long long *mbar, uint32_t parity)
+{
+    const uint32_t tid = threadIdx.x, nthr = blockDim.x;
+    uint32_t n16 = (te + 512 - ws + 15) / 16;
+    if (n16 > data_bytes / 16) n16 = data_bytes / 16;
+    const bool bulk = (reinterpret_cast<uintptr_t>(jb.in) & 15u) == 0;
+    const uint32_t mb = (uint32_t)__cvta_generic_to_shared(mbar);
+    if (bulk) {
+        if (tid == 0) {
+            const uint32_t dsts = (uint32_t)__cvta_generic_to_shared(sdata);
+            asm volatile("fence.proxy.async.shared::cta;" ::: "memory");
+            asm volatile("mbarrier.arrive.expect_tx.shared::cta.b64 _, [%0], %1;" ::"r"(mb), "r"(n16 * 16u) : "memory");
+            asm volatile("cp.async.bulk.shared::cluster.global.mbarrier::complete_tx::bytes [%0], [%1], %2, [%3];"
+                         ::"r"(dsts), "l"(jb.in + ws), "r"(n16 * 16u), "r"(mb) : "memory");
+        }
+    } else {
+        const uint4 *src = reinterpret_cast<const uint4 *>(jb.in + ws);
+        uint4 *dst = reinterpret_cast<uint4 *>(sdata);
+        for (uint32_t i = tid; i < n16; i += nthr) dst[i] = src[i];
+    }
+    const uint32_t nl = (te - ws + 7) / 8;
+    const uint4 *ls = reinterpret_cast<const uint4 *>(jb.Lr + ws);
+    uint4 *ld = reinterpret_cast<uint4 *>(sL);
+    for (uint32_t i = tid; i < nl; i += nthr) {
+        uint4 v = ls[i];
+        v.x |= __vcmpeq2(v.x, 0u); v.y |= __vcmpeq2(v.y, 0u); v.z |= __vcmpeq2(v.z, 0u); v.w |= __vcmpeq2(v.w, 0u);
+        ld[i] = v;
+    }
+    if (bulk) {
+        uint32_t done = 0;
+        while (!done) {
+            asm volatile("{\n.reg .pred p;\nmbarrier.try_wait.parity.shared::cta.b64 p, [%1], %2;\nselp.u32 %0, 1, 0, p;\n}"
+                         : "=r"(done) : "r"(mb), "r"(parity) : "memory");
+        }
+    }
+}
+
+__device__ __forceinline__ void mbar_init(unsigned long long *mbar)
+{
+    const uint32_t mb = (uint32_t)__cvta_generic_to_shared(mbar);
+    asm volatile("mbarrier.init.shared::cta.b64 [%0], 1;" ::"r"(mb) : "memory");
+    asm volatile("fence.proxy.async.shared::cta;" ::: "memory");
+}
+
 __global__ void __launch_bounds__(1024, 2) k_match(JobBufs jb)
 {
     extern __shared__ __align__(16) uint8_t smem[];
@@ -503,6 +520,7 @@
     const uint32_t sub = jb.match_sub;
     const uint32_t per_tile = kMatchTile / sub;
     const uint32_t ts = (jb.skip_list ? jb.skip_list[blockIdx.x / per_tile] * per_tile + blockIdx.x % per_tile : blockIdx.x) * sub;
+    if (jb.debug && threadIdx.x == 0 && !jb.lp.early_exit) atomicAdd(&jb.info->dbg[kDbgCtas], 1ull);
     if (ts >= jb.N) return;
     {
         const uint32_t t0 = ts / kMatchTile, t1 = (min(ts + sub, jb.N) - 1) / kMatchTile;
@@ -511,11 +529,7 @@
     const uint32_t data_bytes = kWSize + sub + 512;
     uint8_t *sdata = smem;
     uint16_t *sL = reinterpret_cast<uint16_t *>(smem + data_bytes);
-    uint32_t *sh = reinterpret_cast<uint32_t *>(smem + data_bytes + (kWSize + sub) * 2);
-    uint32_t *sbm = sh;
-    const uint32_t wmax = (kWSize + sub) / 32 + 1;
-    uint32_t *sdel = sbm + 2048, *pdel = sdel + wmax, *sadd = pdel + wmax, *padd = sadd + wmax;
-    __shared__ uint32_t s_wsum[32];
+    uint32_t *sbm = reinterpret_cast<uint32_t *>(smem + data_bytes + (kWSize + sub) * 2);
     const uint32_t N = jb.N;
     const uint32_t te = min(ts + sub, N);
     const uint32_t ws = ts >= kWSize ? ts - kWSize : 0;
@@ -528,94 +542,31 @@
             const uint8_t *q = jb.in + x;
             const uint32_t h = hash_u32((uint32_t)q[0] | ((uint32_t)q[1] << 8) | ((uint32_t)q[2] << 16) | ((uint32_t)q[3] << 24));
             if (((bm0[h >> 5] | bm1[h >> 5]) >> (h & 31)) & 1u) {
-                const uint32_t rd = jb.SK[x];
-                const uint32_t lo = rd == 0xffffu ? (x > jb.wsize - kMinLookahead ? x - (jb.wsize - kMinLookahead) : 0u) : x - (rd & 0x7fffu);
+                const uint32_t lo = x > jb.wsize - kMinLookahead ? x - (jb.wsize - kMinLookahead) : 0u;
                 for (uint32_t b = lo >> 10; b <= (x >> 10); b++) hit |= jb.hcoarse[b];
             }
         }
         if (!__syncthreads_or(hit)) return;
         for (uint32_t i = tid; i < 2048; i += nthr) sbm[i] = bm0[i] | bm1[i];
-        const uint32_t nwd = (te - ws + 31) / 32;
-        const uint32_t per = (nwd + 1 + nthr - 1) / nthr;
-        const uint32_t wb = tid * per;
-        const uint32_t lane_ = tid & 31, warp_ = tid >> 5;
-        for (int which = 0; which < 2; which++) {
-            const uint32_t *src = which ? jb.hdiff : jb.hdiff + jb.hdiff_words;
-            uint32_t *bits = which ? sadd : sdel, *pre = which ? padd : pdel;
-            uint32_t mine = 0;
-            for (uint32_t k = 0; k < per; k++) {
-                const uint32_t w = wb + k;
-                if (w <= nwd) { const uint32_t v = w < nwd ? src[(ws >> 5) + w] : 0u; bits[w] = v; mine += __popc(v); }
-            }
-            uint32_t incl = mine;
-#pragma unroll
-            for (int d = 1; d < 32; d <<= 1) {
-                const uint32_t t = __shfl_up_sync(0xffffffffu, incl, d);
-                if (lane_ >= (uint32_t)d) incl += t;
-            }
-            __syncthreads();
-            if (lane_ == 31) s_wsum[warp_] = incl;
-            __syncthreads();
-            uint32_t run = incl - mine;
-            for (uint32_t k = 0; k < warp_; k++) run += s_wsum[k];
-            for (uint32_t k = 0; k < per; k++) {
-                const uint32_t w = wb + k;
-                if (w <= nwd) { pre[w] = run; run += __popc(bits[w]); }
-            }
-        }
     }
     if (tid == 0) {
         s_next = ts;
-        const uint32_t mb = (uint32_t)__cvta_generic_to_shared(&s_mbar);
-        asm volatile("mbarrier.init.shared::cta.b64 [%0], 1;" ::"r"(mb) : "memory");
-        asm volatile("fence.proxy.async.shared::cta;" ::: "memory");
-    }
-    const long long t_0 = clock64();
-    __syncthreads();
-    {
-        uint32_t n16 = (te + 512 - ws + 15) / 16;
-        if (n16 > data_bytes / 16) n16 = data_bytes / 16;
-        const bool bulk = (reinterpret_cast<uintptr_t>(jb.in) & 15u) == 0;
-        if (bulk) {
-            if (tid == 0) {
-                const uint32_t mb = (uint32_t)__cvta_generic_to_shared(&s_mbar), dsts = (uint32_t)__cvta_generic_to_shared(sdata);
-                asm volatile("mbarrier.arrive.expect_tx.shared::cta.b64 _, [%0], %1;" ::"r"(mb), "r"(n16 * 16u) : "memory");
-                asm volatile("cp.async.bulk.shared::cluster.global.mbarrier::complete_tx::bytes [%0], [%1], %2, [%3];"
-                             ::"r"(dsts), "l"(jb.in + ws), "r"(n16 * 16u), "r"(mb) : "memory");
-            }
-        } else {
-            const uint4 *src = reinterpret_cast<const uint4 *>(jb.in + ws);
-            uint4 *dst = reinterpret_cast<uint4 *>(sdata);
-            for (uint32_t i = tid; i < n16; i += nthr) dst[i] = src[i];
-        }
-        const uint32_t nl = (te - ws + 7) / 8;
-        const uint4 *ls = reinterpret_cast<const uint4 *>(jb.Lr + ws);
-        uint4 *ld = reinterpret_cast<uint4 *>(sL);
-        for (uint32_t i = tid; i < nl; i += nthr) {
-            uint4 v = ls[i];
-            v.x |= __vcmpeq2(v.x, 0u); v.y |= __vcmpeq2(v.y, 0u); v.z |= __vcmpeq2(v.z, 0u); v.w |= __vcmpeq2(v.w, 0u);
-            ld[i] = v;
-        }
-        if (bulk) {
-            const uint32_t mb = (uint32_t)__cvta_generic_to_shared(&s_mbar);
-            uint32_t done = 0;
-            while (!done) {
-                asm volatile("{\n.reg .pred p;\nmbarrier.try_wait.parity.shared::cta.b64 p, [%1], 0;\nselp.u32 %0, 1, 0, p;\n}"
-                             : "=r"(done) : "r"(mb) : "memory");
-            }
-        }
-    }
-    __syncthreads();
-    const long long t_1 = clock64();
+        mbar_init(&s_mbar);
+    }
+    const uint32_t t_0 = (uint32_t)clock64();
+    __syncthreads();
+    stage_window(jb, sdata, sL, ws, te, data_bytes, &s_mbar, 0);
+    __syncthreads();
+    const uint32_t t_1 = (uint32_t)clock64();
     const LevelParams lp = jb.lp;
     if (!lp.early_exit) {
-        match_tile_fast(jb, sdata, sL, sbm, DiffMaps{sdel, pdel, sadd, padd}, ws, te, &s_next);
-        __syncthreads();
-        if (tid == 0) {
-            const long long t_2 = clock64();
-            atomicAdd(&jb.info->dbg[0], 1ull);
-            atomicAdd(&jb.info->dbg[1], (unsigned long long)(t_1 - t_0));
-            atomicAdd(&jb.info->dbg[2], (unsigned long long)(t_2 - t_1));
+        match_tile_fast<false>(jb, sdata, sL, ws, te, &s_next);
+        __syncthreads();
+        if (jb.debug && tid == 0) {
+            const uint32_t t_2 = (uint32_t)clock64();
+            atomicAdd(&jb.info->dbg[kDbgWindows], 1ull);
+            atomicAdd(&jb.info->dbg[kDbgStage], (unsigned long long)(t_1 - t_0));
+            atomicAdd(&jb.info->dbg[kDbgWalk], (unsigned long long)(t_2 - t_1));
         }
         return;
     }
@@ -634,6 +585,141 @@
         jb.M[x] = v;
         jb.SK[x] = 0xffffu;
     }
+}
+
+__global__ void __launch_bounds__(1024) k_redo_list(JobBufs jb)
+{
+    constexpr uint32_t kPer = kRedoPiece / 1024;
+    constexpr uint32_t wmax = (kWSize + kRedoPiece) / 32 + 1;
+    __shared__ uint32_t sbm[2048], sdel[wmax], pdel[wmax], sadd[wmax], padd[wmax], s_wsum[32];
+    const uint32_t tile = jb.skip_list[blockIdx.x / (kMatchTile / kRedoPiece)];
+    const uint32_t ps = tile * kMatchTile + (blockIdx.x % (kMatchTile / kRedoPiece)) * kRedoPiece, N = jb.N;
+    if (ps >= N) return;
+    const uint32_t pe = min(ps + kRedoPiece, N);
+    const uint32_t ws = ps >= kWSize ? ps - kWSize : 0;
+    const uint32_t tid = threadIdx.x, lane = tid & 31, warp = tid >> 5;
+    {
+        const uint32_t *bm1 = jb.bucket_map + (size_t)tile * 2048, *bm0 = tile ? bm1 - 2048 : bm1;
+        for (uint32_t i = tid; i < 2048; i += 1024) sbm[i] = bm0[i] | bm1[i];
+    }
+    __syncthreads();
+    const uint32_t x0 = ps + kPer * tid;
+    uint32_t hits = 0;
+    if (x0 < pe) {
+        const uint32_t *iw = reinterpret_cast<const uint32_t *>(jb.in + x0);
+        const uint32_t w0 = iw[0], w1 = iw[1];
+#pragma unroll
+        for (uint32_t j = 0; j < kPer; j++) {
+            const uint32_t h = hash_u32(__funnelshift_r(w0, w1, j * 8));
+            if (x0 + j + kMSafe <= N && ((sbm[h >> 5] >> (h & 31)) & 1u)) hits |= 1u << j;
+        }
+    }
+    if (!__syncthreads_or(hits)) return;
+    const uint32_t nwd = (pe - ws + 31) / 32;
+    const uint32_t per = (nwd + 1 + 1023) / 1024;
+    const uint32_t wb = tid * per;
+    for (int which = 0; which < 2; which++) {
+        const uint32_t *src = which ? jb.hdiff : jb.hdiff + jb.hdiff_words;
+        uint32_t *bits = which ? sadd : sdel, *pre = which ? padd : pdel;
+        uint32_t mine = 0;
+        for (uint32_t k = 0; k < per; k++) {
+            const uint32_t w = wb + k;
+            if (w <= nwd) { const uint32_t v = w < nwd ? src[(ws >> 5) + w] : 0u; bits[w] = v; mine += __popc(v); }
+        }
+        uint32_t incl = mine;
+#pragma unroll
+        for (int d = 1; d < 32; d <<= 1) {
+            const uint32_t t = __shfl_up_sync(0xffffffffu, incl, d);
+            if (lane >= (uint32_t)d) incl += t;
+        }
+        __syncthreads();
+        if (lane == 31) s_wsum[warp] = incl;
+        __syncthreads();
+        uint32_t run = incl - mine;
+        for (uint32_t k = 0; k < warp; k++) run += s_wsum[k];
+        for (uint32_t k = 0; k < per; k++) {
+            const uint32_t w = wb + k;
+            if (w <= nwd) { pre[w] = run; run += __popc(bits[w]); }
+        }
+    }
+    __syncthreads();
+    const DiffBits del{sdel, pdel, ws >> 5}, add{sadd, padd, ws >> 5};
+    const uint32_t md = jb.wsize - kMinLookahead;
+    uint32_t mask = 0;
+#pragma unroll
+    for (uint32_t j = 0; j < kPer; j++) {
+        const uint32_t x = x0 + j;
+        if (((hits >> j) & 1u) && redo_position(true, x, jb.SK[x], jb.M[x], jb.Lr[x], md, del, add)) mask |= 1u << j;
+    }
+    const uint32_t c = __popc(mask);
+    uint32_t incl = c;
+#pragma unroll
+    for (int d = 1; d < 32; d <<= 1) {
+        const uint32_t t = __shfl_up_sync(0xffffffffu, incl, d);
+        if (lane >= (uint32_t)d) incl += t;
+    }
+    __syncthreads();
+    if (lane == 31) s_wsum[warp] = incl;
+    __syncthreads();
+    uint32_t off = incl - c;
+    for (uint32_t k = 0; k < warp; k++) off += s_wsum[k];
+    for (uint32_t m = mask, i = off; m; m &= m - 1, i++) jb.redo_pos[ps + i] = x0 + (__ffs(m) - 1);
+    if (tid == 1023) {
+        const uint32_t cnt = off + c, K = jb.redo_item, nit = (cnt + K - 1) / K;
+        const uint32_t base = nit ? atomicAdd(&jb.info->redo_items, nit) : 0u;
+        for (uint32_t j = 0; j < nit; j++) jb.redo_items[base + j] = make_uint4(ps, ps + j * K, min(K, cnt - j * K), 0u);
+    }
+}
+
+__global__ void __launch_bounds__(1024, 2) k_match_sparse(JobBufs jb)
+{
+    extern __shared__ __align__(16) uint8_t smem[];
+    __shared__ uint32_t s_next;
+    __shared__ uint4 s_item;
+    __shared__ __align__(8) unsigned long long s_mbar;
+    constexpr uint32_t data_bytes = kWSize + kRedoPiece + 512;
+    uint8_t *sdata = smem;
+    uint16_t *sL = reinterpret_cast<uint16_t *>(smem + data_bytes);
+    const uint32_t tid = threadIdx.x;
+    if (tid == 0) {
+        mbar_init(&s_mbar);
+        if (jb.debug) atomicAdd(&jb.info->dbg[kDbgCtas], 1ull);
+    }
+    for (uint32_t parity = 0;; parity ^= 1u) {
+        if (tid == 0) {
+            const uint32_t i = atomicAdd(&jb.info->redo_next, 1u);
+            const uint4 it = i < *(volatile uint32_t *)&jb.info->redo_items ? jb.redo_items[i] : make_uint4(0xffffffffu, 0u, 0u, 0u);
+            s_item = it;
+            s_next = it.y;
+        }
+        __syncthreads();
+        const uint4 it = s_item;
+        if (it.x == 0xffffffffu) break;
+        const uint32_t ts = it.x, te = min(ts + kRedoPiece, jb.N);
+        const uint32_t ws = ts >= kWSize ? ts - kWSize : 0;
+        const uint32_t t_0 = (uint32_t)clock64();
+        stage_window(jb, sdata, sL, ws, te, data_bytes, &s_mbar, parity);
+        __syncthreads();
+        const uint32_t t_1 = (uint32_t)clock64();
+        match_tile_fast<true>(jb, sdata, sL, ws, it.y + it.z, &s_next);
+        __syncthreads();
+        if (jb.debug && tid == 0) {
+            const uint32_t t_2 = (uint32_t)clock64();
+            atomicAdd(&jb.info->dbg[kDbgWindows], 1ull);
+            atomicAdd(&jb.info->dbg[kDbgStage], (unsigned long long)(t_1 - t_0));
+            atomicAdd(&jb.info->dbg[kDbgWalk], (unsigned long long)(t_2 - t_1));
+        }
+    }
+}
+
+__global__ void __launch_bounds__(256) k_match_check(JobBufs jb, const uint32_t *m_sparse)
+{
+    const uint32_t ts = jb.skip_list[blockIdx.x] * kMatchTile;
+    const uint32_t te = min(ts + kMatchTile, jb.N);
+    uint32_t bad = 0;
+    for (uint32_t x = ts + threadIdx.x; x < te; x += blockDim.x) bad += jb.M[x] != m_sparse[x];
+    for (int d = 16; d; d >>= 1) bad += __shfl_xor_sync(0xffffffffu, bad, d);
+    if ((threadIdx.x & 31) == 0 && bad) atomicAdd(&jb.info->dbg[kDbgMismatch], (unsigned long long)bad);
 }
 
 constexpr uint32_t kMacroReach = 22016;
@@ -1101,6 +1187,8 @@
         }
         __syncthreads();
         if (tid == 0) {
+            jb.info->redo_items = 0;
+            jb.info->redo_next = 0;
             if (which) { jb.info->n_ptiles = base; jb.info->first_ptile = s_first == 0xffffffffu ? 0u : s_first; }
             else jb.info->n_dirty = base;
         }
diff --git a/zlib_rs_b200/csrc/zb_kernels.cuh b/zlib_rs_b200/csrc/zb_kernels.cuh
--- a/zlib_rs_b200/csrc/zb_kernels.cuh
+++ b/zlib_rs_b200/csrc/zb_kernels.cuh
@@ -3,12 +3,14 @@
 #include "zb_core.h"
 #include "zb_huff.h"
 #include "zb_slow.h"
+#include "zb_redo.h"
 
 namespace zb {
 
 constexpr uint32_t kLinkTile = 32768;
 constexpr uint32_t kMatchTile = 32768;
 constexpr uint32_t kMatchSub = 8192;
+constexpr uint32_t kRedoPiece = 4096;
 constexpr uint32_t kPathTile = 16384;
 constexpr uint32_t kPathSub = 256;
 constexpr uint32_t kLongPerSub = 4;
@@ -29,6 +31,14 @@
     return __funnelshift_r(sld_u32(al), sld_u32(al + 4), (a & 3u) * 8u);
 }
 
+enum { kDbgCtas = 0,
+       kDbgWindows = 1,
+       kDbgWalked = 2,
+       kDbgStage = 3,
+       kDbgWalk = 4,
+       kDbgMismatch = 5,
+       kDbgCounters = 6 };
+
 struct JobInfo {
     uint32_t n_mid_syms;
     uint32_t tail_entry;
@@ -43,7 +53,9 @@
     uint64_t out_bytes;
     uint32_t adler;
     uint64_t marker_byte;
-    unsigned long long dbg[3];
+    uint32_t redo_items;
+    uint32_t redo_next;
+    unsigned long long dbg[kDbgCounters];
 };
 
 struct JobBufs {
@@ -105,6 +117,10 @@
     uint32_t *block_base;
     uint32_t wsize;
     uint32_t cinfo;
+    uint32_t debug;
+    uint32_t *redo_pos;
+    uint4 *redo_items;
+    uint32_t redo_item;
 };
 
 cudaError_t upload_tables();
diff --git a/zlib_rs_b200/csrc/zb_redo.h b/zlib_rs_b200/csrc/zb_redo.h
--- /dev/null
+++ b/zlib_rs_b200/csrc/zb_redo.h
@@ -0,0 +1,39 @@
+#pragma once
+#include "zb_core.h"
+
+namespace zb {
+
+ZB_HD uint32_t popc_u32(uint32_t v)
+{
+#ifdef __CUDA_ARCH__
+    return __popc(v);
+#else
+    return (uint32_t)__builtin_popcount(v);
+#endif
+}
+
+struct DiffBits {
+    const uint32_t *bits, *pre;
+    uint32_t w0;
+    ZB_HD uint32_t count_below(uint32_t y) const
+    {
+        const uint32_t w = (y >> 5) - w0;
+        return pre[w] + popc_u32(bits[w] & ((1u << (y & 31)) - 1u));
+    }
+    ZB_HD bool any(uint32_t lo, uint32_t hi) const { return count_below(hi) != count_below(lo); }
+    ZB_HD bool test(uint32_t y) const { return (bits[(y >> 5) - w0] >> (y & 31)) & 1u; }
+};
+
+ZB_HD bool redo_position(bool bucket_hit, uint32_t x, uint32_t rd, uint32_t m, uint32_t lr, uint32_t md, const DiffBits &del,
+                         const DiffBits &add)
+{
+    if (!bucket_hit) return false;
+    const bool on_budget = rd != 0xffffu && (rd & 0x8000u);
+    const uint32_t lo = rd == 0xffffu ? (x > md ? x - md : 0u) : x - (rd & 0x7fffu);
+    if (del.any(lo, x)) return true;
+    if (on_budget) { if (add.any(lo, x)) return true; }
+    else if (m && add.test(x - (m & 0xffffu))) return true;
+    return lr == md;
+}
+
+}
```
